# Fadi987/PL-BERT

Measured on AMD Instinct MI355X. Metric: phoneme-tokens/sec, higher is better.
Workload: dtype bf16; 1 GPU; PL-BERT masked-phoneme training step (fwd+loss+bwd+allreduce+AdamW), ALBERT hidden 768 / 12 shared layers / FFN 2048 / 12 heads, seq_len 512, batch 32 per GPU; global_batch=32, seq_len=512, parallelism=dp1

## Files before the change

include/plbert.h:

```cpp
#ifndef PLBERT_H
#define PLBERT_H

#include <stdint.h>

#ifdef __cplusplus
extern "C" {
#endif

typedef struct PlbEngine PlbEngine;

typedef struct {
  int32_t vocab_size;
  int32_t embedding_size;
  int32_t hidden_size;
  int32_t num_attention_heads;
  int32_t intermediate_size;
  int32_t num_hidden_layers;
  int32_t max_position_embeddings;
  int32_t type_vocab_size;
  float layer_norm_eps;
  int32_t num_phonemes;
  int32_t num_tokens;
  int32_t max_batch;
  int32_t max_seq;
  int32_t inference_only;
} PlbConfig;

enum PlbParam {
  PLB_WORD_EMB = 0,
  PLB_POS_EMB,
  PLB_TYPE_EMB,
  PLB_EMB_LN_W,
  PLB_EMB_LN_B,
  PLB_MAP_W,
  PLB_MAP_B,
  PLB_LN2_W,
  PLB_LN2_B,
  PLB_Q_W, PLB_K_W, PLB_V_W,
  PLB_Q_B, PLB_K_B, PLB_V_B,
  PLB_DENSE_W,
  PLB_DENSE_B,
  PLB_LN1_W,
  PLB_LN1_B,
  PLB_FFN_W,
  PLB_FFN_B,
  PLB_FFNO_W,
  PLB_FFNO_B,
  PLB_HEAD_W,
  PLB_HEAD_B,
  PLB_POOL_W,
  PLB_POOL_B,
  PLB_TOK_W,
  PLB_TOK_B,
  PLB_NPARAM
};

const char* plb_last_error(void);

int plb_create(const PlbConfig* cfg, PlbEngine** out);
void plb_destroy(PlbEngine* e);

int plb_param_layout(const PlbEngine* e, int64_t* offsets, int64_t* sizes, int64_t* total, int64_t* trainable);

int64_t plb_workspace_bytes(const PlbEngine* e);

int plb_bind(PlbEngine* e, float* params, float* grads, float* exp_avg, float* exp_avg_sq, void* workspace,
             int64_t workspace_bytes);

int plb_sync_weights(PlbEngine* e, void* stream);

int plb_forward(PlbEngine* e, const int64_t* ids, const int32_t* lengths, int32_t B, int32_t S, float* hidden,
                float* phoneme_logits, float* token_logits, void* stream);

int plb_pooler(PlbEngine* e, const float* hidden, int32_t B, int32_t S, float* pooled, void* stream);

int plb_loss_fwd_bwd(PlbEngine* e, const int64_t* masked_ids, const int64_t* labels, const int32_t* lengths,
                     const int32_t* idx_offsets, const int32_t* idx_flat, int32_t n_masked, int32_t B, int32_t S,
                     float* loss, void* stream);

int plb_loss_fwd(PlbEngine* e, const int64_t* masked_ids, const int64_t* labels, const int64_t* token_ids,
                 const int32_t* lengths, const int32_t* idx_offsets, const int32_t* idx_flat, int32_t n_masked, int32_t B,
                 int32_t S, float* loss, float* loss_parts, void* stream);

int plb_loss_fwd_bwd_dual(PlbEngine* e, const int64_t* masked_ids, const int64_t* labels, const int64_t* token_ids,
                          const int32_t* lengths, const int32_t* idx_offsets, const int32_t* idx_flat, int32_t n_masked,
                          int32_t B, int32_t S, float* loss, float* loss_parts, void* stream);

int plb_adamw_step(PlbEngine* e, double lr, double beta1, double beta2, double eps, double weight_decay, int32_t step,
                   double grad_scale, void* stream);

int64_t plb_grad_norm_floats(const PlbEngine* e);
int plb_grad_accum_bind(PlbEngine* e, float* accum);
int plb_grad_accum_add(PlbEngine* e, int32_t phase, float* norm_buf, void* stream);
int plb_grad_norm(PlbEngine* e, double grad_scale, double max_norm, float* norm_buf, int32_t have_partials, void* stream);
int plb_adamw_step_clipped(PlbEngine* e, double lr, double beta1, double beta2, double eps, double weight_decay,
                           int32_t step, double grad_scale, const float* norm_buf, void* stream);

int plb_set_fp8(PlbEngine* e, int32_t on, void* stream);
int plb_fp8_state(const PlbEngine* e, int32_t* enabled, int32_t* calibrated);
int plb_fp8_stats(PlbEngine* e, float clamped_calls[8], float worst_overshoot[8], void* stream);

int32_t plb_token_head_steps(const PlbEngine* e);
int plb_set_token_head_steps(PlbEngine* e, int32_t steps);

#define PLB_COMM_ID_BYTES 128
int plb_comm_unique_id(uint8_t id[PLB_COMM_ID_BYTES]);
int plb_comm_init(PlbEngine* e, const uint8_t id[PLB_COMM_ID_BYTES], int32_t rank, int32_t world);
int plb_comm_destroy(PlbEngine* e);
int plb_comm_info(const PlbEngine* e, int32_t* rank, int32_t* world, int32_t* rccl_version);
int plb_status(PlbEngine* e, int32_t* ln_exchange_timeouts);
int plb_status_ex(PlbEngine* e, int32_t* ln_exchange_timeouts, int32_t* skipped_updates);
int plb_poll_status(const PlbEngine* e, int32_t* ln_exchange_timeouts);
int plb_status_export(PlbEngine* e, float* out, void* stream);
int plb_status_import(PlbEngine* e, const float* summed, void* stream);
int plb_last_application_rows(const PlbEngine* e, int64_t* rows, int64_t* of);
typedef struct {
  const int32_t* row_start;
  int32_t rows;
  int32_t used;
} PlbPacking;
int plb_packing_plan(const int32_t* lengths, int32_t B, int32_t S, int32_t* row_start, int32_t* rows, int32_t* used);
int plb_forward_packed(PlbEngine* e, const int64_t* ids, const int32_t* lengths, int32_t B, int32_t S,
                       const PlbPacking* packing, float* hidden, float* phoneme_logits, float* token_logits, void* stream);
int plb_loss_fwd_bwd_packed(PlbEngine* e, const int64_t* masked_ids, const int64_t* labels, const int32_t* lengths,
                            const int32_t* idx_offsets, const int32_t* idx_flat, int32_t n_masked, int32_t B, int32_t S,
                            const PlbPacking* packing, float* loss, void* stream);
int plb_loss_fwd_packed(PlbEngine* e, const int64_t* masked_ids, const int64_t* labels, const int64_t* token_ids,
                        const int32_t* lengths, const int32_t* idx_offsets, const int32_t* idx_flat, int32_t n_masked,
                        int32_t B, int32_t S, const PlbPacking* packing, float* loss, float* loss_parts, void* stream);
int plb_last_call_rows(const PlbEngine* e, int64_t* rows, int64_t* of);
int plb_set_packed_dual(PlbEngine* e, int32_t on);
int plb_loss_fwd_bwd_dual_packed(PlbEngine* e, const int64_t* masked_ids, const int64_t* labels, const int64_t* token_ids,
                                 const int32_t* lengths, const int32_t* idx_offsets, const int32_t* idx_flat, int32_t n_masked,
                                 int32_t B, int32_t S, const PlbPacking* packing, float* loss, float* loss_parts, void* stream);
int plb_set_packed_fp8(PlbEngine* e, int32_t on);
int plb_encode(PlbEngine* e, const int64_t* ids, const int32_t* lengths, int32_t B, int32_t S, const PlbPacking* packing,
               float* hidden, void* stream);
int plb_encode_bwd(PlbEngine* e, const int64_t* ids, const int32_t* lengths, int32_t B, int32_t S, const PlbPacking* packing,
                   const float* d_hidden, void* stream);
int plb_comm_pieces(const PlbEngine* e, int32_t* collectives, int64_t* floats);
int plb_broadcast_params(PlbEngine* e, int32_t root, void* stream);
int plb_set_grad_overlap(PlbEngine* e, int32_t overlap);
int plb_allreduce_grads(PlbEngine* e, void* stream);

int plb_apply_mask(const int64_t* ids, const int32_t* sample_off, const int32_t* word_off, const int32_t* word_begin,
                   const int32_t* word_len, const int8_t* action, const int64_t* repl, const int64_t* word_token,
                   int64_t sep_token, const int32_t* crop_start, int32_t B, int32_t S, int32_t mask_id, int64_t* labels,
                   int64_t* masked, int64_t* tokens, int32_t* lengths_out, int32_t* idx_offsets, int32_t* idx_flat,
                   int32_t* scratch, void* stream);

int plb_mask_batch(const int64_t* labels, const int32_t* lengths, int32_t B, int32_t S, uint64_t seed, uint32_t step,
                   float word_pred_prob, float phoneme_mask_prob, float replace_prob, int32_t mask_id, int32_t sep_id,
                   int64_t* masked, int32_t* idx_offsets, int32_t* idx_flat, int32_t* scratch, void* stream);

void plb_profile_enable(int on);
int plb_profile_num_classes(void);
const char* plb_profile_class_name(int cls);
int plb_profile_read(double* ms, int64_t* launches, double* flops, double* bytes);

void plb_debug_skip_piece(int index);
void plb_debug_ln_fault(int mode, int launches);
int plb_debug_hb_audit(PlbEngine* e, int32_t on, int32_t break_wait);
int plb_debug_hb_report(const PlbEngine* e, int64_t* checks, int32_t* violations, char* first, int32_t first_bytes);
int plb_comm_trace(PlbEngine* e, int32_t on);
int plb_comm_trace_read(PlbEngine* e, int32_t max_pieces, int32_t* n, int64_t* begin, int64_t* end, float* released_ms,
                        float* done_ms, float* tail_ms);
void plb_set_gemm_nt_tile(int tile);
void plb_set_gemm_nt_prefetch(int on);
void plb_set_attn_bwd_fused(int on);
void plb_set_prune_last(int on);

#ifdef __cplusplus
}
#endif
#endif
```

plbert_amd/_lib.py:

```python
from __future__ import annotations

import ctypes as C
import os

import torch

HERE = os.path.dirname(os.path.abspath(__file__))
LIB_PATH = os.environ.get("PLBERT_HIP_LIB") or os.path.join(HERE, "libplbert_hip.so")

PLB_PARAM_NAMES = [
    "encoder.embeddings.word_embeddings.weight",
    "encoder.embeddings.position_embeddings.weight",
    "encoder.embeddings.token_type_embeddings.weight",
    "encoder.embeddings.LayerNorm.weight",
    "encoder.embeddings.LayerNorm.bias",
    "encoder.encoder.embedding_hidden_mapping_in.weight",
    "encoder.encoder.embedding_hidden_mapping_in.bias",
    "encoder.encoder.albert_layer_groups.0.albert_layers.0.full_layer_layer_norm.weight",
    "encoder.encoder.albert_layer_groups.0.albert_layers.0.full_layer_layer_norm.bias",
    "encoder.encoder.albert_layer_groups.0.albert_layers.0.attention.query.weight",
    "encoder.encoder.albert_layer_groups.0.albert_layers.0.attention.key.weight",
    "encoder.encoder.albert_layer_groups.0.albert_layers.0.attention.value.weight",
    "encoder.encoder.albert_layer_groups.0.albert_layers.0.attention.query.bias",
    "encoder.encoder.albert_layer_groups.0.albert_layers.0.attention.key.bias",
    "encoder.encoder.albert_layer_groups.0.albert_layers.0.attention.value.bias",
    "encoder.encoder.albert_layer_groups.0.albert_layers.0.attention.dense.weight",
    "encoder.encoder.albert_layer_groups.0.albert_layers.0.attention.dense.bias",
    "encoder.encoder.albert_layer_groups.0.albert_layers.0.attention.LayerNorm.weight",
    "encoder.encoder.albert_layer_groups.0.albert_layers.0.attention.LayerNorm.bias",
    "encoder.encoder.albert_layer_groups.0.albert_layers.0.ffn.weight",
    "encoder.encoder.albert_layer_groups.0.albert_layers.0.ffn.bias",
    "encoder.encoder.albert_layer_groups.0.albert_layers.0.ffn_output.weight",
    "encoder.encoder.albert_layer_groups.0.albert_layers.0.ffn_output.bias",
    "phoneme_predictor.weight",
    "phoneme_predictor.bias",
    "encoder.pooler.weight",
    "encoder.pooler.bias",
    "token_predictor.weight",
    "token_predictor.bias",
]
PLB_NPARAM = len(PLB_PARAM_NAMES)

PUBLIC_SYMBOLS = [
    "plb_last_error", "plb_create", "plb_destroy", "plb_param_layout", "plb_workspace_bytes", "plb_bind",
    "plb_sync_weights", "plb_forward", "plb_pooler", "plb_loss_fwd_bwd", "plb_loss_fwd", "plb_loss_fwd_bwd_dual", "plb_adamw_step",
    "plb_set_fp8", "plb_fp8_state", "plb_fp8_stats", "plb_token_head_steps", "plb_set_token_head_steps", "plb_comm_unique_id", "plb_comm_init", "plb_comm_destroy",
    "plb_comm_info", "plb_comm_pieces", "plb_last_application_rows", "plb_last_call_rows",
    "plb_packing_plan", "plb_forward_packed", "plb_loss_fwd_bwd_packed", "plb_loss_fwd_packed", "plb_set_packed_dual",
    "plb_set_packed_fp8",
    "plb_grad_norm_floats", "plb_grad_accum_bind", "plb_grad_accum_add", "plb_grad_norm", "plb_adamw_step_clipped",
    "plb_loss_fwd_bwd_dual_packed", "plb_encode", "plb_encode_bwd", "plb_status", "plb_status_ex", "plb_poll_status", "plb_status_export", "plb_status_import", "plb_broadcast_params", "plb_set_grad_overlap", "plb_allreduce_grads", "plb_apply_mask",
    "plb_mask_batch", "plb_profile_enable", "plb_profile_num_classes", "plb_profile_class_name", "plb_profile_read",
    "plb_debug_skip_piece", "plb_debug_ln_fault", "plb_debug_hb_audit", "plb_debug_hb_report", "plb_comm_trace", "plb_comm_trace_read",
    "plb_set_gemm_nt_tile", "plb_set_gemm_nt_prefetch", "plb_set_attn_bwd_fused", "plb_set_prune_last",
]


class PlbConfig(C.Structure):
    _fields_ = [
        ("vocab_size", C.c_int32), ("embedding_size", C.c_int32), ("hidden_size", C.c_int32),
        ("num_attention_heads", C.c_int32), ("intermediate_size", C.c_int32), ("num_hidden_layers", C.c_int32),
        ("max_position_embeddings", C.c_int32), ("type_vocab_size", C.c_int32), ("layer_norm_eps", C.c_float),
        ("num_phonemes", C.c_int32), ("num_tokens", C.c_int32), ("max_batch", C.c_int32), ("max_seq", C.c_int32),
        ("inference_only", C.c_int32),
    ]


class PlbGemmNT(C.Structure):
    _fields_ = [
        ("A", C.c_void_p), ("lda", C.c_int), ("B", C.c_void_p), ("ldb", C.c_int),
        ("M", C.c_int), ("N", C.c_int), ("K", C.c_int), ("Mstore", C.c_int),
        ("bias", C.c_void_p), ("res", C.c_void_p), ("ldr", C.c_int), ("aux", C.c_void_p), ("ldaux", C.c_int),
        ("C", C.c_void_p), ("ldc", C.c_int), ("C2", C.c_void_p), ("ldc2", C.c_int), ("Cf", C.c_void_p), ("ldcf", C.c_int),
        ("colpart", C.c_void_p),
        ("ce_cols", C.c_int), ("ce_tgt", C.c_void_p), ("ce_pmax", C.c_void_p), ("ce_psum", C.c_void_p),
        ("ce_tlogit", C.c_void_p), ("ce_lse", C.c_void_p), ("ce_w", C.c_void_p),
        ("deq_a", C.c_void_p), ("deq_b", C.c_void_p), ("C8", C.c_void_p), ("ldc8", C.c_int), ("q_scale", C.c_void_p),
        ("q_amax", C.c_void_p), ("c8_bf8", C.c_int),
        ("ln_gamma", C.c_void_p), ("ln_beta", C.c_void_p), ("ln_mean", C.c_void_p), ("ln_rstd", C.c_void_p),
        ("ln_eps", C.c_float), ("ln_xchg", C.c_void_p), ("ln_err", C.c_void_p), ("ln_fault", C.c_int),
    ]


class PlbGemmTN(C.Structure):
    _fields_ = [
        ("A", C.c_void_p), ("lda", C.c_int), ("Ncols", C.c_int), ("B", C.c_void_p), ("ldb", C.c_int),
        ("Mtot", C.c_int), ("N", C.c_int), ("K", C.c_int), ("rows_per_split", C.c_int), ("splits", C.c_int),
        ("slab", C.c_void_p), ("deq_a", C.c_void_p), ("deq_b", C.c_void_p),
    ]


class PlbAttn(C.Structure):
    _fields_ = [
        ("qkv", C.c_void_p), ("ldqkv", C.c_int), ("lengths", C.c_void_p),
        ("B", C.c_int), ("S", C.c_int), ("NH", C.c_int), ("H", C.c_int), ("scale", C.c_float),
        ("ctx", C.c_void_p), ("ldctx", C.c_int), ("lse", C.c_void_p),
        ("dctx", C.c_void_p), ("lddctx", C.c_int), ("delta", C.c_void_p), ("dqkv", C.c_void_p), ("lddqkv", C.c_int),
        ("colpart", C.c_void_p), ("colpart_accumulate", C.c_int),
        ("ctx8", C.c_void_p), ("ldctx8", C.c_int), ("ctx_scale", C.c_void_p), ("ctx_amax", C.c_void_p),
        ("dqkv8", C.c_void_p), ("lddqkv8", C.c_int), ("dqkv_scale", C.c_void_p), ("dqkv_amax", C.c_void_p),
        ("qoff", C.c_void_p), ("q", C.c_void_p), ("ldq", C.c_int), ("nq_total", C.c_int), ("dq", C.c_void_p), ("lddq", C.c_int),
        ("dq8", C.c_void_p), ("lddq8", C.c_int),
        ("row_start", C.c_void_p),
    ]


class PlbEmbed(C.Structure):
    _fields_ = [
        ("ids", C.c_void_p), ("T", C.c_int), ("S", C.c_int), ("E", C.c_int), ("V", C.c_int),
        ("word", C.c_void_p), ("pos", C.c_void_p), ("type0", C.c_void_p), ("gamma", C.c_void_p), ("beta", C.c_void_p),
        ("eps", C.c_float), ("out", C.c_void_p), ("ldo", C.c_int), ("dout", C.c_void_p), ("lddo", C.c_int),
        ("dx", C.c_void_p), ("dword", C.c_void_p), ("dpos", C.c_void_p), ("partials", C.c_void_p), ("nblocks", C.c_int),
        ("row_start", C.c_void_p), ("lengths", C.c_void_p), ("B", C.c_int), ("fill_slots", C.c_int),
    ]


class PlbPacking(C.Structure):
    _fields_ = [("row_start", C.c_void_p), ("rows", C.c_int32), ("used", C.c_int32)]


class PlbLayerNorm(C.Structure):
    _fields_ = [
        ("x", C.c_void_p), ("ldx", C.c_int), ("gamma", C.c_void_p), ("beta", C.c_void_p), ("eps", C.c_float),
        ("y", C.c_void_p), ("ldy", C.c_int), ("mean", C.c_void_p), ("rstd", C.c_void_p),
        ("T", C.c_int), ("H", C.c_int), ("Tzero", C.c_int),
        ("dy", C.c_void_p), ("lddy", C.c_int), ("dx", C.c_void_p), ("lddx", C.c_int),
        ("partials", C.c_void_p), ("nblocks", C.c_int), ("accumulate", C.c_int),
        ("out8", C.c_void_p), ("ld8", C.c_int), ("q_scale", C.c_void_p), ("q_amax", C.c_void_p),
    ]


PLB_NORM_PARTS = 1024


def norm_chunk(n):
    return (n + PLB_NORM_PARTS * 1024 - 1) // (PLB_NORM_PARTS * 1024) * 1024


def norm_chain(n):
    return 4 * (norm_chunk(n) // 1024) + 6 + 3


_lib = None


class HipLibraryMissing(RuntimeError):
    pass


def lib():
    global _lib
    if _lib is not None:
        return _lib
    if not os.path.exists(LIB_PATH):
        raise HipLibraryMissing(
            f"{LIB_PATH} is missing: build it with `python -m plbert_amd.build` (needs hipcc, gfx950). "
            "There is no CPU fallback for the PL-BERT hot path.")
    try:
        L = C.CDLL(LIB_PATH, mode=C.RTLD_GLOBAL)
    except OSError as ex:
        raise HipLibraryMissing(f"cannot load {LIB_PATH}: {ex}") from ex
    vp, i32, i64p, f32, f64 = C.c_void_p, C.c_int32, C.POINTER(C.c_int64), C.c_float, C.c_double
    L.plb_last_error.restype = C.c_char_p
    L.plb_last_error.argtypes = []
    L.plb_create.restype = C.c_int
    L.plb_create.argtypes = [C.POINTER(PlbConfig), C.POINTER(vp)]
    L.plb_destroy.restype = None
    L.plb_destroy.argtypes = [vp]
    L.plb_param_layout.restype = C.c_int
    L.plb_param_layout.argtypes = [vp, i64p, i64p, i64p, i64p]
    L.plb_workspace_bytes.restype = C.c_int64
    L.plb_workspace_bytes.argtypes = [vp]
    L.plb_bind.restype = C.c_int
    L.plb_bind.argtypes = [vp, vp, vp, vp, vp, vp, C.c_int64]
    L.plb_sync_weights.restype = C.c_int
    L.plb_sync_weights.argtypes = [vp, vp]
    L.plb_forward.restype = C.c_int
    L.plb_forward.argtypes = [vp, vp, vp, i32, i32, vp, vp, vp, vp]
    L.plb_loss_fwd_bwd.restype = C.c_int
    L.plb_loss_fwd_bwd.argtypes = [vp, vp, vp, vp, vp, vp, i32, i32, i32, vp, vp]
    L.plb_loss_fwd_bwd_dual.restype = C.c_int
    L.plb_loss_fwd_bwd_dual.argtypes = [vp, vp, vp, vp, vp, vp, vp, i32, i32, i32, vp, vp, vp]
    L.plb_pooler.restype = C.c_int
    L.plb_pooler.argtypes = [vp, vp, i32, i32, vp, vp]
    L.plb_loss_fwd.restype = C.c_int
    L.plb_loss_fwd.argtypes = [vp, vp, vp, vp, vp, vp, vp, i32, i32, i32, vp, vp, vp]
    L.plb_set_fp8.restype = C.c_int
    L.plb_set_fp8.argtypes = [vp, i32, vp]
    L.plb_fp8_state.restype = C.c_int
    L.plb_fp8_state.argtypes = [vp, C.POINTER(i32), C.POINTER(i32)]
    L.plb_token_head_steps.restype = i32
    L.plb_token_head_steps.argtypes = [vp]
    L.plb_set_token_head_steps.restype = C.c_int
    L.plb_set_token_head_steps.argtypes = [vp, i32]
    L.plb_comm_unique_id.restype = C.c_int
    L.plb_comm_unique_id.argtypes = [vp]
    L.plb_comm_init.restype = C.c_int
    L.plb_comm_init.argtypes = [vp, vp, i32, i32]
    L.plb_comm_destroy.restype = C.c_int
    L.plb_comm_destroy.argtypes = [vp]
    L.plb_comm_info.restype = C.c_int
    L.plb_comm_info.argtypes = [vp, C.POINTER(i32), C.POINTER(i32), C.POINTER(i32)]
    L.plb_status.restype = C.c_int
    L.plb_status.argtypes = [vp, C.POINTER(i32)]
    L.plb_status_ex.restype = C.c_int
    L.plb_status_ex.argtypes = [vp, C.POINTER(i32), C.POINTER(i32)]
    L.plb_poll_status.restype = C.c_int
    L.plb_poll_status.argtypes = [vp, C.POINTER(i32)]
    L.plb_fp8_stats.restype = C.c_int
    L.plb_fp8_stats.argtypes = [vp, C.POINTER(f32), C.POINTER(f32), vp]
    L.plb_last_application_rows.restype = C.c_int
    L.plb_last_application_rows.argtypes = [vp, i64p, i64p]
    if hasattr(L, "plb_packing_plan"):
        pk = C.POINTER(PlbPacking)
        L.plb_last_call_rows.restype = C.c_int
        L.plb_last_call_rows.argtypes = [vp, i64p, i64p]
        L.plb_packing_plan.restype = C.c_int
        L.plb_packing_plan.argtypes = [vp, i32, i32, vp, C.POINTER(i32), C.POINTER(i32)]
        L.plb_forward_packed.restype = C.c_int
        L.plb_forward_packed.argtypes = [vp, vp, vp, i32, i32, pk, vp, vp, vp, vp]
        L.plb_loss_fwd_bwd_packed.restype = C.c_int
        L.plb_loss_fwd_bwd_packed.argtypes = [vp, vp, vp, vp, vp, vp, i32, i32, i32, pk, vp, vp]
        L.plb_loss_fwd_packed.restype = C.c_int
        L.plb_loss_fwd_packed.argtypes = [vp, vp, vp, vp, vp, vp, vp, i32, i32, i32, pk, vp, vp, vp]
        L.plb_launch_ce_prepare_packed.restype = C.c_int
        L.plb_launch_ce_prepare_packed.argtypes = [vp, vp, vp, C.c_int, C.c_int, vp, vp, vp, vp, vp]
        L.plb_launch_unpack_rows.restype = C.c_int
        L.plb_launch_unpack_rows.argtypes = [vp, C.c_int, C.c_int, vp, vp, C.c_int, C.c_int, C.c_int, vp, vp]
    if hasattr(L, "plb_encode"):
        L.plb_encode.restype = C.c_int
        L.plb_encode.argtypes = [vp, vp, vp, i32, i32, C.POINTER(PlbPacking), vp, vp]
        L.plb_encode_bwd.restype = C.c_int
        L.plb_encode_bwd.argtypes = [vp, vp, vp, i32, i32, C.POINTER(PlbPacking), vp, vp]
        L.plb_launch_seed_dy.restype = C.c_int
        L.plb_launch_seed_dy.argtypes = [vp, vp, vp, C.c_int, C.c_int, C.c_int, C.c_int, vp, vp]
    if hasattr(L, "plb_set_packed_dual"):
        L.plb_set_packed_dual.restype = C.c_int
        L.plb_set_packed_dual.argtypes = [vp, i32]
        L.plb_loss_fwd_bwd_dual_packed.restype = C.c_int
        L.plb_loss_fwd_bwd_dual_packed.argtypes = [vp, vp, vp, vp, vp, vp, vp, i32, i32, i32, C.POINTER(PlbPacking), vp, vp, vp]
        L.plb_launch_pack_token_targets.restype = C.c_int
        L.plb_launch_pack_token_targets.argtypes = [vp, vp, vp, C.c_int, C.c_int, C.c_int, vp, vp]
        L.plb_launch_token_ce_combine_packed.restype = C.c_int
        L.plb_launch_token_ce_combine_packed.argtypes = [vp, vp, C.c_int, vp, vp, vp, C.c_int, C.c_int, C.c_int, vp, vp, vp, vp]
    if hasattr(L, "plb_set_packed_fp8"):
        L.plb_set_packed_fp8.restype = C.c_int
        L.plb_set_packed_fp8.argtypes = [vp, i32]
    if hasattr(L, "plb_grad_accum_add"):
        L.plb_grad_norm_floats.restype = C.c_int64
        L.plb_grad_norm_floats.argtypes = [vp]
        L.plb_grad_accum_bind.restype = C.c_int
        L.plb_grad_accum_bind.argtypes = [vp, vp]
        L.plb_grad_accum_add.restype = C.c_int
        L.plb_grad_accum_add.argtypes = [vp, i32, vp, vp]
        L.plb_grad_norm.restype = C.c_int
        L.plb_grad_norm.argtypes = [vp, f64, f64, vp, i32, vp]
        L.plb_adamw_step_clipped.restype = C.c_int
        L.plb_adamw_step_clipped.argtypes = [vp, f64, f64, f64, f64, f64, i32, f64, vp, vp]
        L.plb_launch_grad_accum.restype = C.c_int
        L.plb_launch_grad_accum.argtypes = [vp, vp, C.c_size_t, C.c_int, vp, vp]
        L.plb_launch_grad_sumsq.restype = C.c_int
        L.plb_launch_grad_sumsq.argtypes = [vp, C.c_size_t, vp, vp]
        L.plb_launch_grad_norm_finish.restype = C.c_int
        L.plb_launch_grad_norm_finish.argtypes = [vp, C.c_int, f64, f64, vp, vp]
        L.plb_launch_adamw_clipped.restype = C.c_int
        L.plb_launch_adamw_clipped.argtypes = [vp, vp, vp, vp, vp, C.c_size_t, f64, f64, f64, f64, f64, C.c_int, f64, vp, C.c_int,
                                               vp, C.c_int, vp]
    L.plb_status_export.restype = C.c_int
    L.plb_status_export.argtypes = [vp, vp, vp]
    L.plb_status_import.restype = C.c_int
    L.plb_status_import.argtypes = [vp, vp, vp]
    L.plb_debug_hb_audit.restype = C.c_int
    L.plb_debug_hb_audit.argtypes = [vp, i32, i32]
    L.plb_debug_hb_report.restype = C.c_int
    L.plb_debug_hb_report.argtypes = [vp, i64p, C.POINTER(i32), C.c_char_p, i32]
    L.plb_comm_trace.restype = C.c_int
    L.plb_comm_trace.argtypes = [vp, i32]
    L.plb_comm_trace_read.restype = C.c_int
    L.plb_comm_trace_read.argtypes = [vp, i32, C.POINTER(i32), i64p, i64p, C.POINTER(f32), C.POINTER(f32), C.POINTER(f32)]
    L.plb_debug_ln_fault.restype = None
    L.plb_debug_ln_fault.argtypes = [C.c_int, C.c_int]
    L.plb_debug_skip_piece.restype = None
    L.plb_debug_skip_piece.argtypes = [C.c_int]
    L.plb_comm_pieces.restype = C.c_int
    L.plb_comm_pieces.argtypes = [vp, C.POINTER(i32), C.POINTER(C.c_int64)]
    L.plb_broadcast_params.restype = C.c_int
    L.plb_broadcast_params.argtypes = [vp, i32, vp]
    L.plb_set_grad_overlap.restype = C.c_int
    L.plb_set_grad_overlap.argtypes = [vp, i32]
    L.plb_allreduce_grads.restype = C.c_int
    L.plb_allreduce_grads.argtypes = [vp, vp]
    L.plb_apply_mask.restype = C.c_int
    L.plb_apply_mask.argtypes = [vp, vp, vp, vp, vp, vp, vp, vp, C.c_int64, vp, i32, i32, i32, vp, vp, vp, vp, vp, vp, vp, vp]
    L.plb_adamw_step.restype = C.c_int
    L.plb_adamw_step.argtypes = [vp, f64, f64, f64, f64, f64, i32, f64, vp]
    L.plb_mask_batch.restype = C.c_int
    L.plb_mask_batch.argtypes = [vp, vp, i32, i32, C.c_uint64, C.c_uint32, f32, f32, f32, i32, i32, vp, vp, vp, vp, vp]
    L.plb_profile_enable.restype = None
    L.plb_profile_enable.argtypes = [C.c_int]
    L.plb_profile_num_classes.restype = C.c_int
    L.plb_profile_num_classes.argtypes = []
    L.plb_profile_class_name.restype = C.c_char_p
    L.plb_profile_class_name.argtypes = [C.c_int]
    L.plb_profile_read.restype = C.c_int
    L.plb_profile_read.argtypes = [C.POINTER(C.c_double), i64p, C.POINTER(C.c_double), C.POINTER(C.c_double)]
    L.plb_launch_gemm_nt.restype = C.c_int
    L.plb_launch_gemm_nt.argtypes = [C.POINTER(PlbGemmNT), C.c_int, C.c_int, vp]
    L.plb_set_gemm_nt_tile.restype = None
    L.plb_set_gemm_nt_tile.argtypes = [C.c_int]
    L.plb_set_gemm_nt_prefetch.restype = None
    L.plb_set_gemm_nt_prefetch.argtypes = [C.c_int]
    L.plb_launch_gemm_nt_fp8.restype = C.c_int
    L.plb_launch_gemm_nt_fp8.argtypes = [C.POINTER(PlbGemmNT), C.c_int, C.c_int, vp]
    L.plb_launch_gemm_nt_fp8_ln.restype = C.c_int
    L.plb_launch_gemm_nt_fp8_ln.argtypes = [C.POINTER(PlbGemmNT), C.c_int, C.c_int, vp]
    L.plb_launch_gemm_nt_fp8_gelud.restype = C.c_int
    L.plb_launch_gemm_nt_fp8_gelud.argtypes = [C.POINTER(PlbGemmNT), C.c_int, C.c_int, vp]
    L.plb_launch_gemm_tn.restype = C.c_int
    L.plb_launch_gemm_tn.argtypes = [C.POINTER(PlbGemmTN), vp]
    L.plb_launch_gemm_tn_big.restype = C.c_int
    L.plb_launch_gemm_tn_big.argtypes = [C.POINTER(PlbGemmTN), vp]
    L.plb_launch_gemm_tn_fp8.restype = C.c_int
    L.plb_launch_gemm_tn_fp8.argtypes = [C.POINTER(PlbGemmTN), vp]
    L.plb_launch_reduce_slabs.restype = C.c_int
    L.plb_launch_reduce_slabs.argtypes = [vp, C.c_int, C.c_size_t, vp, C.c_int, vp]
    L.plb_launch_attn_fwd.restype = C.c_int
    L.plb_launch_attn_fwd.argtypes = [C.POINTER(PlbAttn), vp]
    L.plb_launch_gemm_nt_ln.restype = C.c_int
    L.plb_launch_gemm_nt_ln.argtypes = [C.POINTER(PlbGemmNT), C.c_int, vp]
    L.plb_launch_gemm_nt_gelud.restype = C.c_int
    L.plb_launch_gemm_nt_gelud.argtypes = [C.POINTER(PlbGemmNT), C.c_int, vp]
    L.plb_launch_attn_bwd.restype = C.c_int
    L.plb_launch_attn_bwd.argtypes = [C.POINTER(PlbAttn), vp]
    L.plb_launch_attn_bwd_fused.restype = C.c_int
    L.plb_launch_attn_bwd_fused.argtypes = [C.POINTER(PlbAttn), vp]
    L.plb_set_prune_last.restype = None
    L.plb_set_prune_last.argtypes = [C.c_int]
    L.plb_set_attn_bwd_fused.restype = None
    L.plb_set_attn_bwd_fused.argtypes = [C.c_int]
    L.plb_launch_ln_fwd.restype = C.c_int
    L.plb_launch_ln_fwd.argtypes = [C.POINTER(PlbLayerNorm), vp]
    L.plb_launch_ln_bwd.restype = C.c_int
    L.plb_launch_ln_bwd.argtypes = [C.POINTER(PlbLayerNorm), vp]
    L.plb_launch_embed_scatter.restype = C.c_int
    L.plb_launch_embed_scatter.argtypes = [C.POINTER(PlbEmbed), C.c_int, vp]
    L.plb_launch_ce_prepare.restype = C.c_int
    L.plb_launch_ce_prepare.argtypes = [vp, vp, vp, C.c_int, C.c_int, vp, vp, vp, vp]
    L.plb_launch_colsum.restype = C.c_int
    L.plb_launch_colsum.argtypes = [vp, C.c_int, C.c_size_t, C.c_int, C.c_int, vp, C.c_int, C.c_int, vp, C.c_int, vp]
    _lib = L
    return L


def profile_enable(on):
    lib().plb_profile_enable(int(bool(on)))


def profile_read():
    L = lib()
    n = L.plb_profile_num_classes()
    ms, fl, by = (C.c_double * n)(), (C.c_double * n)(), (C.c_double * n)()
    cnt = (C.c_int64 * n)()
    check(L.plb_profile_read(ms, cnt, fl, by), "plb_profile_read")
    return {L.plb_profile_class_name(i).decode(): dict(ms=ms[i], launches=int(cnt[i]), flops=fl[i], bytes=by[i])
            for i in range(n) if cnt[i]}


def check(rc, what):
    if rc != 0:
        msg = lib().plb_last_error().decode("utf-8", "replace")
        raise RuntimeError(f"{what} failed: {msg or 'rc=%d' % rc}")
```

plbert_amd/csrc/engine.cpp:

```cpp
#include <stdarg.h>

#include <new>

#include "engine_internal.h"

static thread_local char g_err[512] = "";
int fail(const char* fmt, ...) {
  va_list ap;
  va_start(ap, fmt);
  vsnprintf(g_err, sizeof(g_err), fmt, ap);
  va_end(ap);
  return 1;
}
extern "C" const char* plb_last_error(void) { return g_err; }

static void layout_params(PlbEngine* e) {
  const int64_t V = e->V, E = e->E, H = e->H, I = e->I, P = e->P, NP = e->NP, NT = e->NT;
  int64_t sz[PLB_NPARAM];
  sz[PLB_WORD_EMB] = V * E; sz[PLB_POS_EMB] = P * E; sz[PLB_TYPE_EMB] = (int64_t)e->c.type_vocab_size * E;
  sz[PLB_EMB_LN_W] = E; sz[PLB_EMB_LN_B] = E;
  sz[PLB_MAP_W] = H * E; sz[PLB_MAP_B] = H;
  sz[PLB_LN2_W] = H; sz[PLB_LN2_B] = H;
  sz[PLB_Q_W] = sz[PLB_K_W] = sz[PLB_V_W] = H * H;
  sz[PLB_Q_B] = sz[PLB_K_B] = sz[PLB_V_B] = H;
  sz[PLB_DENSE_W] = H * H; sz[PLB_DENSE_B] = H;
  sz[PLB_LN1_W] = H; sz[PLB_LN1_B] = H;
  sz[PLB_FFN_W] = I * H; sz[PLB_FFN_B] = I;
  sz[PLB_FFNO_W] = H * I; sz[PLB_FFNO_B] = H;
  sz[PLB_HEAD_W] = NP * H; sz[PLB_HEAD_B] = NP;
  sz[PLB_POOL_W] = H * H; sz[PLB_POOL_B] = H;
  sz[PLB_TOK_W] = NT * H; sz[PLB_TOK_B] = NT;
  int64_t off = 0;
  for (int i = 0; i < PLB_NPARAM; ++i) {
    e->poff[i] = off;
    e->psize[i] = sz[i];
    off += sz[i];
    if (i == PLB_HEAD_B) e->ptrain = off;
  }
  e->ptotal = off;
}

namespace {
struct Carve {
  int64_t off = 0;
  int64_t take(int64_t bytes) {
    int64_t o = off;
    off = rup(off + bytes, 256);
    return o;
  }
};
}

extern "C" int plb_create(const PlbConfig* cfg, PlbEngine** out) {
  if (!cfg || !out) return fail("plb_create: null argument");
  const PlbConfig& c = *cfg;
  if (c.hidden_size != c.num_attention_heads * 64) return fail("plb_create: head_dim must be 64 (hidden %d, heads %d)", c.hidden_size, c.num_attention_heads);
  if (c.embedding_size % 64 || c.embedding_size > 256) return fail("plb_create: embedding_size must be a multiple of 64, <= 256");
  if (c.hidden_size % 128 || c.hidden_size > 1024) return fail("plb_create: hidden_size must be a multiple of 128, <= 1024");
  if (c.intermediate_size % 128) return fail("plb_create: intermediate_size must be a multiple of 128");
  if (c.num_phonemes < 4 || c.num_phonemes % 4 || c.num_phonemes > 256) return fail("plb_create: num_phonemes must be a multiple of 4 in [4,256]");
  if (c.num_tokens < 0 || c.num_tokens % 4) return fail("plb_create: num_tokens must be a non-negative multiple of 4");
  if (c.max_seq < 1 || c.max_seq > c.max_position_embeddings) return fail("plb_create: max_seq must be in [1, max_position_embeddings]");
  if (c.max_batch < 1 || c.num_hidden_layers < 1 || c.vocab_size < 1 || c.type_vocab_size < 1) return fail("plb_create: bad sizes");
  PlbEngine* e = new (std::nothrow) PlbEngine();
  if (!e) return fail("plb_create: out of host memory");
  e->c = c;
  e->E = c.embedding_size; e->H = c.hidden_size; e->I = c.intermediate_size; e->L = c.num_hidden_layers;
  e->NH = c.num_attention_heads; e->V = c.vocab_size; e->P = c.max_position_embeddings;
  e->NP = c.num_phonemes; e->NT = c.num_tokens;
  layout_params(e);
  const int64_t E = e->E, H = e->H, I = e->I, L = e->L;
  const int64_t T = (int64_t)c.max_batch * c.max_seq;
  const int64_t Tp = rup(T, 128);
  e->infer = c.inference_only != 0;
  const bool tr = !e->infer;
  const int64_t Ls = tr ? L : 1;
  e->Tcap = Tp;
  e->NMcap = Tp;
  e->ln_blocks = 512;
  if (const char* v = getenv("PLBERT_LN_BLOCKS")) { const int n = atoi(v); if (n >= 64 && n <= 4096) e->ln_blocks = n; }
  e->emb_blocks = 2048;
  if (const char* v = getenv("PLBERT_LN_FUSE"))
    e->ln_fuse = !strcmp(v, "off") ? 0 : !strcmp(v, "fwd") ? 1 : !strcmp(v, "bwd") ? 2 : 3;
  e->part_rows = e->ln_blocks > (int)(2 * Tp / 128) ? e->ln_blocks : (int)(2 * Tp / 128);
  if (const char* v = getenv("PLBERT_GELU_STASH")) e->gelu_dstash_on = strcmp(v, "u") != 0;
  if (const char* v = getenv("PLBERT_FP8_TN")) e->fp8_tn = strcmp(v, "0") != 0;
  if (const char* v = getenv("PLBERT_HB_AUDIT")) e->hb.on = strcmp(v, "0") != 0;
  Carve cv;
  e->o_wbf = cv.take((e->ptotal + 256 * (H > I ? H : I)) * 2);
  if (tr) {
    e->o_wqkvT = cv.take(rup(H, 128) * 3 * H * 2);
    e->o_wdT = cv.take(rup(H, 128) * H * 2);
    e->o_w1T = cv.take(rup(H, 128) * I * 2);
    e->o_w2T = cv.take(rup(I, 128) * H * 2);
    e->o_wpT = cv.take(rup(H, 128) * 256 * 2);
    e->o_winT = cv.take(rup(E, 128) * H * 2);
  }
  e->o_e = cv.take(Tp * E * 2);
  e->o_x = cv.take((tr ? L + 1 : 2) * Tp * H * 2);
  e->o_qkv = cv.take(Ls * Tp * 3 * H * 2);
  e->o_ctx = cv.take(Ls * Tp * H * 2);
  e->o_pre1 = cv.take(Ls * Tp * H * 2);
  e->o_a = cv.take(Ls * Tp * H * 2);
  e->o_u = cv.take(Ls * Tp * I * 2);
  e->o_g = cv.take(Ls * Tp * I * 2);
  e->o_pre2 = cv.take(Ls * Tp * H * 2);
  const int64_t stat = (int64_t)c.max_batch * e->NH * c.max_seq * 4;
  e->o_lse = cv.take(Ls * stat);
  e->o_mean1 = cv.take(Ls * Tp * 4); e->o_rstd1 = cv.take(Ls * Tp * 4);
  e->o_mean2 = cv.take(Ls * Tp * 4); e->o_rstd2 = cv.take(Ls * Tp * 4);
  e->lnx_bytes = (Tp / 128) * 16 * 128 * 2 * 8;
  e->o_lnx = cv.take(e->lnx_bytes);
  e->o_lnerr = cv.take(256);
  if (tr) {
    e->o_delta = cv.take(stat);
    e->o_dqkv = cv.take(L * Tp * 3 * H * 2);
    e->o_dpre1 = cv.take(L * Tp * H * 2);
    e->o_du = cv.take(L * Tp * I * 2);
    e->o_dpre2 = cv.take(L * Tp * H * 2);
    e->o_dy0 = cv.take(Tp * H * 2); e->o_dy1 = cv.take(Tp * H * 2);
    e->o_da = cv.take(Tp * H * 2); e->o_dctx = cv.take(Tp * H * 2);
    e->o_de = cv.take(Tp * E * 2);
  }
  const int64_t NM = e->NMcap;
  e->o_hm = cv.take(NM * H * 2);
  e->o_logm = cv.take(NM * 256 * 4);
  e->o_dlog = cv.take(NM * 256 * 2);
  e->o_rows = cv.take(NM * 4); e->o_tgt = cv.take(NM * 4); e->o_w = cv.take(NM * 4); e->o_lrows = cv.take(NM * 4);
  if (tr) {
    e->o_dhm = cv.take(NM * H * 2);
    int64_t slab = 0;
    {
      const int64_t Mtot = L * Tp;
      const int ntp = (int)rup(e->NT, 256);
      const int shapes[7][2] = {{(int)(3 * H), (int)H}, {(int)H, (int)H}, {(int)I, (int)H}, {(int)H, (int)I}, {(int)H, (int)E}, {e->NP, (int)H}, {ntp, (int)H}};
      for (int i = 0; i < (e->NT ? 7 : 6); ++i) {
        int rps;
        const int64_t mt = i < 4 ? Mtot : Tp;
        const int s = tn_splits(mt, shapes[i][0], shapes[i][1], &rps);
        const int64_t f = (int64_t)s * shapes[i][0] * shapes[i][1];
        if (f > slab) slab = f;
      }
    }
    e->slab_floats = slab;
    e->o_slab = cv.take(slab * 4);
    e->o_part1 = cv.take(L * e->part_rows * 3 * H * 4);
    e->o_part2 = cv.take(L * e->part_rows * 3 * H * 4);
    e->o_parte = cv.take((int64_t)e->emb_blocks * 2 * E * 4);
    e->o_dxe = cv.take(Tp * E * 4);
    e->o_ducol = cv.take(L * (2 * Tp / 128) * I * 4);
    e->qkvcol_rows = c.max_batch * ((c.max_seq + 127) / 128) * 4;
    e->o_qkvcol = cv.take((int64_t)L * e->qkvcol_rows * 3 * H * 4);
    e->o_scratch = cv.take(512 * (3 * H > I ? 3 * H : I) * 4);
    e->o_scratch2 = cv.take(512 * (3 * H > I ? 3 * H : I) * 4);
    {
      int rps;
      const int s2 = tn_splits(Tp, (int)H, (int)E, &rps);
      e->slab2_floats = (int64_t)s2 * H * E;
      e->o_slab2 = cv.take(e->slab2_floats * 4);
    }
  }
  if (e->NT) {
    const int64_t NTp = rup(e->NT, 256);
    e->NTp = (int)NTp;
    e->o_bt = cv.take(NTp * 4);
    e->o_tlrows = cv.take(Tp * 4);
    e->o_tpmax = cv.take(Tp * (NTp / 256) * 4);
    e->o_tpsum = cv.take(Tp * (NTp / 256) * 4);
    e->o_ttl = cv.take(Tp * 4); e->o_tlse = cv.take(Tp * 4); e->o_tw = cv.take(Tp * 4);
    e->o_ttgt = cv.take(Tp * 8);
    e->o_tloss = cv.take(256);
    if (tr) {
      e->o_wtT = cv.take(rup(H, 128) * NTp * 2);
      e->o_tdl = cv.take(Tp * NTp * 2);
      e->o_tscr = cv.take(32 * NTp * 4);
      e->o_tcolp = cv.take(2 * (Tp / 128) * NTp * 4);
      e->o_tgrad = cv.take(NTp * H * 4);
    }
  }
  e->o_x8 = cv.take(Ls * Tp * H); e->o_a8 = cv.take(Ls * Tp * H); e->o_g8 = cv.take(Ls * Tp * I); e->o_c8 = cv.take(Ls * Tp * H);
  e->o_wq8 = cv.take(rup(3 * H, 128) * H + 256 * H);
  e->o_wd8 = cv.take(rup(H, 128) * H + 256 * H);
  e->o_w18 = cv.take(rup(I, 128) * H + 256 * H);
  e->o_w28 = cv.take(rup(H, 128) * I + 256 * I);
  if (tr) {
    e->o_dp8 = cv.take(L * Tp * H); e->o_du8 = cv.take(L * Tp * I); e->o_dp18 = cv.take(L * Tp * H); e->o_dq8 = cv.take(L * Tp * 3 * H);
    e->o_w2T8 = cv.take(rup(I, 128) * H + 256 * H);
    e->o_w1T8 = cv.take(rup(H, 128) * I + 256 * I);
    e->o_wqT8 = cv.take(rup(H, 128) * 3 * H + 256 * 3 * H);
    e->o_wdT8 = cv.take(rup(H, 128) * H + 256 * H);
  }
  e->f8n = 8 * (int)L + 8;
  e->o_f8amax = cv.take((int64_t)e->f8n * 64 * 16 * 4); e->o_f8scale = cv.take(e->f8n * 4); e->o_f8deq = cv.take(e->f8n * 4);
  e->o_f8stats = cv.take(8 * 8 * 4);
  e->ws_bytes = cv.off;
  *out = e;
  return 0;
}

extern "C" void plb_destroy(PlbEngine* e) {
  if (!e) return;
  (void)plb_comm_destroy(e);
  if (e->ev_fork) (void)hipEventDestroy(e->ev_fork);
  if (e->ev_join) (void)hipEventDestroy(e->ev_join);
  if (e->side) (void)hipStreamDestroy(e->side);
  if (e->host_err) (void)hipHostFree(e->host_err);
  for (auto& t : e->trace) { (void)hipEventDestroy(t.released); (void)hipEventDestroy(t.done); }
  for (auto ev : e->trace_pool) (void)hipEventDestroy(ev);
  for (auto ev : {e->tr_call0, e->tr_tail0, e->tr_tail1}) if (ev) (void)hipEventDestroy(ev);
  delete e;
}

extern "C" int plb_param_layout(const PlbEngine* e, int64_t* offsets, int64_t* sizes, int64_t* total, int64_t* trainable) {
  if (!e) return fail("plb_param_layout: null engine");
  for (int i = 0; i < PLB_NPARAM; ++i) {
    if (offsets) offsets[i] = e->poff[i];
    if (sizes) sizes[i] = e->psize[i];
  }
  if (total) *total = e->ptotal;
  if (trainable) *trainable = e->ptrain;
  return 0;
}

extern "C" int64_t plb_workspace_bytes(const PlbEngine* e) { return e ? e->ws_bytes : -1; }

extern "C" int plb_bind(PlbEngine* e, float* params, float* grads, float* exp_avg, float* exp_avg_sq, void* workspace,
                        int64_t workspace_bytes) {
  if (!e || !params || !workspace) return fail("plb_bind: null argument");
  if (workspace_bytes < e->ws_bytes) return fail("plb_bind: workspace too small (%lld < %lld)", (long long)workspace_bytes, (long long)e->ws_bytes);
  if (((uintptr_t)params | (uintptr_t)grads | (uintptr_t)exp_avg | (uintptr_t)exp_avg_sq) & 15) return fail("plb_bind: buffers must be 16-byte aligned");
  if ((uintptr_t)workspace & 255) return fail("plb_bind: workspace must be 256-byte aligned");
  e->params = params; e->grads = grads; e->m = exp_avg; e->v = exp_avg_sq;
  e->ws = (char*)workspace;
  if (!e->host_err) {
    void* h = nullptr;
    if (hipHostMalloc(&h, 64, hipHostMallocMapped) == hipSuccess && h) {
      void* d = nullptr;
      if (hipHostGetDevicePointer(&d, h, 0) == hipSuccess && d) {
        e->host_err = (unsigned int*)h;
        e->host_err_dev = (unsigned int*)d;
        *e->host_err = 0;
      } else {
        (void)hipHostFree(h);
      }
    }
    if (!e->host_err) return fail("plb_bind: cannot allocate the pinned status word");
  }
  if (!e->side && grads && !getenv("PLBERT_NO_SIDE_STREAM")) {
    if (hipStreamCreateWithFlags(&e->side, hipStreamNonBlocking) != hipSuccess) e->side = nullptr;
    if (e->side && (hipEventCreateWithFlags(&e->ev_fork, kStreamOrderEvent) != hipSuccess ||
                    hipEventCreateWithFlags(&e->ev_join, kStreamOrderEvent) != hipSuccess)) {
      (void)hipStreamDestroy(e->side);
      e->side = nullptr;
    }
  }
  return 0;
}

int sync_transposes(PlbEngine* e, hipStream_t s, bool exact_fp8) {
  const int H = e->H, I = e->I, E = e->E;

  if (e->NT) {
    if (!e->tok_pad_zeroed) HIPTRY(hipMemsetAsync(e->at<float>(e->o_bt), 0, (size_t)e->NTp * 4, s));
    HIPTRY(hipMemcpyAsync(e->at<float>(e->o_bt), e->par(PLB_TOK_B), (size_t)e->NT * 4, hipMemcpyDeviceToDevice, s));
  }
  if (e->infer) {
    e->tok_pad_zeroed = true;
    if (e->fp8_on) return fp8_quantize_weights(e, s, exact_fp8 || e->fp8_wstale);
    return 0;
  }
  const float* tsrc[8] = {e->par(PLB_Q_W), e->par(PLB_DENSE_W), e->par(PLB_FFN_W), e->par(PLB_FFNO_W), e->par(PLB_HEAD_W),
                          e->par(PLB_MAP_W)};
  bf16_t* tdst[8] = {e->at<bf16_t>(e->o_wqkvT), e->at<bf16_t>(e->o_wdT), e->at<bf16_t>(e->o_w1T), e->at<bf16_t>(e->o_w2T),
                     e->at<bf16_t>(e->o_wpT), e->at<bf16_t>(e->o_winT)};
  int tR[8] = {3 * H, H, I, H, e->NP, H}, tC[8] = {H, H, H, I, H, E}, tld[8] = {3 * H, H, I, H, 256, H};
  int nt = 6;
  if (e->NT) {
    if (!e->tok_pad_zeroed) HIPTRY(hipMemsetAsync(e->at<bf16_t>(e->o_wtT), 0, (size_t)rup(H, 128) * e->NTp * 2, s));
    tsrc[nt] = e->par(PLB_TOK_W); tdst[nt] = e->at<bf16_t>(e->o_wtT); tR[nt] = e->NT; tC[nt] = H; tld[nt] = e->NTp;
    ++nt;
  }
  TRY(plb_launch_transpose_cast_multi(nt, tsrc, tR, tC, tdst, tld, s));
  e->tok_pad_zeroed = true;
  if (e->fp8_on) return fp8_quantize_weights(e, s, exact_fp8 || e->fp8_wstale);
  return 0;
}

extern "C" int plb_sync_weights(PlbEngine* e, void* stream) {
  if (!e || !e->ws) return fail("plb_sync_weights: engine not bound");
  drop_stash(e, "plb_sync_weights refreshed the compute copies since");
  end_accum_window(e, "plb_sync_weights refreshed the compute copies");
  hipStream_t s = (hipStream_t)stream;
  TRY(plb_launch_cast_bf16(e->params, e->at<bf16_t>(e->o_wbf), (size_t)e->ptotal, s));
  return sync_transposes(e, s);
}

extern "C" int plb_pooler(PlbEngine* e, const float* hidden, int32_t B, int32_t S, float* pooled, void* stream) {
  if (!e || !e->ws) return fail("plb_pooler: engine not bound");
  if (!hidden || !pooled || B < 1 || S < 1) return fail("plb_pooler: bad argument");
  TRY(plb_launch_pooler(hidden, B, S, e->H, e->par(PLB_POOL_W), e->par(PLB_POOL_B), pooled, (hipStream_t)stream));
  return 0;
}

#ifndef PLB_PACK_GRAN_MAX
#define PLB_PACK_GRAN_MAX 1024
#endif
extern "C" int plb_packing_plan(const int32_t* lengths, int32_t B, int32_t S, int32_t* row_start, int32_t* rows,
                                int32_t* used) {
  if (!lengths || !row_start || !rows || !used) return fail("plb_packing_plan: null argument");
  if (B < 1 || S < 1 || (int64_t)B * S > (int64_t)1 << 30) return fail("plb_packing_plan: bad shape %d x %d", B, S);
  const int64_t padded = rup((int64_t)B * S, 128);
  int64_t at = 0;
  bool full = true;
  for (int b = 0; b < B; ++b) {
    const int len = lengths[b] < 1 ? 1 : (lengths[b] > S ? S : lengths[b]);
    full = full && len == S;
    at += rup(len, 128);
  }
  const int64_t gran = (PLB_PACK_GRAN_MAX >= 1024 && rup(at, 1024) < padded) ? 1024
                       : (PLB_PACK_GRAN_MAX >= 256 && rup(at, 256) < padded) ? 256 : 128;
  if (full || rup(at, gran) >= padded) {
    for (int b = 0; b <= B; ++b) row_start[b] = b * S;
    *rows = (int32_t)padded; *used = B * S;
    return 0;
  }
  at = 0;
  for (int b = 0; b < B; ++b) {
    const int len = lengths[b] < 1 ? 1 : (lengths[b] > S ? S : lengths[b]);
    row_start[b] = (int32_t)at;
    at += rup(len, 128);
  }
  row_start[B] = (int32_t)at;
  *used = (int32_t)at;
  *rows = (int32_t)rup(at, gran);
  return 0;
}

extern "C" int plb_last_application_rows(const PlbEngine* e, int64_t* rows, int64_t* of) {
  if (!e) return fail("plb_last_application_rows: null engine");
  if (rows) *rows = e->last_app_rows[0];
  if (of) *of = e->last_app_rows[1];
  return 0;
}

extern "C" int plb_last_call_rows(const PlbEngine* e, int64_t* rows, int64_t* of) {
  if (!e) return fail("plb_last_call_rows: null engine");
  if (rows) *rows = e->last_exec_rows[0];
  if (of) *of = e->last_exec_rows[1];
  return 0;
}

extern "C" int plb_set_packed_dual(PlbEngine* e, int32_t on) {
  if (!e) return fail("plb_set_packed_dual: null engine");
  e->packed_dual = on != 0;
  return 0;
}
extern "C" int plb_set_packed_fp8(PlbEngine* e, int32_t on) {
  if (!e) return fail("plb_set_packed_fp8: null engine");
  e->packed_fp8 = on != 0;
  return 0;
}

extern "C" int32_t plb_token_head_steps(const PlbEngine* e) { return e ? e->tok_steps : -1; }
extern "C" int plb_set_token_head_steps(PlbEngine* e, int32_t steps) {
  if (!e || steps < 0) return fail("plb_set_token_head_steps: bad argument");
  e->tok_steps = steps;
  return 0;
}

extern "C" int plb_apply_mask(const int64_t* ids, const int32_t* sample_off, const int32_t* word_off,
                              const int32_t* word_begin, const int32_t* word_len, const int8_t* action, const int64_t* repl,
                              const int64_t* word_token, int64_t sep_token, const int32_t* crop_start, int32_t B, int32_t S,
                              int32_t mask_id, int64_t* labels, int64_t* masked, int64_t* tokens, int32_t* lengths_out,
                              int32_t* idx_offsets, int32_t* idx_flat, int32_t* scratch, void* stream) {
  if (!ids || !sample_off || !word_off || !word_begin || !word_len || !action || !repl || !crop_start || !labels || !masked ||
      !lengths_out || !idx_offsets || !idx_flat || !scratch)
    return fail("plb_apply_mask: null argument");
  if ((tokens != nullptr) != (word_token != nullptr)) return fail("plb_apply_mask: tokens and word_token go together");
  if (S < 1 || S > 1024 || B < 1 || B > 1024) return fail("plb_apply_mask: needs 1 <= S <= 1024, 1 <= B <= 1024");
  PlbApplyMask m;
  memset(&m, 0, sizeof(m));
  m.ids = ids; m.sample_off = sample_off; m.word_off = word_off; m.word_begin = word_begin; m.word_len = word_len;
  m.action = action; m.repl = repl; m.word_token = word_token; m.sep_token = sep_token; m.crop_start = crop_start;
  m.B = B; m.S = S; m.mask_id = mask_id;
  m.labels = labels; m.masked = masked; m.tokens = tokens; m.lengths_out = lengths_out;
  m.counts = scratch; m.idx_padded = scratch + B; m.offsets = idx_offsets; m.flat = idx_flat;
  TRY(plb_launch_apply_mask(&m, (hipStream_t)stream));
  return 0;
}

extern "C" int plb_mask_batch(const int64_t* labels, const int32_t* lengths, int32_t B, int32_t S, uint64_t seed,
                              uint32_t step, float word_pred_prob, float phoneme_mask_prob, float replace_prob,
                              int32_t mask_id, int32_t sep_id, int64_t* masked, int32_t* idx_offsets, int32_t* idx_flat,
                              int32_t* scratch, void* stream) {
  if (!labels || !masked || !idx_offsets || !idx_flat || !scratch) return fail("plb_mask_batch: null argument");
  if (S < 1 || S > 512 || B < 1 || B > 1024) return fail("plb_mask_batch: needs 1 <= S <= 512, 1 <= B <= 1024");
  PlbMask m;
  memset(&m, 0, sizeof(m));
  m.labels = labels; m.lengths = lengths; m.B = B; m.S = S; m.seed = seed; m.step = step;
  m.word_pred_prob = word_pred_prob; m.mask_prob = phoneme_mask_prob; m.replace_prob = replace_prob;
  m.mask_id = mask_id; m.sep_id = sep_id;
  m.masked = masked; m.counts = scratch; m.idx_padded = scratch + B; m.offsets = idx_offsets; m.flat = idx_flat;
  TRY(plb_launch_mask(&m, (hipStream_t)stream));
  return 0;
}

extern "C" int plb_adamw_step(PlbEngine* e, double lr, double beta1, double beta2, double eps, double weight_decay,
// ... 25 lines not shown
```

plbert_amd/csrc/engine_calls.cpp:

```cpp
#include "engine_internal.h"

void drop_stash(PlbEngine* e, const char* by) {
  if (e && e->stash_live) { e->stash_live = false; e->stash_dead_by = by; }
}

static int check_shape(const PlbEngine* e, int B, int S, const char* who) {
  if (!e || !e->ws) return fail("%s: engine not bound", who);
  if (B < 1 || S < 1 || B > e->c.max_batch || S > e->c.max_seq || (int64_t)B * S > (int64_t)e->c.max_batch * e->c.max_seq)
    return fail("%s: batch %d x seq %d exceeds the engine capacity %d x %d", who, B, S, e->c.max_batch, e->c.max_seq);
  return 0;
}

static Rows padded_rows(int B, int S) { return Rows{nullptr, B * S, rup(B * S, 128)}; }
static int pick_rows(PlbEngine* e, const PlbPacking* pk, const int32_t* lengths, bool padded, int B, int S, const char* who,
                     Rows* out) {
  *out = padded_rows(B, S);
  e->last_exec_rows[0] = e->last_exec_rows[1] = (int64_t)B * S;
  if (!pk || !pk->row_start) return 0;
  if (pk->rows < 128 || pk->rows % 128 || pk->used < 1 || pk->used > pk->rows)
    return fail("%s: packing plan of %d rows (%d used) is not one plb_packing_plan made", who, pk->rows, pk->used);
  if (pk->rows > out->Tp) return fail("%s: packing plan of %d rows exceeds the call's %lld", who, pk->rows, (long long)out->Tp);
  if (!lengths || padded || (e->fp8_on && !e->packed_fp8) || pk->rows == out->Tp) return 0;
  if (pk->used % 128) return fail("%s: packing plan with %d used rows: slots are multiples of 128", who, pk->used);
  *out = Rows{pk->row_start, pk->used, pk->rows};
// ... 101 lines not shown

static int phoneme_head(PlbEngine* e, bool backward, bool prune, const bf16_t* xL, int n_masked, int64_t Tp, bf16_t* dy,
                        float* loss, hipStream_t s) {
  const int H = e->H, NP = e->NP;
  const int NM = (int)rup(n_masked, 128);
  int32_t* rows = e->at<int32_t>(e->o_rows);
  bf16_t* hm = e->at<bf16_t>(e->o_hm);
  float* logm = e->at<float>(e->o_logm);
  float* lrows = e->at<float>(e->o_lrows);
  bf16_t* dlog = e->at<bf16_t>(e->o_dlog);
  bf16_t* dhm = e->at<bf16_t>(e->o_dhm);
  if (backward && !prune) HIPTRY(hipMemsetAsync(dy, 0, (size_t)Tp * H * 2, s));
  if (n_masked > 0) {
    if (!prune) TRY(plb_launch_gather_rows(xL, H, rows, n_masked, NM, H, hm, H, s));
    PlbGemmNT g = nt_desc(hm, e->wbf(PLB_HEAD_W), NM, NP, H);
    g.bias = e->par(PLB_HEAD_B); g.Cf = logm; g.ldcf = 256;
    TRY(plb_launch_gemm_nt(&g, 0, 1, s));
    TRY(plb_launch_ce_fwd_bwd(logm, 256, NP, e->at<int32_t>(e->o_tgt), e->at<float>(e->o_w), n_masked, NM, lrows, dlog, 256, s));
    TRY(plb_launch_sum_rows(lrows, n_masked, loss, s));
    if (backward) {
      if (weight_grad(e, dlog, 256, 256, hm, H, NM, NP, H, e->grd(PLB_HEAD_W), s)) return 1;
      TRY(plb_launch_colsum(dlog, 1, (size_t)NM, 256, 256, e->grd(PLB_HEAD_B), NP, 0, e->at<float>(e->o_scratch), 8, s));
      g = nt_desc(dlog, e->at<bf16_t>(e->o_wpT), NM, H, 256);
      g.C = dhm; g.ldc = H;
      TRY(plb_launch_gemm_nt(&g, 0, 0, s));
      if (!prune) TRY(plb_launch_scatter_rows(dhm, H, rows, n_masked, H, dy, H, s));
    }
  } else {
    HIPTRY(hipMemsetAsync(loss, 0, sizeof(float), s));
    if (backward)
      HIPTRY(hipMemsetAsync(e->grd(PLB_HEAD_W), 0, (size_t)(e->psize[PLB_HEAD_W] + e->psize[PLB_HEAD_B]) * 4, s));
  }
  if (!backward) return 0;
  HB_W(s, e->grd(PLB_HEAD_W), (e->ptrain - e->poff[PLB_HEAD_W]) * 4, "phoneme head gradients (weight-gradient GEMM, bias column sums)");
  if (overlapping(e) && reduce_pieces(e, kPieceHead, kPieceHead + 1, s)) return 1;
  return 0;
}

static int token_head(PlbEngine* e, bool backward, const bf16_t* xL, const int64_t* token_targets, const int32_t* lengths,
                      int B, int S, const Rows& rw, bf16_t* dy, float* loss, float* loss_parts, hipStream_t s) {
  const int H = e->H, NT = e->NT, NTp = e->NTp, T = B * S;
  const int64_t Tp = rw.Tp;
  const int tile = (Tp % 256 == 0) ? 256 : 1256;
  const int ntile = NTp / 256, cprows = tile == 256 ? 2 * (int)(Tp / 256) : 2 * (int)(Tp / 128);
  float* tlrows = e->at<float>(e->o_tlrows);
  float* tloss = e->at<float>(e->o_tloss);
  int64_t* ttgt = e->at<int64_t>(e->o_ttgt);
  if (rw.row_start) {
    TRY(plb_launch_pack_token_targets(token_targets, lengths, rw.row_start, B, S, (int)Tp, ttgt, s));
  } else {
  HIPTRY(hipMemcpyAsync(ttgt, token_targets, (size_t)T * 8, hipMemcpyDeviceToDevice, s));
  if (Tp > T) HIPTRY(hipMemsetAsync(ttgt + T, 0, (size_t)(Tp - T) * 8, s));
  }
  PlbGemmNT g = nt_desc(xL, e->wbf(PLB_TOK_W), Tp, NTp, H);
  g.bias = e->at<float>(e->o_bt);
  g.ce_cols = NT; g.ce_tgt = ttgt;
  g.ce_pmax = e->at<float>(e->o_tpmax); g.ce_psum = e->at<float>(e->o_tpsum); g.ce_tlogit = e->at<float>(e->o_ttl);
  const double ce_flops = 2.0 * (double)Tp * NTp * H;
  int tok = plb_prof_begin(PLB_K_GEMM_NT_CE, s, ce_flops, 0.0);
  TRY(plb_launch_gemm_nt_big(&g, tile, 3, 0, s));
  plb_prof_end(tok, s);
  if (rw.row_start) {
    TRY(plb_launch_token_ce_combine_packed(g.ce_pmax, g.ce_psum, ntile, g.ce_tlogit, lengths, rw.row_start, B, S, (int)Tp,
                                           e->at<float>(e->o_tlse), e->at<float>(e->o_tw), tlrows, s));
    TRY(plb_launch_sum_rows(tlrows, (int)Tp, tloss, s));
  } else {
  TRY(plb_launch_token_ce_combine(g.ce_pmax, g.ce_psum, ntile, g.ce_tlogit, lengths, B, S, (int)Tp,
                                  e->at<float>(e->o_tlse), e->at<float>(e->o_tw), tlrows, s));
  TRY(plb_launch_sum_rows(tlrows, T, tloss, s));
  }
  TRY(plb_launch_add_scalar(loss, loss, tloss, s));
  if (loss_parts) HIPTRY(hipMemcpyAsync(loss_parts + 1, tloss, sizeof(float), hipMemcpyDeviceToDevice, s));
  if (!backward) return 0;
  bf16_t* tdl = e->at<bf16_t>(e->o_tdl);
  g.ce_lse = e->at<float>(e->o_tlse); g.ce_w = e->at<float>(e->o_tw);
  g.C = tdl; g.ldc = NTp; g.colpart = e->at<float>(e->o_tcolp);
  tok = plb_prof_begin(PLB_K_GEMM_NT_CE, s, ce_flops, 0.0);
  TRY(plb_launch_gemm_nt_big(&g, tile, 4, 0, s));
  plb_prof_end(tok, s);
  TRY(plb_launch_colsum(g.colpart, 0, (size_t)cprows, NTp, NTp, e->grd(PLB_TOK_B), NT, 0, e->at<float>(e->o_tscr), 1, s));
  float* gw = NTp == NT ? e->grd(PLB_TOK_W) : e->at<float>(e->o_tgrad);
  if (weight_grad(e, tdl, NTp, NTp, xL, H, Tp, NTp, H, gw, s)) return 1;
  if (NTp != NT) HIPTRY(hipMemcpyAsync(e->grd(PLB_TOK_W), gw, (size_t)NT * H * 4, hipMemcpyDeviceToDevice, s));
  HB_W(s, e->grd(PLB_TOK_W), (e->ptotal - e->poff[PLB_TOK_W]) * 4, "token head gradients");
  if (overlapping(e) && reduce_piece(e, e->poff[PLB_TOK_W], e->ptotal, s)) return 1;
  g = nt_desc(tdl, e->at<bf16_t>(e->o_wtT), Tp, H, NTp);
  g.res = dy; g.ldr = H; g.C = dy; g.ldc = H;
  TRY(plb_launch_gemm_nt(&g, 0, 0, s));
  return 0;
}

static int backward_tail_streams(PlbEngine* e, const int64_t* masked_ids, const int32_t* lengths, bf16_t* dy, int B, int S,
                                 const Rows& rw, int du_rows, hipStream_t s, hipStream_t s2, float* scratch2) {
  const int E = e->E, H = e->H, I = e->I, L = e->L;
  const int T = rw.T;
  const int64_t Tp = rw.Tp;
  const int64_t Mtot = (int64_t)L * Tp;
  const int64_t Mtot_c = e->pruned_rows ? (int64_t)(L - 1) * Tp + e->pruned_rows : Mtot;
  const Slots st = slots(e, Tp, B, S, 0, true, e->part_rows_used, du_rows);
  const int64_t qkvcol_all = (int64_t)L * qkvcol_rows(B, S);
  bf16_t* evec = e->at<bf16_t>(e->o_e);
  bf16_t* de = e->at<bf16_t>(e->o_de);
  PlbGemmNT g = nt_desc(dy, e->at<bf16_t>(e->o_winT), Tp, E, H);
  g.C = de; g.ldc = E;
  HB_R(s2, dy, Tp * H * 2, "dX of application 0"); HB_W(s2, de, Tp * E * 2, "dE (map-in backward)");
  TRY(plb_launch_gemm_nt(&g, 0, 0, s2));
  HB_W(s2, e->at<float>(s2 != s ? e->o_slab2 : e->o_slab), (s2 != s ? e->slab2_floats : e->slab_floats) * 4, "map-in weight-gradient slab");
  HB_W(s2, e->grd(PLB_MAP_W), e->psize[PLB_MAP_W] * 4, "map-in weight gradient");
  if (weight_grad(e, dy, H, H, evec, E, Tp, H, E, e->grd(PLB_MAP_W), s2, s2 != s)) return 1;
  HB_W(s2, scratch2, 512 * (3 * H > I ? 3 * H : I) * 4, "column-sum scratch of the side stream");
  HB_W(s2, e->grd(PLB_MAP_B), H * 4, "map-in bias gradient");
  TRY(plb_launch_colsum(dy, 1, (size_t)Tp, H, H, e->grd(PLB_MAP_B), H, 0, scratch2, 128, s2));
  HB_W(s2, e->grd(PLB_TYPE_EMB), e->psize[PLB_TYPE_EMB] * 4, "token-type embedding gradient");
  HIPTRY(hipMemsetAsync(e->grd(PLB_TYPE_EMB), 0, (size_t)e->psize[PLB_TYPE_EMB] * 4, s2));
  PlbEmbed em;
  memset(&em, 0, sizeof(em));
  em.ids = masked_ids; em.T = T; em.S = S; em.E = E; em.V = e->V;
  em.word = e->par(PLB_WORD_EMB); em.pos = e->par(PLB_POS_EMB); em.type0 = e->par(PLB_TYPE_EMB);
  em.gamma = e->par(PLB_EMB_LN_W); em.beta = e->par(PLB_EMB_LN_B); em.eps = e->c.layer_norm_eps;
  em.dout = de; em.lddo = E; em.dword = e->grd(PLB_WORD_EMB); em.dpos = e->grd(PLB_POS_EMB);
  em.dx = e->at<float>(e->o_dxe);
  em.partials = e->at<float>(e->o_parte); em.nblocks = e->emb_blocks;
  if (rw.row_start) { em.row_start = rw.row_start; em.lengths = lengths; em.B = B; }
  HB_W(s2, em.dx, Tp * E * 4, "embedding LayerNorm backward rows"); HB_W(s2, em.partials, (int64_t)e->emb_blocks * 2 * E * 4, "embedding LayerNorm partials");
  HB_W(s2, e->grd(PLB_WORD_EMB), (e->poff[PLB_MAP_W] - e->poff[PLB_WORD_EMB]) * 4, "embedding tables' and embedding LayerNorm's gradients");
  TRY(plb_launch_embed_bwd(&em, s2));
  TRY(plb_launch_embed_scatter(&em, e->P, s2));
  TRY(plb_launch_colsum(em.partials, 0, (size_t)e->emb_blocks, 2 * E, 2 * E, e->grd(PLB_EMB_LN_W), 2 * E, 0, scratch2, 1, s2));
  TRY(plb_launch_colsum(e->grd(PLB_POS_EMB), 0, (size_t)e->P, E, E, e->grd(PLB_TYPE_EMB), E, 0, scratch2, 1, s2));
  HB_R(s2, st.qkvcol, qkvcol_all * 3 * H * 4, "Q/K/V bias partial rows");
  HB_W(s2, e->grd(PLB_Q_B), 3 * H * 4, "Q/K/V bias gradients");
  TRY(plb_launch_colsum(st.qkvcol, 0, (size_t)qkvcol_all, 3 * H, 3 * H, e->grd(PLB_Q_B), 3 * H, 0, scratch2, 64, s2));
  HB_W(s2, e->grd(PLB_FFN_B), I * 4, "ffn.bias gradient");
  if (du_rows > 0) {
    HB_R(s2, st.ducol, (int64_t)L * du_rows * I * 4, "dU column-sum partial rows");
    TRY(plb_launch_colsum(st.ducol, 0, (size_t)L * du_rows, I, I, e->grd(PLB_FFN_B), I, 0, scratch2, 16, s2));
  } else {
    HB_R(s2, st.du, Mtot_c * I * 2, "dU of every application");
    TRY(plb_launch_colsum(st.du, 1, (size_t)Mtot_c, I, I, e->grd(PLB_FFN_B), I, 0, scratch2, 64, s2));
  }
  const size_t prow = (size_t)L * e->part_rows_used;
  HB_R(s2, st.part1, (int64_t)L * e->part_rows * 3 * H * 4, "LayerNorm-1 backward partial rows");
  HB_W(s2, e->grd(PLB_DENSE_B), 3 * H * 4, "dense.bias + LayerNorm-1 affine gradients");
  TRY(plb_launch_colsum(st.part1, 0, prow, 3 * H, 3 * H, e->grd(PLB_LN1_W), 2 * H, 0, scratch2, 64, s2));
  TRY(plb_launch_copy_cols(scratch2, 64, 3 * H, 2 * H, H, e->grd(PLB_DENSE_B), s2));
  HB_R(s2, st.part2, (int64_t)L * e->part_rows * 3 * H * 4, "LayerNorm-2 backward partial rows");
  HB_W(s2, e->grd(PLB_LN2_W), 2 * H * 4, "LayerNorm-2 affine gradients"); HB_W(s2, e->grd(PLB_FFNO_B), H * 4, "ffn_output.bias gradient");
  TRY(plb_launch_colsum(st.part2, 0, prow, 3 * H, 3 * H, e->grd(PLB_LN2_W), 2 * H, 0, scratch2, 64, s2));
  TRY(plb_launch_copy_cols(scratch2, 64, 3 * H, 2 * H, H, e->grd(PLB_FFNO_B), s2));
  if (s2 != s) HIPTRY(ev_record(e, e->ev_join, s2));
  const bool ov = overlapping(e);
  const bool t8 = e->tn8_call;
  float* const slab = e->at<float>(e->o_slab);
  HB_W(s, slab, e->slab_floats * 4, "weight-gradient slab"); HB_W(s, e->grd(PLB_Q_W), 3 * H * H * 4, "Q/K/V weight gradients");
  if (t8 ? weight_grad8(e, st.dq8, st.x8, Mtot, 3 * H, H, F8_DQ, F8_X, e->grd(PLB_Q_W), s)
         : weight_grad(e, st.dqkv, 3 * H, 3 * H, st.x, H, Mtot, 3 * H, H, e->grd(PLB_Q_W), s)) return 1;
  if (ov && reduce_pieces(e, kPieceQkvW, kPieceFfnW, s)) return 1;
  HB_W(s, slab, e->slab_floats * 4, "weight-gradient slab"); HB_W(s, e->grd(PLB_FFN_W), (int64_t)I * H * 4, "ffn.weight gradient");
  if (t8 ? weight_grad8(e, st.du8, st.a8, Mtot_c, I, H, F8_DU, F8_A, e->grd(PLB_FFN_W), s)
         : weight_grad(e, st.du, I, I, st.a, H, Mtot_c, I, H, e->grd(PLB_FFN_W), s)) return 1;
  if (ov && reduce_pieces(e, kPieceFfnW, kPieceSmall, s)) return 1;
  if (ov) {
    if (reduce_pieces(e, kPieceSmall, kPieceFfnoW, s2)) return 1;
  }
  HB_W(s, slab, e->slab_floats * 4, "weight-gradient slab"); HB_W(s, e->grd(PLB_FFNO_W), (int64_t)I * H * 4, "ffn_output.weight gradient");
  if (t8 ? weight_grad8(e, st.dp8, st.g8, Mtot_c, H, I, F8_DP, F8_G, e->grd(PLB_FFNO_W), s)
         : weight_grad(e, st.dpre2, H, H, st.g, I, Mtot_c, H, I, e->grd(PLB_FFNO_W), s)) return 1;
  if (ov && reduce_pieces(e, kPieceFfnoW, kPieceDenseW, s)) return 1;
  HB_W(s, slab, e->slab_floats * 4, "weight-gradient slab"); HB_W(s, e->grd(PLB_DENSE_W), (int64_t)H * H * 4, "dense.weight gradient");
  if (t8 ? weight_grad8(e, st.dp18, st.c8, Mtot_c, H, H, F8_DP1, F8_C, e->grd(PLB_DENSE_W), s)
         : weight_grad(e, st.dpre1, H, H, st.ctx, H, Mtot_c, H, H, e->grd(PLB_DENSE_W), s)) return 1;
  if (ov && reduce_pieces(e, kPieceDenseW, kNPieces, s)) return 1;
  return 0;
}

static int backward_tail(PlbEngine* e, const int64_t* masked_ids, const int32_t* lengths, bf16_t* dy, int B, int S,
                         const Rows& rw, int du_rows, hipStream_t s) {
  hipStream_t s2 = s;
  float* scratch2 = e->at<float>(e->o_scratch);
  HB_W(s, e->ws, e->ws_bytes, "layer loop (whole workspace)");
  if (e->trace_on) (void)hipEventRecord(e->tr_tail0, s);
  if (e->side) {
    s2 = e->side;
    scratch2 = e->at<float>(e->o_scratch2);
    HIPTRY(ev_record(e, e->ev_fork, s));
    HIPTRY(ev_wait(e, s2, e->ev_fork));
  }
  const int rc = backward_tail_streams(e, masked_ids, lengths, dy, B, S, rw, du_rows, s, s2, scratch2);
  if (s2 != s) {
    if (rc) (void)ev_record(e, e->ev_join, s2);
    const hipError_t je = ev_wait(e, s, e->ev_join);
    if (!rc && je != hipSuccess) return fail("plb_loss_fwd_bwd: joining the side stream: %s", hipGetErrorString(je));
  }
  if (e->trace_on) { (void)hipEventRecord(e->tr_tail1, s); e->tr_tail_valid = true; }
  if (rc) return rc;
  HB_W(s, e->ws, e->ws_bytes, "after the side stream's join (whole workspace)");
  return pieces_done(e);
}

static int loss_impl(PlbEngine* e, bool backward, const int64_t* masked_ids, const int64_t* labels,
                     const int64_t* token_targets, const int32_t* lengths, const int32_t* idx_offsets,
                     const int32_t* idx_flat, int32_t n_masked, int32_t B, int32_t S, const PlbPacking* pk, float* loss,
                     float* loss_parts, void* stream) {
  const char* who = backward ? "plb_loss_fwd_bwd" : "plb_loss_fwd";
  if (check_shape(e, B, S, who)) return 1;
  drop_stash(e, "a plb_loss_* call rewrote the workspace since");
  if (backward && e->infer) return fail("%s: inference-only engine (PlbConfig.inference_only = 1)", who);
  if (backward && !e->grads) return fail("%s: no gradient buffer bound", who);
  if (!masked_ids || !labels || !idx_offsets || !loss) return fail("%s: null argument", who);
  if (n_masked < 0 || n_masked > e->NMcap) return fail("%s: n_masked %d out of range", who, n_masked);
  if (token_targets && !e->NT) return fail("%s: the engine has no token head (num_tokens = 0)", who);
  hipStream_t s = (hipStream_t)stream;
  Rows rw;
  if (pick_rows(e, pk, lengths, token_targets != nullptr && !e->packed_dual, B, S, who, &rw)) return 1;
  const int64_t Tp = rw.Tp;
  if (backward && begin_training_call(e, token_targets != nullptr, s)) return 1;
  if (n_masked == 0 && !token_targets) return zero_loss_call(e, backward, loss, s);

  const int NM = (int)rup(n_masked, 128);
  Prune pr = {e->at<int32_t>(e->o_rows), n_masked, NM};
  const bool prune = prune_enabled() && n_masked > 0 && !token_targets && e->L >= 2 && 2 * (int64_t)NM <= Tp;
  if (n_masked > 0) {
    if (rw.row_start)
      TRY(plb_launch_ce_prepare_packed(idx_offsets, idx_flat, labels, B, S, rw.row_start, e->at<int32_t>(e->o_rows),
                                       e->at<int32_t>(e->o_tgt), e->at<float>(e->o_w), s));
    else
      TRY(plb_launch_ce_prepare(idx_offsets, idx_flat, labels, B, S, e->at<int32_t>(e->o_rows), e->at<int32_t>(e->o_tgt),
                                e->at<float>(e->o_w), s));
  }
  if (backward) e->pruned_rows = prune ? NM : 0;
  e->last_app_rows[0] = prune ? NM : Tp; e->last_app_rows[1] = Tp;
  bf16_t* xL = nullptr;
  if (run_encoder(e, masked_ids, lengths, B, S, rw, backward, &xL, s, prune ? &pr : nullptr)) return 1;
  bf16_t* dy = backward ? e->at<bf16_t>(e->o_dy0) : nullptr;
  if (phoneme_head(e, backward, prune, xL, n_masked, Tp, dy, loss, s)) return 1;
  if (loss_parts) HIPTRY(hipMemcpyAsync(loss_parts, loss, sizeof(float), hipMemcpyDeviceToDevice, s));
  if (token_targets && token_head(e, backward, xL, token_targets, lengths, B, S, rw, dy, loss, loss_parts, s)) return 1;
  if (!backward) {
    if (e->fp8_on) {
      TRY(fp8_update_scales(e, s));
      e->fp8_ready = true;
    }
    e->last_loss = loss;
    TRY(plb_launch_step_status(e->at<unsigned int>(e->o_lnerr), loss, e->host_err_dev, nullptr, s));
    return 0;
  }

  int du_rows = 0;
  if (encoder_bwd(e, prune ? &pr : nullptr, lengths, B, S, rw, &dy, &du_rows, s)) return 1;
  if (status_exchange(e, s)) return 1;
  if (backward_tail(e, masked_ids, lengths, dy, B, S, rw, du_rows, s)) return 1;
  if (e->fp8_on) {
    TRY(fp8_update_scales(e, s));
    e->fp8_ready = true;
    e->fp8_bwd_ready = true;
  }
  return status_finish(e, loss, s);
}

extern "C" int plb_loss_fwd_bwd(PlbEngine* e, const int64_t* masked_ids, const int64_t* labels, const int32_t* lengths,
                                const int32_t* idx_offsets, const int32_t* idx_flat, int32_t n_masked, int32_t B,
                                int32_t S, float* loss, void* stream) {
  return loss_impl(e, true, masked_ids, labels, nullptr, lengths, idx_offsets, idx_flat, n_masked, B, S, nullptr, loss, nullptr,
                   stream);
}
extern "C" int plb_loss_fwd_bwd_packed(PlbEngine* e, const int64_t* masked_ids, const int64_t* labels, const int32_t* lengths,
                                       const int32_t* idx_offsets, const int32_t* idx_flat, int32_t n_masked, int32_t B,
                                       int32_t S, const PlbPacking* packing, float* loss, void* stream) {
  return loss_impl(e, true, masked_ids, labels, nullptr, lengths, idx_offsets, idx_flat, n_masked, B, S, packing, loss, nullptr,
                   stream);
}

extern "C" int plb_loss_fwd_bwd_dual(PlbEngine* e, const int64_t* masked_ids, const int64_t* labels,
                                     const int64_t* token_ids, const int32_t* lengths, const int32_t* idx_offsets,
                                     const int32_t* idx_flat, int32_t n_masked, int32_t B, int32_t S, float* loss,
                                     float* loss_parts, void* stream) {
  if (!token_ids) return fail("plb_loss_fwd_bwd_dual: token_ids is null");
  return loss_impl(e, true, masked_ids, labels, token_ids, lengths, idx_offsets, idx_flat, n_masked, B, S, nullptr, loss,
                   loss_parts, stream);
}

extern "C" int plb_loss_fwd_bwd_dual_packed(PlbEngine* e, const int64_t* masked_ids, const int64_t* labels,
                                            const int64_t* token_ids, const int32_t* lengths, const int32_t* idx_offsets,
                                            const int32_t* idx_flat, int32_t n_masked, int32_t B, int32_t S,
                                            const PlbPacking* packing, float* loss, float* loss_parts, void* stream) {
  if (!token_ids) return fail("plb_loss_fwd_bwd_dual_packed: token_ids is null");
  return loss_impl(e, true, masked_ids, labels, token_ids, lengths, idx_offsets, idx_flat, n_masked, B, S, packing, loss,
                   loss_parts, stream);
}

extern "C" int plb_loss_fwd(PlbEngine* e, const int64_t* masked_ids, const int64_t* labels, const int64_t* token_ids,
                            const int32_t* lengths, const int32_t* idx_offsets, const int32_t* idx_flat, int32_t n_masked,
                            int32_t B, int32_t S, float* loss, float* loss_parts, void* stream) {
  return loss_impl(e, false, masked_ids, labels, token_ids, lengths, idx_offsets, idx_flat, n_masked, B, S, nullptr, loss,
                   loss_parts, stream);
}
extern "C" int plb_loss_fwd_packed(PlbEngine* e, const int64_t* masked_ids, const int64_t* labels, const int64_t* token_ids,
                                   const int32_t* lengths, const int32_t* idx_offsets, const int32_t* idx_flat,
                                   int32_t n_masked, int32_t B, int32_t S, const PlbPacking* packing, float* loss,
                                   float* loss_parts, void* stream) {
  return loss_impl(e, false, masked_ids, labels, token_ids, lengths, idx_offsets, idx_flat, n_masked, B, S, packing, loss,
                   loss_parts, stream);
}

extern "C" int plb_encode(PlbEngine* e, const int64_t* ids, const int32_t* lengths, int32_t B, int32_t S,
                          const PlbPacking* pk, float* hidden, void* stream) {
  if (check_shape(e, B, S, "plb_encode")) return 1;
  if (e->infer) return fail("plb_encode: inference-only engine (PlbConfig.inference_only = 1): a differentiable forward keeps every application's activations");
  if (!e->grads) return fail("plb_encode: no gradient buffer bound");
  if (e->fp8_on) return fail("plb_encode: fp8 mode is on (the gradient sites' delayed scales belong to the pre-training loss); call plb_set_fp8(e, 0, stream) first");
  if (!ids || !hidden) return fail("plb_encode: %s is null", !ids ? "ids" : "hidden");
  hipStream_t s = (hipStream_t)stream;
  Rows rw;
  if (pick_rows(e, pk, lengths, false, B, S, "plb_encode", &rw)) return 1;
  drop_stash(e, "a plb_encode call that failed rewrote the workspace since");
  HB_W(s, e->ws, e->ws_bytes, "plb_encode (whole workspace)");
  e->last_app_rows[0] = e->last_app_rows[1] = rw.Tp;
  bf16_t* x = nullptr;
  if (run_encoder(e, ids, lengths, B, S, rw, true, &x, s)) return 1;
  if (lengths) TRY(plb_launch_unpack_rows(x, 1, e->H, rw.row_start, lengths, B, S, e->H, hidden, s));
  else TRY(plb_launch_bf16_to_f32(x, e->H, hidden, e->H, rw.T, e->H, s));
  TRY(plb_launch_step_status(e->at<unsigned int>(e->o_lnerr), nullptr, e->host_err_dev, nullptr, s));
  e->stash_live = true;
  e->stash_B = B; e->stash_S = S; e->stash_rows = rw.Tp; e->stash_used = rw.T; e->stash_row_start = rw.row_start;
  return 0;
}

extern "C" int plb_encode_bwd(PlbEngine* e, const int64_t* ids, const int32_t* lengths, int32_t B, int32_t S,
                              const PlbPacking* pk, const float* d_hidden, void* stream) {
  if (check_shape(e, B, S, "plb_encode_bwd")) return 1;
  if (e->infer) return fail("plb_encode_bwd: inference-only engine (PlbConfig.inference_only = 1)");
  if (!e->grads) return fail("plb_encode_bwd: no gradient buffer bound");
  if (!ids || !d_hidden) return fail("plb_encode_bwd: %s is null", !ids ? "ids" : "d_hidden");
  if (!e->stash_live) return fail("plb_encode_bwd: no live plb_encode stash: %s", e->stash_dead_by);
  if (B != e->stash_B || S != e->stash_S)
    return fail("plb_encode_bwd: batch %d x seq %d differs from the plb_encode call's %d x %d", B, S, e->stash_B, e->stash_S);
  hipStream_t s = (hipStream_t)stream;
  Rows rw;
  const int64_t exec_rows[2] = {e->last_exec_rows[0], e->last_exec_rows[1]};
  const bool plan_ok = pick_rows(e, pk, lengths, false, B, S, "plb_encode_bwd", &rw) == 0;
  const bool same = plan_ok && rw.Tp == e->stash_rows && rw.T == e->stash_used && rw.row_start == e->stash_row_start;
// ... 26 lines not shown
```

plbert_amd/csrc/engine_comm.cpp:

```cpp
#include <dlfcn.h>

#include "engine_internal.h"

namespace {
struct RcclId { char internal[128]; };
enum { kNcclSuccess = 0, kNcclFloat32 = 7, kNcclSum = 0 };
struct RcclApi {
  void* handle = nullptr;
  int (*GetUniqueId)(RcclId*) = nullptr;
  int (*CommInitRank)(RcclComm*, int, RcclId, int) = nullptr;
  int (*CommDestroy)(RcclComm) = nullptr;
  int (*AllReduce)(const void*, void*, size_t, int, int, RcclComm, hipStream_t) = nullptr;
  int (*Broadcast)(const void*, void*, size_t, int, int, RcclComm, hipStream_t) = nullptr;
  int (*GetVersion)(int*) = nullptr;
  const char* (*GetErrorString)(int) = nullptr;
  bool ok = false;
};
RcclApi g_rccl;
const char* rccl_load() {
  if (g_rccl.ok) return nullptr;
  const char* env = getenv("PLBERT_RCCL_LIB");
  void* h = nullptr;
  if (env && *env) h = dlopen(env, RTLD_NOW | RTLD_GLOBAL);
  if (!h) h = dlopen("librccl.so.1", RTLD_NOW | RTLD_NOLOAD);
  if (!h) h = dlopen("librccl.so.1", RTLD_NOW | RTLD_GLOBAL);
  if (!h) h = dlopen("librccl.so", RTLD_NOW | RTLD_GLOBAL);
  if (!h) return "cannot load librccl.so.1 (set PLBERT_RCCL_LIB)";
  g_rccl.handle = h;
#define RSYM(field, name) \
  *(void**)(&g_rccl.field) = dlsym(h, name); \
  if (!g_rccl.field) return "librccl lacks " name
  RSYM(GetUniqueId, "ncclGetUniqueId");
  RSYM(CommInitRank, "ncclCommInitRank");
  RSYM(CommDestroy, "ncclCommDestroy");
  RSYM(AllReduce, "ncclAllReduce");
  RSYM(Broadcast, "ncclBroadcast");
  RSYM(GetVersion, "ncclGetVersion");
  RSYM(GetErrorString, "ncclGetErrorString");
#undef RSYM
  g_rccl.ok = true;
  return nullptr;
}
}

void HbAudit::wait(int st, hipEvent_t e) {
  const int n = waits++;
  if (n == break_wait) { break_wait = -1; return; }
  auto it = ev.find(e);
  if (it == ev.end()) return;
  for (int i = 0; i < NS; ++i) if (it->second[i] > vc[st][i]) vc[st][i] = it->second[i];
}
void HbAudit::access(int st, const void* p, size_t bytes, bool wr, const char* what) {
  if (!p || !bytes) return;
  const uintptr_t a = (uintptr_t)p, b = a + bytes;
  vc[st][st] += 1;
  for (const Acc& x : log) {
    if (x.st == st || !(wr || x.wr) || x.b <= a || b <= x.a) continue;
    ++checks;
    if (x.tick > vc[st][x.st]) {
      if (!violations++) {
        char m[384];
        snprintf(m, sizeof(m), "%s of '%s' on the %s stream is not ordered after the %s of '%s' on the %s stream", wr ? "write" : "read",
                 what, name(st), x.wr ? "write" : "read", x.what, name(x.st));
        first = m;
      }
    }
  }
  log.push_back(Acc{what, a, b, st, vc[st][st], wr});
}

int hb_idx(const PlbEngine* e, hipStream_t s) {
  if (e->side && s == e->side) return HbAudit::SIDE;
  if (e->comm_stream && s == e->comm_stream) return HbAudit::COMM;
  return HbAudit::MAIN;
}
hipError_t ev_record(PlbEngine* e, hipEvent_t ev, hipStream_t s) {
  const hipError_t r = hipEventRecord(ev, s);
  if (e->hb.on) e->hb.record(ev, hb_idx(e, s));
  return r;
}
hipError_t ev_wait(PlbEngine* e, hipStream_t s, hipEvent_t ev) {
  const hipError_t r = hipStreamWaitEvent(s, ev, 0);
  if (e->hb.on) e->hb.wait(hb_idx(e, s), ev);
  return r;
}

static int g_debug_skip_piece = -1;
extern "C" void plb_debug_skip_piece(int index) { g_debug_skip_piece = index; }

static hipEvent_t trace_event(PlbEngine* e) {
  if (!e->trace_pool.empty()) { hipEvent_t v = e->trace_pool.back(); e->trace_pool.pop_back(); return v; }
  hipEvent_t v = nullptr;
  (void)hipEventCreate(&v);
  return v;
}
int reduce_piece(PlbEngine* e, int64_t a, int64_t b, hipStream_t after) {
  if (!e->comm || b <= a) return 0;
  if (g_debug_skip_piece >= 0 && e->piece_count == g_debug_skip_piece) {
    g_debug_skip_piece = -1;
    e->piece_count += 1;
    return 0;
  }
  PlbEngine::PieceTrace tr{a, b, nullptr, nullptr};
  if (e->trace_on) {
    tr.released = trace_event(e); tr.done = trace_event(e);
    (void)hipEventRecord(tr.released, after);
  }
  HIPTRY(ev_record(e, e->ev_piece, after));
  HIPTRY(ev_wait(e, e->comm_stream, e->ev_piece));
  HB_W(e->comm_stream, e->grads + a, (b - a) * 4, "all-reduce piece (in place)");
  const int rc = g_rccl.AllReduce(e->grads + a, e->grads + a, (size_t)(b - a), kNcclFloat32, kNcclSum, e->comm, e->comm_stream);
  if (rc != kNcclSuccess) return fail("ncclAllReduce: %s", g_rccl.GetErrorString(rc));
  if (e->trace_on) {
    (void)hipEventRecord(tr.done, e->comm_stream);
    e->trace.push_back(tr);
  }
  e->comm_pending = true;
  e->piece_floats += b - a;
  e->piece_count += 1;
  return 0;
}
bool overlapping(const PlbEngine* e) { return e->comm && e->overlap; }
int pieces_done(PlbEngine* e) {
  if (e->hb.on && e->hb.violations)
    return fail("happens-before audit: %d violation(s), first: %s", e->hb.violations, e->hb.first.c_str());
  if (!e->comm_pending) return 0;
  const int64_t want = e->ptrain + (e->tok_grads_live ? e->ptotal - e->poff[PLB_TOK_W] : 0);
  if (e->piece_floats != want)
    return fail("gradient exchange covered %lld of %lld floats", (long long)e->piece_floats, (long long)want);
  HIPTRY(ev_record(e, e->ev_comm_done, e->comm_stream));
  e->grads_reduced = true;
  return 0;
}
struct PieceRange { int begin, end; };
static const PieceRange kPieces[] = {
    {PLB_HEAD_W, PLB_HEAD_B + 1},
    {PLB_Q_W, PLB_Q_B},
    {PLB_FFN_W, PLB_FFN_B},
    {PLB_WORD_EMB, PLB_Q_W}, {PLB_Q_B, PLB_DENSE_W}, {PLB_DENSE_B, PLB_FFN_W}, {PLB_FFN_B, PLB_FFNO_W}, {PLB_FFNO_B, PLB_HEAD_W},
    {PLB_FFNO_W, PLB_FFNO_B},
    {PLB_DENSE_W, PLB_DENSE_B}};
static_assert(sizeof(kPieces) / sizeof(kPieces[0]) == kNPieces, "piece table");
int64_t piece_begin(const PlbEngine* e, int i) { return e->poff[kPieces[i].begin]; }
int64_t piece_end(const PlbEngine* e, int i) { return e->poff[kPieces[i].end]; }
int reduce_pieces(PlbEngine* e, int from, int to, hipStream_t after) {
  for (int i = from; i < to; ++i)
    if (reduce_piece(e, piece_begin(e, i), piece_end(e, i), after)) return 1;
  return 0;
}

static float* status_float(const PlbEngine* e) { return e->at<float>(e->o_lnerr) + 16; }
int status_exchange(PlbEngine* e, hipStream_t s) {
  if (!e->comm) return 0;
  float* f = status_float(e);
  TRY(plb_launch_status_export(e->at<unsigned int>(e->o_lnerr), f, s));
  hipStream_t cs = overlapping(e) ? e->comm_stream : s;
  if (cs != s) {
    HIPTRY(ev_record(e, e->ev_piece, s));
    HIPTRY(ev_wait(e, cs, e->ev_piece));
  }
  const int rc = g_rccl.AllReduce(f, f, 1, kNcclFloat32, kNcclSum, e->comm, cs);
  if (rc != kNcclSuccess) return fail("ncclAllReduce (status word): %s", g_rccl.GetErrorString(rc));
  if (cs != s) {
    HIPTRY(ev_record(e, e->ev_status, cs));
    e->status_pending = true;
  }
  e->status_collectives += 1;
  return 0;
}
int status_finish(PlbEngine* e, float* loss, hipStream_t s) {
  if (e->status_pending) {
    HIPTRY(ev_wait(e, s, e->ev_status));
    e->status_pending = false;
  }
  e->last_loss = loss;
  TRY(plb_launch_step_status(e->at<unsigned int>(e->o_lnerr), loss, e->host_err_dev, e->comm ? status_float(e) : nullptr, s));
  return 0;
}

extern "C" int plb_comm_unique_id(uint8_t id[PLB_COMM_ID_BYTES]) {
  if (!id) return fail("plb_comm_unique_id: null argument");
  if (const char* err = rccl_load()) return fail("plb_comm_unique_id: %s", err);
  RcclId u;
  memset(&u, 0, sizeof(u));
  const int rc = g_rccl.GetUniqueId(&u);
  if (rc != kNcclSuccess) return fail("ncclGetUniqueId: %s", g_rccl.GetErrorString(rc));
  static_assert(sizeof(u) == PLB_COMM_ID_BYTES, "unique id size");
  memcpy(id, &u, sizeof(u));
  return 0;
}

extern "C" int plb_comm_destroy(PlbEngine* e) {
  if (!e) return fail("plb_comm_destroy: null engine");
  if (e->comm_stream) (void)hipStreamSynchronize(e->comm_stream);
  if (e->comm && g_rccl.ok) (void)g_rccl.CommDestroy(e->comm);
  e->comm = nullptr; e->comm_rank = 0; e->comm_world = 1; e->comm_pending = false;
  if (e->ev_piece) { (void)hipEventDestroy(e->ev_piece); e->ev_piece = nullptr; }
  if (e->ev_comm_done) { (void)hipEventDestroy(e->ev_comm_done); e->ev_comm_done = nullptr; }
  if (e->ev_status) { (void)hipEventDestroy(e->ev_status); e->ev_status = nullptr; }
  e->status_pending = false;
  if (e->comm_stream) { (void)hipStreamDestroy(e->comm_stream); e->comm_stream = nullptr; }
  return 0;
}

extern "C" int plb_comm_init(PlbEngine* e, const uint8_t id[PLB_COMM_ID_BYTES], int32_t rank, int32_t world) {
  if (!e || !id) return fail("plb_comm_init: null argument");
  if (!e->grads) return fail("plb_comm_init: bind the gradient buffer first (plb_bind)");
  if (world < 1 || rank < 0 || rank >= world) return fail("plb_comm_init: rank %d of %d", rank, world);
  if (e->comm) return fail("plb_comm_init: the engine already has a communicator");
  if (const char* err = rccl_load()) return fail("plb_comm_init: %s", err);
  int lo = 0, hi = 0;
  (void)hipDeviceGetStreamPriorityRange(&lo, &hi);
  HIPTRY(hipStreamCreateWithPriority(&e->comm_stream, hipStreamNonBlocking, hi));
  HIPTRY(hipEventCreateWithFlags(&e->ev_piece, kStreamOrderEvent));
  HIPTRY(hipEventCreateWithFlags(&e->ev_comm_done, kStreamOrderEvent));
  HIPTRY(hipEventCreateWithFlags(&e->ev_status, kStreamOrderEvent));
  RcclId u;
  memcpy(&u, id, sizeof(u));
  const int rc = g_rccl.CommInitRank(&e->comm, world, u, rank);
  if (rc != kNcclSuccess) {
    e->comm = nullptr;
    (void)plb_comm_destroy(e);
    return fail("ncclCommInitRank(rank %d of %d): %s", rank, world, g_rccl.GetErrorString(rc));
  }
  e->comm_rank = rank; e->comm_world = world;
  return 0;
// ... 141 lines not shown
```

plbert_amd/csrc/engine_internal.h:

```cpp
#pragma once
#include <hip/hip_runtime.h>
#include <stdint.h>
#include <stdio.h>
#include <stdlib.h>
#include <string.h>

#include <array>
#include <map>
#include <string>
#include <vector>

#include "../../include/plbert.h"
#include "plbert_kernels.h"

#pragma GCC visibility push(hidden)

int fail(const char* fmt, ...);

static const unsigned kStreamOrderEvent = hipEventDisableTiming | hipEventReleaseToDevice;

inline int64_t rup(int64_t x, int64_t m) { return (x + m - 1) / m * m; }

#define TRY(x)                                                                    \
  do {                                                                            \
    int rc_ = (x);                                                                \
    if (rc_) return fail("%s failed (rc %d) at %s:%d", #x, rc_, __FILE__, __LINE__); \
  } while (0)
#define HIPTRY(x)                                                                                   \
  do {                                                                                              \
    hipError_t e_ = (x);                                                                            \
    if (e_ != hipSuccess) return fail("%s: %s at %s:%d", #x, hipGetErrorString(e_), __FILE__, __LINE__); \
  } while (0)
#define HB_R(stream, ptr, bytes, what) do { if (e->hb.on) e->hb.access(hb_idx(e, stream), (ptr), (size_t)(bytes), false, what); } while (0)
#define HB_W(stream, ptr, bytes, what) do { if (e->hb.on) e->hb.access(hb_idx(e, stream), (ptr), (size_t)(bytes), true, what); } while (0)

typedef void* RcclComm;

struct HbAudit {
  enum { MAIN = 0, SIDE = 1, COMM = 2, NS = 3 };
  typedef std::array<uint64_t, NS> VC;
  struct Acc { const char* what; uintptr_t a, b; int st; uint64_t tick; bool wr; };
  bool on = false;
  int break_wait = -1;
  int waits = 0;
  VC vc[NS] = {{0, 0, 0}, {0, 0, 0}, {0, 0, 0}};
  std::map<hipEvent_t, VC> ev;
  std::vector<Acc> log;
  int64_t checks = 0;
  int violations = 0;
  std::string first;
  static const char* name(int st) { return st == MAIN ? "main" : st == SIDE ? "side" : "comm"; }
  void record(hipEvent_t e, int st) { vc[st][st] += 1; ev[e] = vc[st]; }
  void wait(int st, hipEvent_t e);
  void access(int st, const void* p, size_t bytes, bool wr, const char* what);
  void new_call() { log.clear(); waits = 0; }
};

struct PlbEngine {
  PlbConfig c;
  int64_t poff[PLB_NPARAM], psize[PLB_NPARAM], ptotal, ptrain;
  int E, H, I, L, NH, V, P, NP, NT;
  int64_t Tcap;
  int64_t NMcap;
  int NTp = 0;
  bool infer = false;
  int qkvcol_rows = 0;
  int64_t slab2_floats;
  int64_t slab_floats;
  int64_t ws_bytes;
  int ln_blocks, emb_blocks;
  int part_rows = 0;
  int ln_fuse = 3;
  int64_t lnx_bytes = 0;
  bool gelu_dstash_on = true;
  bool fp8_tn = true;
  int f8n = 0;
  bool packed_dual = false;
  bool packed_fp8 = false;
  int64_t o_wbf, o_wqkvT, o_wdT, o_w1T, o_w2T, o_wpT, o_winT;
  int64_t o_e, o_x, o_qkv, o_ctx, o_pre1, o_a, o_u, o_g, o_pre2;
  int64_t o_lse, o_delta, o_mean1, o_rstd1, o_mean2, o_rstd2;
  int64_t o_dqkv, o_dpre1, o_du, o_dpre2;
  int64_t o_dy0, o_dy1, o_da, o_dctx, o_de;
  int64_t o_hm, o_logm, o_dlog, o_dhm, o_rows, o_tgt, o_w, o_lrows;
  int64_t o_slab, o_part1, o_part2, o_parte, o_scratch, o_dxe, o_ducol, o_slab2, o_scratch2, o_qkvcol = 0;
  int64_t o_lnx = 0, o_lnerr = 0;
  int64_t o_bt = 0, o_wtT = 0, o_tdl = 0, o_tlrows = 0, o_tscr = 0, o_tgrad = 0, o_tloss = 0;
  int64_t o_tpmax = 0, o_tpsum = 0, o_ttl = 0, o_tlse = 0, o_tw = 0, o_ttgt = 0, o_tcolp = 0;
  int64_t o_x8 = 0, o_a8 = 0, o_g8 = 0, o_c8 = 0, o_dp8 = 0, o_du8 = 0, o_dp18 = 0, o_dq8 = 0;
  int64_t o_wq8 = 0, o_wd8 = 0, o_w18 = 0, o_w28 = 0, o_w2T8 = 0, o_w1T8 = 0, o_wqT8 = 0, o_wdT8 = 0;
  int64_t o_f8amax = 0, o_f8scale = 0, o_f8deq = 0, o_f8stats = 0;
  bool fp8_on = false, fp8_ready = false, fp8_bwd_ready = false, fp8_wstale = true;
  bool u_is_derivative = false;
  bool tn8_call = false;
  int part_rows_used = 0;
  int pruned_rows = 0;
  int64_t last_app_rows[2] = {0, 0};
  int64_t last_exec_rows[2] = {0, 0};
  bool tok_grads_live = false;
  bool head_grads_live = true;
  bool tok_pad_zeroed = false;
  int tok_steps = 0;
  float* accum = nullptr;
  bool grads_fresh = false;
  bool win_open = false;
  const char* win_closed_by = "no FIRST add has opened one";
  bool win_head = false, win_tok = false;
  bool win_reduced = false;
  const float* norm_src = nullptr;
  int norm_nparts = 0;
  bool norm_reduced = false;
  bool stash_live = false;
  const char* stash_dead_by = "no plb_encode has run on this engine";
  int stash_B = 0, stash_S = 0;
  int64_t stash_rows = 0, stash_used = 0;
  const int32_t* stash_row_start = nullptr;
  RcclComm comm = nullptr;
  int comm_rank = 0, comm_world = 1;
  hipStream_t comm_stream = nullptr;
  hipEvent_t ev_piece = nullptr, ev_comm_done = nullptr;
  bool overlap = true;
  bool comm_pending = false;
  bool grads_reduced = false;
  int64_t piece_floats = 0;
  int32_t piece_count = 0;
  hipEvent_t ev_status = nullptr;
  bool status_pending = false;
  int32_t status_collectives = 0;
  float* last_loss = nullptr;
  HbAudit hb;
  struct PieceTrace { int64_t a, b; hipEvent_t released, done; };
  bool trace_on = false;
  std::vector<PieceTrace> trace;
  std::vector<hipEvent_t> trace_pool;
  hipEvent_t tr_call0 = nullptr, tr_tail0 = nullptr, tr_tail1 = nullptr;
  bool tr_tail_valid = false;
  hipStream_t side = nullptr;
  hipEvent_t ev_fork = nullptr, ev_join = nullptr;
  unsigned int* host_err = nullptr;
  unsigned int* host_err_dev = nullptr;
  float *params = nullptr, *grads = nullptr, *m = nullptr, *v = nullptr;
  char* ws = nullptr;

  template <typename T>
  T* at(int64_t off) const { return reinterpret_cast<T*>(ws + off); }
  bf16_t* wbf(int which) const { return at<bf16_t>(o_wbf) + poff[which]; }
  float* par(int which) const { return params + poff[which]; }
  float* grd(int which) const { return grads + poff[which]; }
};

enum { F8_X = 0, F8_A, F8_G, F8_C, F8_DP, F8_DU, F8_DP1, F8_DQ, F8_NSITE };
enum { F8_AMAX_WORDS = 64 * 16 };
enum { F8W_QKV = 0, F8W_D, F8W_1, F8W_2, F8W_2T, F8W_1T, F8W_QKVT, F8W_DT, F8W_N };

struct Rows {
  const int32_t* row_start;
  int T; int64_t Tp;
};

struct F8Site {
  float* scale = nullptr;
  float* amax = nullptr;
  float* deq = nullptr;
  F8Site() = default;
  F8Site(const PlbEngine* e, int kind, int l);
};
struct F8Weight {
  const uint8_t* img;
  const float* deq;
  F8Weight(const PlbEngine* e, int w);
};

struct F8Op { const uint8_t* A8; const uint8_t* B8; const float* deq_a; const float* deq_b; int a_bf8; };

struct Slots {
  bf16_t *x, *y;
  bf16_t *qkv, *ctx, *pre1, *a, *u, *g, *pre2;
  float *mean1, *rstd1, *mean2, *rstd2, *lse;
  uint8_t *x8, *x8n, *c8, *a8, *g8;
  bf16_t *dqkv, *dpre1, *du, *dpre2;
  uint8_t *dp8, *du8, *dp18, *dq8;
  float *part1, *part2, *qkvcol, *ducol;
};

struct LnSlot { const float* gamma; const float* beta; const bf16_t* pre; float* mean; float* rstd; float* partials; };

struct Prune { const int32_t* rows; int n; int Mc; };

struct Bwd {
  const int32_t* lengths;
  const int32_t* row_start;
  int B, S, T;
  int64_t Tp;
  bool f8, calib;
  bool fuse_b;
  int prows;
  int du_rows;
  hipStream_t s;
};

enum { kPieceHead = 0, kPieceQkvW, kPieceFfnW, kPieceSmall, kPieceFfnoW = kPieceSmall + 5, kPieceDenseW, kNPieces };

int hb_idx(const PlbEngine* e, hipStream_t s);
hipError_t ev_record(PlbEngine* e, hipEvent_t ev, hipStream_t s);
hipError_t ev_wait(PlbEngine* e, hipStream_t s, hipEvent_t ev);
int reduce_piece(PlbEngine* e, int64_t a, int64_t b, hipStream_t after);
bool overlapping(const PlbEngine* e);
int pieces_done(PlbEngine* e);
int64_t piece_begin(const PlbEngine* e, int i);
int64_t piece_end(const PlbEngine* e, int i);
int reduce_pieces(PlbEngine* e, int from, int to, hipStream_t after);
int status_exchange(PlbEngine* e, hipStream_t s);
int status_finish(PlbEngine* e, float* loss, hipStream_t s);
int f8_site(const PlbEngine* e, int site, int l);
float* f8_deq(const PlbEngine* e, int i);
int fp8_quantize_weights(PlbEngine* e, hipStream_t s, bool exact = true);
int fp8_update_scales(PlbEngine* e, hipStream_t s);
bool f8_call(const PlbEngine* e, int64_t Tp, bool train);
bool tn8_ok(const PlbEngine* e, int64_t Mtot);
PlbGemmNT nt_desc(const bf16_t* A, const bf16_t* B, int64_t M, int N, int K);
int qkvcol_rows(int B, int S);
Slots slots(const PlbEngine* e, int64_t Tp, int B, int S, int l, bool stash, int prows = 0, int du_rows = 0);
bool prune_enabled();
int run_encoder(PlbEngine* e, const int64_t* ids, const int32_t* lengths, int B, int S, const Rows& rw, bool stash,
                bf16_t** xout, hipStream_t s, const Prune* pr = nullptr);
int tn_splits(int64_t Mtot, int N, int K, int* rows_per_split);
int weight_grad(PlbEngine* e, const bf16_t* A, int lda, int Ncols, const bf16_t* Bm, int ldb, int64_t Mtot, int N,
                int K, float* out, hipStream_t s, bool side_slab = false);
int weight_grad8(PlbEngine* e, const uint8_t* A8, const uint8_t* B8, int64_t Mtot, int N, int K, int site_a, int site_b,
                 float* out, hipStream_t s);
int encoder_bwd(PlbEngine* e, const Prune* pr, const int32_t* lengths, int B, int S, const Rows& rw, bf16_t** dy,
                int* du_rows, hipStream_t s);
void drop_stash(PlbEngine* e, const char* by);
int sync_transposes(PlbEngine* e, hipStream_t s, bool exact_fp8 = true);
void end_accum_window(PlbEngine* e, const char* by);

#pragma GCC visibility pop
```

plbert_amd/csrc/engine_layers.cpp:

```cpp
#include "engine_internal.h"

static bool tn_big(int64_t Mtot, int Ncols, int K) { return Ncols % 256 == 0 && K % 256 == 0 && Mtot >= 8192; }
static bool tn_fill_chip() {
  static const bool v = [] { const char* e = getenv("PLBERT_TN_SPLITS"); return !(e && !strcmp(e, "xcd")); }();
  return v;
}
static int tn_cus() {
  static const int v = [] {
    const char* e = getenv("PLBERT_TN_CUS");
    const int n = e ? atoi(e) : 256;
    return (n >= 64 && n <= 256) ? n : 256;
  }();
  return v;
}
int tn_splits(int64_t Mtot, int N, int K, int* rows_per_split) {
  const bool big = tn_big(Mtot, N, K);
  const int tiles = big ? (N / 256) * (K / 256) : ((N + 127) / 128) * ((K + 127) / 128);
  int splits = 768 / tiles;
  if (big) {
    int s = 32 / tiles;
    if (s < 1) s = 1;
    splits = tiles >= 256 ? 1 : (tn_fill_chip() ? (tn_cus() / tiles > 0 ? tn_cus() / tiles : 1) : 8 * s);
  }
  const int64_t maxs = Mtot / 64;
  if (splits > maxs) splits = (int)maxs;
  if (splits < 1) splits = 1;
  int64_t rps = rup((Mtot + splits - 1) / splits, 64);
  splits = (int)((Mtot + rps - 1) / rps);
  *rows_per_split = (int)rps;
  return splits;
}

PlbGemmNT nt_desc(const bf16_t* A, const bf16_t* B, int64_t M, int N, int K) {
  PlbGemmNT g;
  memset(&g, 0, sizeof(g));
  g.A = A; g.lda = K; g.B = B; g.ldb = K; g.M = (int)M; g.N = N; g.K = K; g.Mstore = (int)M;
  return g;
}

static F8Op f8_op(const uint8_t* a8, const F8Site& a, const F8Weight& w, int a_bf8) { return F8Op{a8, w.img, a.deq, w.deq, a_bf8}; }
static PlbGemmNT f8_operands(const PlbGemmNT* g, const F8Op* f8) {
  PlbGemmNT q = *g;
  q.A = reinterpret_cast<const bf16_t*>(f8->A8); q.B = reinterpret_cast<const bf16_t*>(f8->B8);
  q.deq_a = f8->deq_a; q.deq_b = f8->deq_b;
  return q;
}
static int gemm_nt_any(PlbGemmNT* g, int act, const F8Op* f8, hipStream_t s) {
  if (!f8) return plb_launch_gemm_nt(g, act, 0, s);
  PlbGemmNT q = f8_operands(g, f8);
  return plb_launch_gemm_nt_fp8(&q, act, f8->a_bf8, s);
}
static int gemm_nt_ln_any(PlbGemmNT* g, int mode, const F8Op* f8, hipStream_t s) {
  if (!f8) return plb_launch_gemm_nt_ln(g, mode, s);
  PlbGemmNT q = f8_operands(g, f8);
  return plb_launch_gemm_nt_fp8_ln(&q, mode, f8->a_bf8, s);
}
static int gemm_nt_gelud_any(PlbGemmNT* g, int backward, const F8Op* f8, hipStream_t s) {
  if (!f8) return plb_launch_gemm_nt_gelud(g, backward, s);
  PlbGemmNT q = f8_operands(g, f8);
  return plb_launch_gemm_nt_fp8_gelud(&q, backward, f8->a_bf8, s);
}
static void f8_out(PlbGemmNT* g, uint8_t* img, int ld, const F8Site& q, int bf8) {
  g->C8 = img; g->ldc8 = ld; g->q_scale = q.scale; g->q_amax = q.amax; g->c8_bf8 = bf8;
}

int qkvcol_rows(int B, int S) { return B * ((S + 127) / 128) * 4; }
Slots slots(const PlbEngine* e, int64_t Tp, int B, int S, int l, bool stash, int prows, int du_rows) {
  const int64_t H = e->H, I = e->I, sl = stash ? l : 0;
  auto bf = [&](int64_t off, int64_t width) { return e->at<bf16_t>(off) + sl * Tp * width; };
  auto u8 = [&](int64_t off, int64_t width) { return e->at<uint8_t>(off) + sl * Tp * width; };
  auto f32 = [&](int64_t off, int64_t per_layer) { return e->at<float>(off) + sl * per_layer; };
  Slots v;
  memset(&v, 0, sizeof(v));
  v.x = e->at<bf16_t>(e->o_x) + (int64_t)(stash ? l : l & 1) * Tp * H;
  v.y = e->at<bf16_t>(e->o_x) + (int64_t)(stash ? l + 1 : (l + 1) & 1) * Tp * H;
  v.qkv = bf(e->o_qkv, 3 * H); v.ctx = bf(e->o_ctx, H); v.pre1 = bf(e->o_pre1, H); v.a = bf(e->o_a, H);
  v.u = bf(e->o_u, I); v.g = bf(e->o_g, I); v.pre2 = bf(e->o_pre2, H);
  v.mean1 = f32(e->o_mean1, Tp); v.rstd1 = f32(e->o_rstd1, Tp); v.mean2 = f32(e->o_mean2, Tp); v.rstd2 = f32(e->o_rstd2, Tp);
  v.lse = f32(e->o_lse, (int64_t)B * e->NH * S);
  v.x8 = u8(e->o_x8, H); v.c8 = u8(e->o_c8, H); v.a8 = u8(e->o_a8, H); v.g8 = u8(e->o_g8, I);
  v.x8n = e->at<uint8_t>(e->o_x8) + (stash ? l + 1 : 0) * Tp * H;
  if (stash) {
    v.dqkv = bf(e->o_dqkv, 3 * H); v.dpre1 = bf(e->o_dpre1, H); v.du = bf(e->o_du, I); v.dpre2 = bf(e->o_dpre2, H);
    v.dp8 = u8(e->o_dp8, H); v.du8 = u8(e->o_du8, I); v.dp18 = u8(e->o_dp18, H); v.dq8 = u8(e->o_dq8, 3 * H);
    v.part1 = f32(e->o_part1, (int64_t)prows * 3 * H); v.part2 = f32(e->o_part2, (int64_t)prows * 3 * H);
    v.qkvcol = f32(e->o_qkvcol, (int64_t)qkvcol_rows(B, S) * 3 * H); v.ducol = f32(e->o_ducol, (int64_t)du_rows * I);
  }
  return v;
}

static bool ln_fusable(const PlbEngine* e, int64_t Tp, int bit) {
  const int H = e->H;
  return (e->ln_fuse & bit) && Tp % 1024 == 0 && (H % 384 == 0 ? H / 384 : H % 256 == 0 ? H / 256 : 99) <= 4;
}
static bool gelu_dstash(PlbEngine* e, int64_t Tp, bool f8_call) {
  e->u_is_derivative = e->gelu_dstash_on && (f8_call ? Tp % 128 == 0 : Tp % 256 == 0) && e->I % 256 == 0;
  return e->u_is_derivative;
}
static void ln_fields(const PlbEngine* e, PlbGemmNT* g, const float* gamma, const float* beta, float* mean, float* rstd) {
  g->ln_gamma = gamma; g->ln_beta = beta; g->ln_mean = mean; g->ln_rstd = rstd; g->ln_eps = e->c.layer_norm_eps;
  g->ln_xchg = e->at<unsigned long long>(e->o_lnx); g->ln_err = e->at<unsigned int>(e->o_lnerr);
}
static LnSlot ln1_slot(const PlbEngine* e, const Slots& v) {
  return LnSlot{e->par(PLB_LN1_W), e->par(PLB_LN1_B), v.pre1, v.mean1, v.rstd1, v.part1};
}
static LnSlot ln2_slot(const PlbEngine* e, const Slots& v) {
  return LnSlot{e->par(PLB_LN2_W), e->par(PLB_LN2_B), v.pre2, v.mean2, v.rstd2, v.part2};
}
static int gemm_ln_fwd(PlbEngine* e, PlbGemmNT* g, const F8Op* f8, bool fused, const LnSlot& ln, bf16_t* y, int T,
                       uint8_t* y8, const F8Site& q, hipStream_t s) {
  const int H = e->H;
  if (fused) {
    g->C2 = y; g->ldc2 = H;
    ln_fields(e, g, ln.gamma, ln.beta, ln.mean, ln.rstd);
    if (y8) f8_out(g, y8, H, q, 0);
    TRY(gemm_nt_ln_any(g, 5, f8, s));
    return 0;
  }
  TRY(gemm_nt_any(g, 0, f8, s));
  PlbLayerNorm p;
  memset(&p, 0, sizeof(p));
  p.x = g->C; p.ldx = H; p.gamma = ln.gamma; p.beta = ln.beta; p.eps = e->c.layer_norm_eps;
  p.y = y; p.ldy = H; p.T = T; p.H = H; p.mean = ln.mean; p.rstd = ln.rstd;
  if (y8) { p.out8 = y8; p.ld8 = H; p.q_scale = q.scale; p.q_amax = q.amax; }
  TRY(plb_launch_ln_fwd(&p, s));
  return 0;
}
static int ln_bwd(PlbEngine* e, const LnSlot& ln, int nblocks, const bf16_t* dy, bf16_t* dx, int T, int Tzero, uint8_t* dx8,
                  const F8Site& q, hipStream_t s) {
  const int H = e->H;
  PlbLayerNorm p;
  memset(&p, 0, sizeof(p));
  p.x = ln.pre; p.ldx = H; p.gamma = ln.gamma; p.T = T; p.H = H; p.Tzero = Tzero; p.mean = ln.mean; p.rstd = ln.rstd;
  p.dy = dy; p.lddy = H; p.dx = dx; p.lddx = H; p.partials = ln.partials; p.nblocks = nblocks;
  if (dx8) { p.out8 = dx8; p.ld8 = H; p.q_scale = q.scale; p.q_amax = q.amax; }
  TRY(plb_launch_ln_bwd(&p, s));
  return 0;
}
static int gemm_ln_bwd(PlbEngine* e, PlbGemmNT* g, const F8Op* f8, bool fused, const LnSlot& ln, int nblocks, bf16_t* dx, int T,
                       int Tzero, uint8_t* dx8, const F8Site& q, hipStream_t s) {
  if (fused) {
    g->C = dx; g->aux = ln.pre; g->ldaux = e->H; g->colpart = ln.partials;
    ln_fields(e, g, ln.gamma, nullptr, ln.mean, ln.rstd);
    if (dx8) f8_out(g, dx8, e->H, q, 1);
    TRY(gemm_nt_ln_any(g, 6, f8, s));
    return 0;
  }
  TRY(gemm_nt_any(g, 0, f8, s));
  return ln_bwd(e, ln, nblocks, g->C, dx, T, Tzero, dx8, q, s);
}

static int g_prune_last = -1;
extern "C" void plb_set_prune_last(int on) { g_prune_last = on < 0 ? -1 : (on ? 1 : 0); }
bool prune_enabled() {
  static const bool v = [] { const char* e = getenv("PLBERT_PRUNE_LAST"); return !(e && !strcmp(e, "0")); }();
  return g_prune_last < 0 ? v : g_prune_last != 0;
}
static int last_application_fwd_pruned(PlbEngine* e, const Prune* pr, bool stash, bool calib, bool tn8, const Slots& sl,
                                       const bf16_t* ctx_att, hipStream_t s) {
  const int H = e->H, I = e->I, L = e->L, Mc = pr->Mc, n = pr->n;
  const F8Site sA(e, F8_A, L - 1), sG(e, F8_G, L - 1), sC(e, F8_C, L - 1);
  bf16_t* ctxc = stash ? sl.ctx : sl.pre1;
  bf16_t* xc = stash ? e->at<bf16_t>(e->o_da) : sl.a;
  bf16_t* pre1c = stash ? sl.pre1 : sl.ctx;
  bf16_t* ac = stash ? sl.a : sl.pre1;
  TRY(plb_launch_gather_rows(ctx_att, H, pr->rows, n, Mc, H, ctxc, H, s));
  TRY(plb_launch_gather_rows(sl.x, H, pr->rows, n, Mc, H, xc, H, s));
  PlbGemmNT g = nt_desc(ctxc, e->wbf(PLB_DENSE_W), Mc, H, H);
  g.bias = e->par(PLB_DENSE_B); g.res = xc; g.ldr = H; g.C = pre1c; g.ldc = H;
  const LnSlot ln1 = {e->par(PLB_LN1_W), e->par(PLB_LN1_B), pre1c, sl.mean1, sl.rstd1, nullptr};
  if (gemm_ln_fwd(e, &g, nullptr, false, ln1, ac, Mc, nullptr, F8Site(), s)) return 1;
  if (calib) TRY(plb_launch_amax(ac, 1, (size_t)n, H, H, sA.amax, s));
  g = nt_desc(ac, e->wbf(PLB_FFN_W), Mc, I, H);
  g.bias = e->par(PLB_FFN_B); g.C = sl.u; g.ldc = I; g.C2 = sl.g; g.ldc2 = I;
  TRY(plb_launch_gemm_nt(&g, 1, 0, s));
  if (calib) TRY(plb_launch_amax(sl.g, 1, (size_t)n, I, I, sG.amax, s));
  g = nt_desc(sl.g, e->wbf(PLB_FFNO_W), Mc, H, I);
  g.bias = e->par(PLB_FFNO_B); g.res = ac; g.ldr = H; g.C = sl.pre2; g.ldc = H;
  if (gemm_ln_fwd(e, &g, nullptr, false, ln2_slot(e, sl), e->at<bf16_t>(e->o_hm), Mc, nullptr, F8Site(), s)) return 1;
  if (tn8) {
    const void* src[3] = {ctxc, ac, sl.g}; const int fl[3] = {1, 1, 1};
    const size_t nel[3] = {(size_t)Mc * H, (size_t)Mc * H, (size_t)Mc * I};
    const float* sc[3] = {sC.scale, sA.scale, sG.scale};
    uint8_t* dst[3] = {sl.c8, sl.a8, sl.g8};
    float* am[3] = {sC.amax, sA.amax, sG.amax};
    TRY(plb_launch_quantize_multi(3, src, fl, nel, sc, dst, am, s));
  }
  return 0;
}

int run_encoder(PlbEngine* e, const int64_t* ids, const int32_t* lengths, int B, int S, const Rows& rw, bool stash,
                       bf16_t** xout, hipStream_t s, const Prune* pr) {
  const int E = e->E, H = e->H, I = e->I, L = e->L;
  const int T = rw.T;
  const int64_t Tp = rw.Tp;
  const bool f8 = f8_call(e, Tp, stash);
  const bool calib = e->fp8_on && !f8;
  const int T8 = (f8 && rw.row_start) ? (int)Tp : T;
  if (e->fp8_on && e->fp8_wstale) TRY(fp8_quantize_weights(e, s));
  PlbEmbed em;
  memset(&em, 0, sizeof(em));
  em.ids = ids; em.T = T; em.S = S; em.E = E; em.V = e->V;
  em.word = e->par(PLB_WORD_EMB); em.pos = e->par(PLB_POS_EMB); em.type0 = e->par(PLB_TYPE_EMB);
  em.gamma = e->par(PLB_EMB_LN_W); em.beta = e->par(PLB_EMB_LN_B); em.eps = e->c.layer_norm_eps;
  em.out = e->at<bf16_t>(e->o_e); em.ldo = E;
  if (rw.row_start) {
    em.row_start = rw.row_start; em.lengths = lengths; em.B = B; em.T = (int)Tp;
    em.fill_slots = e->fp8_on;
  }
  TRY(plb_launch_embed_fwd(&em, s));

  const Slots first = slots(e, Tp, B, S, 0, stash);
  PlbGemmNT g = nt_desc(em.out, e->wbf(PLB_MAP_W), Tp, H, E);
  g.bias = e->par(PLB_MAP_B); g.C = first.x; g.ldc = H;
  TRY(plb_launch_gemm_nt(&g, 0, 0, s));
  if (f8) {
    const F8Site sX(e, F8_X, 0);
    const void* src1[1] = {first.x}; const int bf1[1] = {1}; const size_t n1[1] = {(size_t)T8 * H};
    const float* sc1[1] = {sX.scale}; uint8_t* dst1[1] = {first.x8}; float* am1[1] = {sX.amax};
    TRY(plb_launch_quantize_multi(1, src1, bf1, n1, sc1, dst1, am1, s));
  }
  const bool fuse_f = ln_fusable(e, Tp, 1);
  const bool dstash = gelu_dstash(e, Tp, f8);
  if (stash) e->tn8_call = f8 && e->fp8_tn && dstash && tn8_ok(e, (int64_t)L * Tp);
  const bool tn8 = stash && e->tn8_call;

  for (int l = 0; l < L; ++l) {
    const Slots sl = slots(e, Tp, B, S, l, stash);
    const F8Site sX(e, F8_X, l), sA(e, F8_A, l), sG(e, F8_G, l), sC(e, F8_C, l);
    if (calib) TRY(plb_launch_amax(sl.x, 1, (size_t)T, H, H, sX.amax, s));
    g = nt_desc(sl.x, e->wbf(PLB_Q_W), Tp, 3 * H, H);
    g.bias = e->par(PLB_Q_B); g.C = sl.qkv; g.ldc = 3 * H;
    const F8Op oq = f8_op(sl.x8, sX, F8Weight(e, F8W_QKV), 0);
    TRY(gemm_nt_any(&g, 0, f8 ? &oq : nullptr, s));
    PlbAttn at;
    memset(&at, 0, sizeof(at));
    at.qkv = sl.qkv; at.ldqkv = 3 * H; at.lengths = lengths; at.B = B; at.S = S; at.NH = e->NH; at.H = H;
    at.row_start = rw.row_start;
    const bool pruned_layer = pr != nullptr && l == L - 1;
    bf16_t* const ctx_att = (pruned_layer && stash) ? e->at<bf16_t>(e->o_dy1) : sl.ctx;
    at.scale = 0.125f; at.ctx = ctx_att; at.ldctx = H; at.lse = sl.lse;
    if (f8 && !pruned_layer) { at.ctx8 = sl.c8; at.ldctx8 = H; at.ctx_scale = sC.scale; at.ctx_amax = sC.amax; }
    if (rw.row_start && e->fp8_on && S % 128) {
      HIPTRY(hipMemsetAsync(ctx_att, 0, (size_t)T * H * 2, s));
      if (at.ctx8) HIPTRY(hipMemsetAsync(sl.c8, 0, (size_t)T * H, s));
    }
    TRY(plb_launch_attn_fwd(&at, s));
    if (rw.row_start && Tp > T) {
      HIPTRY(hipMemsetAsync(ctx_att + (int64_t)T * H, 0, (size_t)(Tp - T) * H * 2, s));
      if (at.ctx8) HIPTRY(hipMemsetAsync(sl.c8 + (int64_t)T * H, 0, (size_t)(Tp - T) * H, s));
    }
    if (calib) TRY(plb_launch_amax(ctx_att, 1, (size_t)T, H, H, sC.amax, s));
    if (pruned_layer) {
      if (last_application_fwd_pruned(e, pr, stash, calib, tn8, sl, ctx_att, s)) return 1;
      *xout = e->at<bf16_t>(e->o_hm);
      break;
    }
    g = nt_desc(sl.ctx, e->wbf(PLB_DENSE_W), Tp, H, H);
    g.bias = e->par(PLB_DENSE_B); g.res = sl.x; g.ldr = H; g.C = sl.pre1; g.ldc = H;
    const F8Op od = f8_op(sl.c8, sC, F8Weight(e, F8W_D), 0);
    if (gemm_ln_fwd(e, &g, f8 ? &od : nullptr, fuse_f, ln1_slot(e, sl), sl.a, T8, f8 ? sl.a8 : nullptr, sA, s)) return 1;
    if (calib) TRY(plb_launch_amax(sl.a, 1, (size_t)T, H, H, sA.amax, s));
    g = nt_desc(sl.a, e->wbf(PLB_FFN_W), Tp, I, H);
    g.bias = e->par(PLB_FFN_B); g.C = sl.u; g.ldc = I; g.C2 = sl.g; g.ldc2 = I;
    if (f8) f8_out(&g, sl.g8, I, sG, 0);
    const F8Op o1 = f8_op(sl.a8, sA, F8Weight(e, F8W_1), 0);
    if (dstash) {
      if (tn8) { g.C2 = nullptr; g.ldc2 = 0; }
      TRY(gemm_nt_gelud_any(&g, 0, f8 ? &o1 : nullptr, s));
    } else {
      TRY(gemm_nt_any(&g, 1, f8 ? &o1 : nullptr, s));
    }
    if (calib) TRY(plb_launch_amax(sl.g, 1, (size_t)T, I, I, sG.amax, s));
    g = nt_desc(sl.g, e->wbf(PLB_FFNO_W), Tp, H, I);
    g.bias = e->par(PLB_FFNO_B); g.res = sl.a; g.ldr = H; g.C = sl.pre2; g.ldc = H;
    const F8Op o2 = f8_op(sl.g8, sG, F8Weight(e, F8W_2), 0);
    const bool next8 = f8 && l + 1 < L;
    if (gemm_ln_fwd(e, &g, f8 ? &o2 : nullptr, fuse_f, ln2_slot(e, sl), sl.y, T8, next8 ? sl.x8n : nullptr,
                    next8 ? F8Site(e, F8_X, l + 1) : F8Site(), s))
      return 1;
    *xout = sl.y;
  }
  return 0;
}

int weight_grad(PlbEngine* e, const bf16_t* A, int lda, int Ncols, const bf16_t* Bm, int ldb, int64_t Mtot, int N,
                       int K, float* out, hipStream_t s, bool side_slab) {
  PlbGemmTN t;
  memset(&t, 0, sizeof(t));
  t.A = A; t.lda = lda; t.Ncols = Ncols; t.B = Bm; t.ldb = ldb; t.Mtot = (int)Mtot; t.N = N; t.K = K;
  t.splits = tn_splits(Mtot, N, K, &t.rows_per_split);
  const bool direct = t.splits == 1 && N == Ncols;
  if (!direct && (int64_t)t.splits * N * K > (side_slab ? e->slab2_floats : e->slab_floats)) return fail("weight_grad: slab too small");
  t.slab = direct ? out : e->at<float>(side_slab ? e->o_slab2 : e->o_slab);
  if (N == Ncols && tn_big(Mtot, Ncols, K)) {
    const int tok = plb_prof_begin(PLB_K_GEMM_TN, s, 2.0 * (double)Mtot * N * K, 0.0);
    TRY(plb_launch_gemm_tn_big(&t, s));
    plb_prof_end(tok, s);
  } else {
    TRY(plb_launch_gemm_tn(&t, s));
  }
  if (!direct) TRY(plb_launch_reduce_slabs(t.slab, t.splits, (size_t)N * K, out, 0, s));
  return 0;
}

int weight_grad8(PlbEngine* e, const uint8_t* A8, const uint8_t* B8, int64_t Mtot, int N, int K, int site_a, int site_b,
                        float* out, hipStream_t s) {
  PlbGemmTN t;
  memset(&t, 0, sizeof(t));
  t.A = reinterpret_cast<const bf16_t*>(A8); t.lda = N; t.Ncols = N; t.B = reinterpret_cast<const bf16_t*>(B8); t.ldb = K;
  t.Mtot = (int)Mtot; t.N = N; t.K = K;
  t.splits = tn_splits(Mtot, N, K, &t.rows_per_split);
  t.rows_per_split = (int)rup(t.rows_per_split, 128);
  t.splits = (int)((Mtot + t.rows_per_split - 1) / t.rows_per_split);
  if ((int64_t)t.splits * N * K > e->slab_floats) return fail("weight_grad8: slab too small");
  t.slab = e->at<float>(e->o_slab);
  t.deq_a = f8_deq(e, f8_site(e, site_a, 0)); t.deq_b = f8_deq(e, f8_site(e, site_b, 0));
  const int tok = plb_prof_begin(PLB_K_GEMM_TN_FP8, s, 2.0 * (double)Mtot * N * K, 0.0);
  TRY(plb_launch_gemm_tn_fp8(&t, s));
  plb_prof_end(tok, s);
  TRY(plb_launch_reduce_slabs(t.slab, t.splits, (size_t)N * K, out, 0, s));
  return 0;
}

static int post_attention_bwd(PlbEngine* e, const Bwd& c, int l, const Slots& sl, const bf16_t* dy) {
  const int H = e->H, I = e->I, T = c.T, Tp = (int)c.Tp;
  hipStream_t s = c.s;
  const F8Site sDP(e, F8_DP, l), sDU(e, F8_DU, l), sDP1(e, F8_DP1, l);
  if (l == e->L - 1 && ln_bwd(e, ln2_slot(e, sl), c.prows, dy, sl.dpre2, T, Tp, c.f8 ? sl.dp8 : nullptr, sDP, s)) return 1;
  if (c.calib) TRY(plb_launch_amax(sl.dpre2, 1, (size_t)T, H, H, sDP.amax, s));
  PlbGemmNT g = nt_desc(sl.dpre2, e->at<bf16_t>(e->o_w2T), Tp, I, H);
  g.aux = sl.u; g.ldaux = I; g.C = sl.du; g.ldc = I;
  if (c.du_rows > 0) g.colpart = sl.ducol;
  if (c.f8) f8_out(&g, sl.du8, I, sDU, 1);
  const F8Op ou = f8_op(sl.dp8, sDP, F8Weight(e, F8W_2T), 1);
  if (e->u_is_derivative) {
    if (e->tn8_call) g.C = nullptr;
    TRY(gemm_nt_gelud_any(&g, 1, c.f8 ? &ou : nullptr, s));
  } else {
    TRY(gemm_nt_any(&g, 2, c.f8 ? &ou : nullptr, s));
  }
  if (c.calib) TRY(plb_launch_amax(sl.du, 1, (size_t)T, I, I, sDU.amax, s));
  g = nt_desc(sl.du, e->at<bf16_t>(e->o_w1T), Tp, H, I);
  g.res = sl.dpre2; g.ldr = H; g.C = e->at<bf16_t>(e->o_da); g.ldc = H;
  const F8Op oa = f8_op(sl.du8, sDU, F8Weight(e, F8W_1T), 1);
  if (gemm_ln_bwd(e, &g, c.f8 ? &oa : nullptr, c.fuse_b, ln1_slot(e, sl), c.prows, sl.dpre1, T, Tp, c.f8 ? sl.dp18 : nullptr,
                  sDP1, s))
    return 1;
  if (c.calib) TRY(plb_launch_amax(sl.dpre1, 1, (size_t)T, H, H, sDP1.amax, s));
  g = nt_desc(sl.dpre1, e->at<bf16_t>(e->o_wdT), Tp, H, H);
  g.C = e->at<bf16_t>(e->o_dctx); g.ldc = H;
  const F8Op oc = f8_op(sl.dp18, sDP1, F8Weight(e, F8W_DT), 1);
  TRY(gemm_nt_any(&g, 0, c.f8 ? &oc : nullptr, s));
  return 0;
}

static int last_application_bwd_pruned(PlbEngine* e, const Bwd& c, const Slots& sl, const Prune* pr) {
  const int H = e->H, I = e->I, L = e->L, Mc = pr->Mc, n = pr->n;
  hipStream_t s = c.s;
  const F8Site sDP(e, F8_DP, L - 1), sDU(e, F8_DU, L - 1), sDP1(e, F8_DP1, L - 1);
  bf16_t* const dac = e->at<bf16_t>(e->o_da);
  bf16_t* const dctxc = e->at<bf16_t>(e->o_dy0);
  bf16_t* const dctx = e->at<bf16_t>(e->o_dctx);
  if (ln_bwd(e, ln2_slot(e, sl), c.prows, e->at<bf16_t>(e->o_dhm), sl.dpre2, Mc, Mc, nullptr, F8Site(), s)) return 1;
  if (c.calib) TRY(plb_launch_amax(sl.dpre2, 1, (size_t)n, H, H, sDP.amax, s));
  PlbGemmNT g = nt_desc(sl.dpre2, e->at<bf16_t>(e->o_w2T), Mc, I, H);
  g.aux = sl.u; g.ldaux = I; g.C = sl.du; g.ldc = I;
  TRY(plb_launch_gemm_nt(&g, 2, 0, s));
  if (c.calib) TRY(plb_launch_amax(sl.du, 1, (size_t)n, I, I, sDU.amax, s));
  if (c.du_rows > 0) {
    TRY(plb_launch_colsum(sl.du, 1, (size_t)Mc, I, I, sl.ducol, I, 0, e->at<float>(e->o_scratch), 16, s));
    if (c.du_rows > 1) HIPTRY(hipMemsetAsync(sl.ducol + I, 0, (size_t)(c.du_rows - 1) * I * 4, s));
  }
  g = nt_desc(sl.du, e->at<bf16_t>(e->o_w1T), Mc, H, I);
  g.res = sl.dpre2; g.ldr = H; g.C = dac; g.ldc = H;
  if (gemm_ln_bwd(e, &g, nullptr, false, ln1_slot(e, sl), c.prows, sl.dpre1, Mc, Mc, nullptr, F8Site(), s)) return 1;
  if (c.calib) TRY(plb_launch_amax(sl.dpre1, 1, (size_t)n, H, H, sDP1.amax, s));
  if (e->tn8_call) {
    const void* src[3] = {sl.dpre2, sl.du, sl.dpre1}; const int fl[3] = {3, 3, 3};
    const size_t nel[3] = {(size_t)Mc * H, (size_t)Mc * I, (size_t)Mc * H};
    const float* sc[3] = {sDP.scale, sDU.scale, sDP1.scale};
    uint8_t* dst[3] = {sl.dp8, sl.du8, sl.dp18};
    float* am[3] = {sDP.amax, sDU.amax, sDP1.amax};
    TRY(plb_launch_quantize_multi(3, src, fl, nel, sc, dst, am, s));
  }
  g = nt_desc(sl.dpre1, e->at<bf16_t>(e->o_wdT), Mc, H, H);
  g.C = dctxc; g.ldc = H;
  TRY(plb_launch_gemm_nt(&g, 0, 0, s));
  HIPTRY(hipMemsetAsync(dctx, 0, (size_t)c.Tp * H * 2, s));
  TRY(plb_launch_scatter_rows(dctxc, H, pr->rows, n, H, dctx, H, s));
  HIPTRY(hipMemsetAsync(dac, 0, (size_t)c.Tp * H * 2, s));
  TRY(plb_launch_scatter_rows(sl.dpre1, H, pr->rows, n, H, dac, H, s));
  return 0;
}

static int attention_bwd_dx(PlbEngine* e, const Bwd& c, int l, const Slots& sl, bf16_t* ctx, const bf16_t* res,
                            bf16_t* dx) {
  const int H = e->H, T = c.T;
  hipStream_t s = c.s;
  const F8Site sDQ(e, F8_DQ, l);
  PlbAttn at;
  memset(&at, 0, sizeof(at));
  at.qkv = sl.qkv; at.ldqkv = 3 * H; at.lengths = c.lengths; at.B = c.B; at.S = c.S; at.NH = e->NH; at.H = H; at.scale = 0.125f;
  at.row_start = c.row_start;
  at.ctx = ctx; at.ldctx = H; at.lse = sl.lse;
  at.dctx = e->at<bf16_t>(e->o_dctx); at.lddctx = H; at.delta = e->at<float>(e->o_delta); at.dqkv = sl.dqkv; at.lddqkv = 3 * H;
  at.colpart = sl.qkvcol; at.colpart_accumulate = 0;
  if (c.f8) {
    at.dqkv8 = sl.dq8; at.lddqkv8 = 3 * H; at.dqkv_scale = sDQ.scale; at.dqkv_amax = sDQ.amax;
    if (e->tn8_call) at.dqkv = nullptr;
  }
  if (c.row_start && c.S % 128 && at.dqkv) HIPTRY(hipMemsetAsync(sl.dqkv, 0, (size_t)T * 3 * H * 2, s));
  if (c.row_start && c.S % 128 && at.dqkv8) HIPTRY(hipMemsetAsync(sl.dq8, 0, (size_t)T * 3 * H, s));
  TRY(plb_launch_attn_bwd(&at, s));
  if (c.Tp > T) {
    if (at.dqkv) HIPTRY(hipMemsetAsync(sl.dqkv + (int64_t)T * 3 * H, 0, (size_t)(c.Tp - T) * 3 * H * 2, s));
    if (c.f8) HIPTRY(hipMemsetAsync(sl.dq8 + (int64_t)T * 3 * H, 0, (size_t)(c.Tp - T) * 3 * H, s));
  }
  if (c.calib) TRY(plb_launch_amax(sl.dqkv, 1, (size_t)T, 3 * H, 3 * H, sDQ.amax, s));
  PlbGemmNT g = nt_desc(sl.dqkv, e->at<bf16_t>(e->o_wqkvT), c.Tp, H, 3 * H);
  g.res = res; g.ldr = H; g.C = dx; g.ldc = H;
  const F8Op ox = f8_op(sl.dq8, sDQ, F8Weight(e, F8W_QKVT), 1);
  if (l == 0) {
    TRY(gemm_nt_any(&g, 0, c.f8 ? &ox : nullptr, s));
    return 0;
  }
  const Slots below = slots(e, c.Tp, c.B, c.S, l - 1, true, c.prows, c.du_rows);
  return gemm_ln_bwd(e, &g, c.f8 ? &ox : nullptr, c.fuse_b, ln2_slot(e, below), c.prows, below.dpre2, T, (int)c.Tp,
                     c.f8 ? below.dp8 : nullptr, F8Site(e, F8_DP, l - 1), s);
}

int encoder_bwd(PlbEngine* e, const Prune* pr, const int32_t* lengths, int B, int S, const Rows& rw, bf16_t** dy,
                       int* du_rows, hipStream_t s) {
  const int I = e->I, L = e->L;
  Bwd c;
  c.lengths = lengths; c.row_start = rw.row_start; c.B = B; c.S = S; c.T = rw.T; c.Tp = rw.Tp; c.s = s;
  const int Tp = (int)c.Tp;
  c.f8 = f8_call(e, Tp, true);
  c.calib = e->fp8_on && !c.f8;
  c.du_rows = e->u_is_derivative ? (c.f8 ? 2 * (Tp / plb_gemm_nt_fp8_gelud_tile_rows(Tp)) : 2 * (Tp / 256))
                                 : (c.f8 ? 2 * (Tp / 128) : plb_gemm_nt_colpart_rows(Tp, I, e->H));
  c.fuse_b = ln_fusable(e, Tp, 2);
  c.prows = c.fuse_b ? 2 * Tp / 128 : e->ln_blocks;
  e->part_rows_used = c.prows;
  bf16_t* dx = e->at<bf16_t>(e->o_dy1);
  for (int l = L - 1; l >= 0; --l) {
    const Slots sl = slots(e, c.Tp, B, S, l, true, c.prows, c.du_rows);
    if (pr && l == L - 1) {
      if (last_application_bwd_pruned(e, c, sl, pr)) return 1;
      if (attention_bwd_dx(e, c, l, sl, e->at<bf16_t>(e->o_dy1), e->at<bf16_t>(e->o_da), dx)) return 1;
    } else {
      if (post_attention_bwd(e, c, l, sl, *dy)) return 1;
      if (attention_bwd_dx(e, c, l, sl, sl.ctx, sl.dpre1, dx)) return 1;
    }
    bf16_t* tmp = *dy; *dy = dx; dx = tmp;
// ... 5 lines not shown
```

plbert_amd/csrc/gemm_big.hip:

```cpp
#include "gemm_nt_pipeline.h"

namespace {

template <int V, bool PF>
int launch_big(const PlbGemmNT* p, int act, int out_f32, hipStream_t stream) {
  constexpr int TM = (V == 2 ? 2 : 1) * 128, TN = (V == 3 ? 3 : 2) * 128;
  if (p->M % TM || p->N % TN || p->K % 64 || p->M <= 0 || p->N <= 0 || p->K <= 0) return 1;
  dim3 grid((p->M / TM) * (p->N / TN)), block(512);
  if (out_f32) {
    if (act != 0) return 1;
    hipLaunchKernelGGL((gemm_nt_big_kernel<V, 0, true, PF>), grid, block, 0, stream, *p);
  } else if (act == 0) {
    if (p->colpart) hipLaunchKernelGGL((gemm_nt_big_kernel<V, 0, false, PF>), grid, block, 0, stream, *p);
    else hipLaunchKernelGGL((gemm_nt_big_kernel<V, 0, false, PF, false, false, true>), grid, block, 0, stream, *p);
  } else if (act == 1) {
    hipLaunchKernelGGL((gemm_nt_big_kernel<V, 1, false, PF>), grid, block, 0, stream, *p);
  } else if (act == 2) {
    hipLaunchKernelGGL((gemm_nt_big_kernel<V, 2, false, PF>), grid, block, 0, stream, *p);
  } else if ((act == 3 || act == 4) && TN == 256) {
    if (!p->ce_tgt || p->ce_cols < 1 || p->ce_cols > p->N) return 1;
    if (act == 3) {
      if (!p->ce_pmax || !p->ce_psum || !p->ce_tlogit) return 1;
      hipLaunchKernelGGL((gemm_nt_big_kernel<V, 3, false, PF>), grid, block, 0, stream, *p);
    } else {
      if (!p->ce_lse || !p->ce_w || !p->C) return 1;
      hipLaunchKernelGGL((gemm_nt_big_kernel<V, 4, false, PF>), grid, block, 0, stream, *p);
    }
  } else {
    return 1;
  }
  return hipGetLastError() == hipSuccess ? 0 : 2;
}

DEVI int tn_g(int row) { return ((row >> 1) & 1) | (((row >> 3) & 1) << 1); }

__global__ __launch_bounds__(512) __attribute__((amdgpu_num_vgpr(224))) void gemm_tn_big_kernel(PlbGemmTN p) {
  __shared__ __attribute__((aligned(16))) bf16_t smem[2 * 4 * HT];
  const int tid = threadIdx.x, lane = tid & 63;
  const int uw = __builtin_amdgcn_readfirstlane(tid >> 6);
  const int wm = uw >> 2, wn = uw & 3;
  const int nbk = p.K >> 8;
  const int tiles = (p.Ncols >> 8) * nbk;
  const int logical = xcd_remap(blockIdx.x, gridDim.x);
  const int split = logical / tiles, tile = logical % tiles;
  const int bn = tile / nbk, bk = tile % nbk;
  const int t_begin = split * p.rows_per_split;
  int t_end = t_begin + p.rows_per_split;
  if (t_end > p.Mtot) t_end = p.Mtot;
  const int nk = (t_end - t_begin) >> 6;

  const int i0 = 2 * uw, i1 = 2 * uw + 1;
  const int r0 = (i0 & 7) * 8 + (lane >> 3), r1 = (i1 & 7) * 8 + (lane >> 3);
  const int sc0 = (((lane & 7) ^ (2 * tn_g(r0))) * 8) + (i0 >> 3) * 64;
  const int sc1 = (((lane & 7) ^ (2 * tn_g(r1))) * 8) + (i1 >> 3) * 64;
  const int dst0 = (i0 >> 3) * 4096 + (i0 & 7) * 8 * 64, dst1 = (i1 >> 3) * 4096 + (i1 & 7) * 8 * 64;
  const int fg = lane >> 4, li = lane & 15, q4 = li >> 2, p4 = li & 3;
  const int gsw = 2 * (((q4 >> 1) & 1) | ((fg & 1) << 1));
  const int rowbase = (8 * fg + q4) * 64 + (p4 & 1) * 4;
  int aoff[4], boff[2];
#pragma unroll
  for (int mi = 0; mi < 4; ++mi) aoff[mi] = wm * 4096 + rowbase + (((2 * mi + (p4 >> 1)) ^ gsw) << 3);
#pragma unroll
  for (int ni = 0; ni < 2; ++ni)
    boff[ni] = (wn >> 1) * 4096 + rowbase + (((4 * (wn & 1) + 2 * ni + (p4 >> 1)) ^ gsw) << 3);
  const unsigned lds0 = (unsigned)(size_t)&smem[0];
#define FRAG(r, kk) (bf16x8{r[2 * (kk)][0], r[2 * (kk)][1], r[2 * (kk)][2], r[2 * (kk)][3],              \
                            r[2 * (kk) + 1][0], r[2 * (kk) + 1][1], r[2 * (kk) + 1][2], r[2 * (kk) + 1][3]})

  f32x4 acc[2][4][2][2];
#pragma unroll
  for (int a = 0; a < 2; ++a)
#pragma unroll
    for (int b = 0; b < 4; ++b)
#pragma unroll
      for (int c = 0; c < 2; ++c)
#pragma unroll
        for (int d = 0; d < 2; ++d) acc[a][b][c][d] = f32x4{0.f, 0.f, 0.f, 0.f};
#ifndef TN_DBG
#define TN_DBG 0
#endif
#if TN_DBG
  unsigned long long tnw_ = 0, tnq_ = 0;
#define TN_W0() tnq_ = __builtin_readcyclecounter()
#define TN_W1() tnw_ += __builtin_readcyclecounter() - tnq_
#else
#define TN_W0()
#define TN_W1()
#endif
#define LANDED(more)                                                      \
  do {                                                                    \
    TN_W0();                                                              \
    if (more) asm volatile("s_waitcnt vmcnt(6)" ::: "memory");            \
    else asm volatile("s_waitcnt vmcnt(0)" ::: "memory");                 \
    TN_W1();                                                              \
  } while (0)

  s16x4 ra1[4][4], rb2[2][2][4];
#define TR1(dst, addr, OFF) dst = lds_read_tr16_addr((addr) + (OFF))
#define RD4(dst, ad_, o_)   \
  do { TR1(dst[0], ad_, (o_)); TR1(dst[1], ad_, (o_) + 512); TR1(dst[2], ad_, (o_) + 4096); TR1(dst[3], ad_, (o_) + 4608); PIN(); } while (0)
#define RA4(buf, h, mi) RD4(ra1[mi], abase[buf][mi], (h) * 16384)
#define RB4(bb, buf, h, ni) RD4(rb2[bb][ni], bbase[buf][ni], (2 + (h)) * 16384)
#define SA_(h, kt) ((const char*)p.A + ((size_t)(t_begin + (kt) * 64) * p.lda + bn * 256 + (h) * 128) * 2)
#define SB_(h, kt) ((const char*)p.B + ((size_t)(t_begin + (kt) * 64) * p.ldb + bk * 256 + (h) * 128) * 2)
#define STG_A(buf, h, kt)                                                                     \
  do {                                                                                        \
    const char* sb_ = SA_(h, kt);                                                             \
    DMA16(sb_, vA0, ldsb + (((buf) * 4 + (h)) * HT + dst0) * 2);                              \
    DMA16(sb_, vA1, ldsb + (((buf) * 4 + (h)) * HT + dst1) * 2);                              \
    PIN();                                                                                    \
  } while (0)
#define STG_B(buf, h, kt)                                                                     \
  do {                                                                                        \
    const char* sb_ = SB_(h, kt);                                                             \
    DMA16(sb_, vB0, ldsb + (((buf) * 4 + 2 + (h)) * HT + dst0) * 2);                          \
    DMA16(sb_, vB1, ldsb + (((buf) * 4 + 2 + (h)) * HT + dst1) * 2);                          \
    PIN();                                                                                    \
  } while (0)
  const uint32_t vA0 = (uint32_t)(r0 * p.lda + sc0) * 2, vA1 = (uint32_t)(r1 * p.lda + sc1) * 2;
  const uint32_t vB0 = (uint32_t)(r0 * p.ldb + sc0) * 2, vB1 = (uint32_t)(r1 * p.ldb + sc1) * 2;
  const uint32_t ldsb = LDS_ADDR(&smem[0]);
  unsigned abase[2][4], bbase[2][2];
#pragma unroll
  for (int bf = 0; bf < 2; ++bf) {
#pragma unroll
    for (int mi = 0; mi < 4; ++mi) abase[bf][mi] = lds0 + 65536u * bf + 2u * aoff[mi];
#pragma unroll
    for (int ni = 0; ni < 2; ++ni) bbase[bf][ni] = lds0 + 65536u * bf + 2u * boff[ni];
  }
#define PO_(pc) ((pc) == 0 ? 0 : (pc) == 1 ? 512 : (pc) == 2 ? 4096 : 4608)
#define RA1(buf, h, mi, pc) do { TR1(ra1[mi][pc], abase[buf][mi], (h) * 16384 + PO_(pc)); PIN(); } while (0)
#define RB1(bb, buf, h, ni, pc) do { TR1(rb2[bb][ni][pc], bbase[buf][ni], (2 + (h)) * 16384 + PO_(pc)); PIN(); } while (0)
#define MF1(mh, nh, bb, j)                                                                                      \
  do {                                                                                                          \
    acc[mh][(j) >> 2][nh][(j) & 1] = __builtin_amdgcn_mfma_f32_16x16x32_bf16(                                   \
        FRAG(rb2[bb][(j) & 1], ((j) >> 1) & 1), FRAG(ra1[(j) >> 2], ((j) >> 1) & 1), acc[mh][(j) >> 2][nh][(j) & 1], 0, 0, 0); \
    PIN();                                                                                                      \
  } while (0)
#define PH1(mh, nh, bb, s0, s1, s2, s3, s4, s5, s6, s7, s8, s9, s10, s11, s12, s13, s14, s15)                    \
  do {                                                                                                          \
    BARRIER(); PIN();                                                                                           \
    MF1(mh, nh, bb, 0); s0; MF1(mh, nh, bb, 1); s1; MF1(mh, nh, bb, 2); s2; MF1(mh, nh, bb, 3); s3;             \
    MF1(mh, nh, bb, 4); s4; MF1(mh, nh, bb, 5); s5; MF1(mh, nh, bb, 6); s6; MF1(mh, nh, bb, 7); s7;             \
    MF1(mh, nh, bb, 8); s8; MF1(mh, nh, bb, 9); s9; MF1(mh, nh, bb, 10); s10; MF1(mh, nh, bb, 11); s11;         \
    MF1(mh, nh, bb, 12); s12; MF1(mh, nh, bb, 13); s13; MF1(mh, nh, bb, 14); s14; MF1(mh, nh, bb, 15); s15;     \
  } while (0)
#define NOP_ (void)0
#define TWO(x, y) do { x; y; } while (0)
#define TN_STEP(bb)                                                                                             \
  do {                                                                                                          \
    constexpr int b = (bb);  \
    const bool n1 = t + 1 < nk, n2 = t + 2 < nk;                                                                \
                                  \
    PH1(0, 0, bb, RA1(b, 0, 3, 0), RA1(b, 0, 3, 1), RA1(b, 0, 3, 2), RA1(b, 0, 3, 3),                           \
        RB1(1 - bb, b, 1, 0, 0), RB1(1 - bb, b, 1, 0, 1), RB1(1 - bb, b, 1, 0, 2), RB1(1 - bb, b, 1, 0, 3),     \
        RB1(1 - bb, b, 1, 1, 0), RB1(1 - bb, b, 1, 1, 1), RB1(1 - bb, b, 1, 1, 2), RB1(1 - bb, b, 1, 1, 3),     \
        TWO(if (n1) STG_A(b ^ 1, 1, t + 1), NOP_), NOP_, NOP_, NOP_);                                           \
                              \
    PH1(0, 1, 1 - bb, NOP_, NOP_, NOP_, NOP_, RA1(b, 1, 0, 0), RA1(b, 1, 0, 1), RA1(b, 1, 0, 2), RA1(b, 1, 0, 3), \
        RA1(b, 1, 1, 0), RA1(b, 1, 1, 1), RA1(b, 1, 1, 2), RA1(b, 1, 1, 3),                                     \
        RA1(b, 1, 2, 0), RA1(b, 1, 2, 1), RA1(b, 1, 2, 2), TWO(RA1(b, 1, 2, 3), TWO(if (n2) STG_A(b, 0, t + 2), NOP_))); \
                                                                             \
    PH1(1, 1, 1 - bb, RA1(b, 1, 3, 0), RA1(b, 1, 3, 1), RA1(b, 1, 3, 2), RA1(b, 1, 3, 3),                       \
        TWO(if (n2) STG_B(b, 0, t + 2), NOP_), NOP_, NOP_, NOP_, TWO(if (n2) STG_B(b, 1, t + 2), NOP_), NOP_, NOP_, NOP_, \
        NOP_, NOP_, NOP_, NOP_);                                                                                \
    LANDED(n2);                                                                                                 \
                    \
    PH1(1, 0, bb, RB1(1 - bb, b ^ 1, 0, 0, 0), RB1(1 - bb, b ^ 1, 0, 0, 1), RB1(1 - bb, b ^ 1, 0, 0, 2),        \
        RB1(1 - bb, b ^ 1, 0, 0, 3),                                                                            \
        TWO(RA1(b ^ 1, 0, 0, 0), RB1(1 - bb, b ^ 1, 0, 1, 0)), TWO(RA1(b ^ 1, 0, 0, 1), RB1(1 - bb, b ^ 1, 0, 1, 1)), \
        TWO(RA1(b ^ 1, 0, 0, 2), RB1(1 - bb, b ^ 1, 0, 1, 2)), TWO(RA1(b ^ 1, 0, 0, 3), RB1(1 - bb, b ^ 1, 0, 1, 3)), \
        RA1(b ^ 1, 0, 1, 0), RA1(b ^ 1, 0, 1, 1), RA1(b ^ 1, 0, 1, 2), RA1(b ^ 1, 0, 1, 3),                     \
        RA1(b ^ 1, 0, 2, 0), RA1(b ^ 1, 0, 2, 1), RA1(b ^ 1, 0, 2, 2), RA1(b ^ 1, 0, 2, 3));                    \
  } while (0)
  if (nk > 0) {
    STG_A(0, 0, 0); STG_B(0, 0, 0); STG_B(0, 1, 0); STG_A(0, 1, 0);
    if (nk > 1) { STG_A(1, 0, 1); STG_B(1, 0, 1); STG_B(1, 1, 1); }
    LANDED(nk > 1);
  }
  BARRIER();
#if TN_DBG
  tnw_ = 0;
  const unsigned long long tn_c0 = __builtin_readcyclecounter(), tn_r0 = __builtin_amdgcn_s_memrealtime();
#endif
  if (nk > 0) {
    RA4(0, 0, 0); RA4(0, 0, 1); RA4(0, 0, 2); RB4(0, 0, 0, 0); RB4(0, 0, 0, 1);
    int t = 0;
    while (true) {
      TN_STEP(0);
      if (++t >= nk) break;
      TN_STEP(1);
      if (++t >= nk) break;
    }
    BARRIER();
  }
#if TN_DBG
  if ((blockIdx.x == 17 || blockIdx.x == 130) && lane == 0 && (uw == 0 || uw == 5)) {
    const unsigned long long dc = __builtin_readcyclecounter() - tn_c0, dr = __builtin_amdgcn_s_memrealtime() - tn_r0;
    printf("TN blk %d wave %d: %d K-tiles, %.3f us per K-tile, %.0f MHz, vmcnt wait %.1f %% of the loop\n", (int)blockIdx.x, uw, nk,
           (double)dr / 100.0 / nk, (double)dc / ((double)dr / 100.0), 100.0 * (double)tnw_ / (double)dc);
  }
#endif
#undef TN_STEP
#undef TWO
#undef NOP_
#undef PH1
#undef MF1
#undef RA1
#undef RB1
#undef PO_
#undef RA4
#undef RB4
#undef RD4
#undef TR1
#undef STG_A
#undef STG_B
#undef SA_
#undef SB_
#undef FRAG
#undef LANDED

  float* out = p.slab + (size_t)split * p.N * p.K;
  int lane_e = (int)__builtin_amdgcn_mbcnt_hi(~0u, __builtin_amdgcn_mbcnt_lo(~0u, 0u));
  asm volatile("" : "+v"(lane_e));
  const int li_e = lane_e & 15, fg_e = lane_e >> 4;
#pragma unroll
  for (int mh = 0; mh < 2; ++mh)
#pragma unroll
    for (int mi = 0; mi < 4; ++mi) {
      const int n = bn * 256 + mh * 128 + wm * 64 + mi * 16 + li_e;
      if (n >= p.N) continue;
#pragma unroll
      for (int nh = 0; nh < 2; ++nh)
#pragma unroll
        for (int ni = 0; ni < 2; ++ni) {
          const int k0 = bk * 256 + nh * 128 + wn * 32 + ni * 16 + 4 * fg_e;
          const f32x4 v = acc[mh][mi][nh][ni];
          *(float4*)(out + (size_t)n * p.K + k0) = make_float4(v[0], v[1], v[2], v[3]);
        }
    }
}

}

extern "C" int plb_launch_gemm_tn_big(const PlbGemmTN* p, hipStream_t stream) {
  if (p->Ncols % 256 || p->K % 256 || p->rows_per_split % 64 || p->Mtot % 64 || p->splits <= 0) return 1;
  if ((long)p->splits * p->rows_per_split < p->Mtot) return 1;
  dim3 grid((p->Ncols / 256) * (p->K / 256) * p->splits), block(512);
  hipLaunchKernelGGL(gemm_tn_big_kernel, grid, block, 0, stream, *p);
  return hipGetLastError() == hipSuccess ? 0 : 2;
}

static int g_nt_prefetch = -1;
extern "C" void plb_set_gemm_nt_prefetch(int on) { g_nt_prefetch = on; }

extern "C" int plb_launch_gemm_nt_big(const PlbGemmNT* p, int tile, int act, int out_f32, hipStream_t stream) {
  const bool pf = g_nt_prefetch < 0 ? (tile != 256 || act != 0) : (g_nt_prefetch != 0);
  if (pf)
    return tile == 384 ? launch_big<3, true>(p, act, out_f32, stream)
           : tile == 1256 ? launch_big<1, true>(p, act, out_f32, stream) : launch_big<2, true>(p, act, out_f32, stream);
  return tile == 384 ? launch_big<3, false>(p, act, out_f32, stream)
         : tile == 1256 ? launch_big<1, false>(p, act, out_f32, stream) : launch_big<2, false>(p, act, out_f32, stream);
}
```

plbert_amd/csrc/plbert_kernels.h:

```cpp
#pragma once
#include <hip/hip_runtime.h>
#include <stdint.h>

typedef uint16_t bf16_t;

extern "C" {

enum PlbKernelClass {
  PLB_K_GEMM_NT = 0, PLB_K_GEMM_NT_GELU, PLB_K_GEMM_NT_GELUBWD, PLB_K_GEMM_NT_F32, PLB_K_GEMM_TN,
  PLB_K_ATTN_FWD, PLB_K_ATTN_BWD_DQ, PLB_K_ATTN_BWD_DKV, PLB_K_LN_FWD, PLB_K_LN_BWD, PLB_K_EMBED_FWD,
  PLB_K_EMBED_BWD, PLB_K_COLSUM, PLB_K_REDUCE, PLB_K_ROWS, PLB_K_CE, PLB_K_ADAMW, PLB_K_CAST, PLB_K_TOKEN_CE, PLB_K_GEMM_NT_CE, PLB_K_GEMM_NT_SMALL, PLB_K_FP8, PLB_K_ATTN_BWD,
  PLB_K_GEMM_NT_FP8, PLB_K_GEMM_NT_GELU_FP8, PLB_K_GEMM_NT_GELUBWD_FP8,
  PLB_K_GEMM_NT_LNFWD, PLB_K_GEMM_NT_LNBWD,
  PLB_K_GEMM_NT_LNFWD_FP8, PLB_K_GEMM_NT_LNBWD_FP8, PLB_K_GEMM_TN_FP8,
  PLB_K_NCLASS
};
int plb_prof_begin(int cls, hipStream_t s, double flops, double bytes);
void plb_prof_end(int tok, hipStream_t s);

typedef struct {
  const bf16_t* A; int lda;
  const bf16_t* B; int ldb;
  int M, N, K;
  int Mstore;
  const float* bias;
  const bf16_t* res; int ldr;
  const bf16_t* aux; int ldaux;
  bf16_t* C; int ldc;
  bf16_t* C2; int ldc2;
  float* Cf; int ldcf;
  float* colpart;
  int ce_cols;
  const int64_t* ce_tgt;
  float* ce_pmax; float* ce_psum;
  float* ce_tlogit;
  const float* ce_lse;
  const float* ce_w;
  const float* deq_a; const float* deq_b;
  uint8_t* C8; int ldc8;
  const float* q_scale;
  float* q_amax;
  int c8_bf8;
  const float* ln_gamma; const float* ln_beta;
  float* ln_mean; float* ln_rstd;
  float ln_eps;
  unsigned long long* ln_xchg;
  unsigned int* ln_err;
  int ln_fault;
} PlbGemmNT;
int plb_launch_gemm_nt_ln(const PlbGemmNT* p, int mode, hipStream_t stream);
int plb_launch_gemm_nt_gelud(const PlbGemmNT* p, int backward, hipStream_t stream);
int plb_launch_gemm_nt_fp8(const PlbGemmNT* p, int act, int a_bf8, hipStream_t stream);
int plb_launch_gemm_nt_fp8_ln(const PlbGemmNT* p, int mode, int a_bf8, hipStream_t stream);
int plb_launch_gemm_nt_fp8_gelud(const PlbGemmNT* p, int backward, int a_bf8, hipStream_t stream);
int plb_gemm_nt_fp8_gelud_tile_rows(int M);
int plb_ln_fault_take(void);
int plb_launch_gemm_nt(const PlbGemmNT* p, int act, int out_f32, hipStream_t stream);
int plb_launch_gemm_nt_big(const PlbGemmNT* p, int tile, int act, int out_f32, hipStream_t stream);
int plb_gemm_nt_colpart_rows(int M, int N, int K);
void plb_set_gemm_nt_tile(int tile);
void plb_set_gemm_nt_prefetch(int on);

typedef struct {
  const bf16_t* A; int lda; int Ncols;
  const bf16_t* B; int ldb;
  int Mtot, N, K;
  int rows_per_split, splits;
  float* slab;
  const float* deq_a; const float* deq_b;
} PlbGemmTN;
int plb_launch_gemm_tn(const PlbGemmTN* p, hipStream_t stream);
int plb_launch_gemm_tn_fp8(const PlbGemmTN* p, hipStream_t stream);
int plb_launch_gemm_tn_big(const PlbGemmTN* p, hipStream_t stream);

int plb_launch_reduce_slabs(const float* slab, int splits, size_t n, float* out, int accumulate, hipStream_t stream);

typedef struct {
  const int64_t* ids; int T, S, E, V;
  const float *word, *pos, *type0, *gamma, *beta;
  float eps;
  bf16_t* out; int ldo;
  const bf16_t* dout; int lddo;
  float* dx;
  float *dword, *dpos;
  float* partials;
  int nblocks;
  const int32_t* row_start; const int32_t* lengths; int B; int fill_slots;
} PlbEmbed;
int plb_launch_embed_fwd(const PlbEmbed* p, hipStream_t stream);
int plb_launch_embed_bwd(const PlbEmbed* p, hipStream_t stream);
int plb_launch_embed_scatter(const PlbEmbed* p, int P, hipStream_t stream);

typedef struct {
  const bf16_t* x; int ldx;
  const float *gamma, *beta; float eps;
  bf16_t* y; int ldy;
  float *mean, *rstd;
  int T, H;
  int Tzero;
  const bf16_t* dy; int lddy;
  bf16_t* dx; int lddx;
  float* partials; int nblocks;
  int accumulate;
  uint8_t* out8; int ld8; const float* q_scale; float* q_amax;
} PlbLayerNorm;
int plb_launch_amax(const void* x, int is_bf16, size_t rows, int cols, int ld, float* amax, hipStream_t stream);
int plb_launch_fp8_scales(float* amax, float* scale, float* deq, int n, float fmax, int group, hipStream_t stream);
int plb_launch_fp8_scales2(float* amax, float* scale, float* deq, int n, float fmax, int group, int n2, float fmax2,
                           float* stats, int hist_from, hipStream_t stream);
int plb_launch_quantize(const void* x, int is_bf16, size_t rows, int cols, int ld, const float* scale, uint8_t* out, int ldo,
                        int bf8, hipStream_t stream);
int plb_launch_quantize_multi(int n, const void* const* src, const int* is_bf16, const size_t* elements,
                              const float* const* scale, uint8_t* const* dst, float* const* amax, hipStream_t stream);
int plb_launch_ln_fwd(const PlbLayerNorm* p, hipStream_t stream);
int plb_launch_ln_bwd(const PlbLayerNorm* p, hipStream_t stream);

int plb_launch_colsum(const void* X, int is_bf16, size_t R, int N, int ld, float* out, int Nout, int accumulate,
                      float* scratch, int nsplit, hipStream_t stream);

int plb_launch_copy_cols(const float* scratch, int nsplit, int N, int col0, int Nout, float* out, hipStream_t stream);

int plb_launch_pooler(const float* hidden, int B, int S, int H, const float* W, const float* bias, float* pooled,
                      hipStream_t stream);

typedef struct {
  const bf16_t* qkv; int ldqkv;
  const int32_t* lengths;
  int B, S, NH, H;
  float scale;
  bf16_t* ctx; int ldctx;
  float* lse;
  const bf16_t* dctx; int lddctx;
  float* delta;
  bf16_t* dqkv; int lddqkv;
  float* colpart;
  int colpart_accumulate;
  uint8_t* ctx8; int ldctx8; const float* ctx_scale; float* ctx_amax;
  uint8_t* dqkv8; int lddqkv8; const float* dqkv_scale; float* dqkv_amax;
  const int32_t* qoff; const bf16_t* q; int ldq; int nq_total; bf16_t* dq; int lddq; uint8_t* dq8; int lddq8;
  const int32_t* row_start;
} PlbAttn;
int plb_launch_attn_fwd(const PlbAttn* p, hipStream_t stream);
int plb_launch_attn_bwd(const PlbAttn* p, hipStream_t stream);
int plb_launch_attn_bwd_fused(const PlbAttn* p, hipStream_t stream);
void plb_debug_skip_piece(int index);
void plb_debug_ln_fault(int mode, int launches);
void plb_set_attn_bwd_fused(int on);

int plb_launch_gather_rows(const bf16_t* src, int lds_, const int32_t* rows, int n, int npad, int H, bf16_t* dst,
                           int ldd, hipStream_t stream);
int plb_launch_scatter_rows(const bf16_t* src, int lds_, const int32_t* rows, int n, int H, bf16_t* dst, int ldd,
                            hipStream_t stream);
int plb_launch_ce_prepare(const int32_t* offsets, const int32_t* flat, const int64_t* labels, int B, int S,
                          int32_t* rows, int32_t* tgt, float* w, hipStream_t stream);
int plb_launch_ce_prepare_packed(const int32_t* offsets, const int32_t* flat, const int64_t* labels, int B, int S,
                                 const int32_t* row_start, int32_t* rows, int32_t* tgt, float* w, hipStream_t stream);
int plb_launch_unpack_rows(const void* src, int src_is_bf16, int lds_, const int32_t* row_start, const int32_t* lengths,
                           int B, int S, int C, float* dst, hipStream_t stream);
int plb_launch_seed_dy(const float* d_hidden, const int32_t* lengths, const int32_t* row_start, int B, int S, int H, int Tp,
                       bf16_t* dy, hipStream_t stream);
int plb_launch_ce_fwd_bwd(const float* logits, int ldl, int V, const int32_t* tgt, const float* w, int n, int npad,
                          float* loss_rows, bf16_t* dlogits, int ldd, hipStream_t stream);
int plb_launch_sum_rows(const float* x, int n, float* out, hipStream_t stream);
int plb_launch_token_ce_combine(const float* pmax, const float* psum, int ntiles, const float* tlogit,
                                const int32_t* lengths, int B, int S, int rows, float* lse, float* w, float* loss_rows,
                                hipStream_t stream);
int plb_launch_token_ce_combine_packed(const float* pmax, const float* psum, int ntiles, const float* tlogit,
                                       const int32_t* lengths, const int32_t* row_start, int B, int S, int rows, float* lse,
                                       float* w, float* loss_rows, hipStream_t stream);
int plb_launch_pack_token_targets(const int64_t* token_ids, const int32_t* lengths, const int32_t* row_start, int B, int S,
                                  int rows, int64_t* out, hipStream_t stream);
int plb_launch_add_scalar(float* out, const float* a, const float* b, hipStream_t stream);

typedef struct {
  const int64_t* labels; const int32_t* lengths;
  int B, S;
  uint64_t seed; uint32_t step;
  float word_pred_prob, mask_prob, replace_prob;
  int mask_id, sep_id;
  int64_t* masked; int32_t *counts, *idx_padded, *offsets, *flat;
} PlbMask;
int plb_launch_mask(const PlbMask* p, hipStream_t stream);

typedef struct {
  const int64_t* ids; const int32_t *sample_off, *word_off, *word_begin, *word_len; const int8_t* action;
  const int64_t* repl; const int64_t* word_token; int64_t sep_token; const int32_t* crop_start;
  int B, S, mask_id;
  int64_t *labels, *masked, *tokens; int32_t *lengths_out, *counts, *idx_padded, *offsets, *flat;
} PlbApplyMask;
int plb_launch_apply_mask(const PlbApplyMask* p, hipStream_t stream);

int plb_launch_adamw(float* p, const float* g, float* m, float* v, bf16_t* p_bf16, size_t n, double lr, double beta1,
                     double beta2, double eps, double wd, int step, double grad_scale, unsigned int* skip_if_nonzero,
                     int count_skip, hipStream_t stream);
#define PLB_NORM_PARTS 1024
static inline size_t plb_norm_chunk(size_t n) {
  return (n + (size_t)PLB_NORM_PARTS * 1024 - 1) / ((size_t)PLB_NORM_PARTS * 1024) * 1024;
}
#define PLB_NORM_CHAIN(n) (4 * (plb_norm_chunk(n) / 1024) + 6 + 3)
int plb_launch_grad_accum(float* accum, float* grads, size_t n, int phase, float* partials, hipStream_t stream);
int plb_launch_grad_sumsq(const float* grads, size_t n, float* partials, hipStream_t stream);
int plb_launch_grad_norm_finish(const float* partials, int nparts, double grad_scale, double max_norm, float* out,
                                hipStream_t stream);
int plb_launch_adamw_clipped(float* p, const float* g, float* m, float* v, bf16_t* p_bf16, size_t n, double lr, double beta1,
                             double beta2, double eps, double wd, int step, double grad_scale,
                             unsigned int* skip_if_nonzero, int count_skip, float* norm, int count_nonfinite,
                             hipStream_t stream);
int plb_launch_step_status(unsigned int* ln_err, float* loss, unsigned int* host_mirror, const float* summed, hipStream_t stream);
int plb_launch_status_export(const unsigned int* ln_err, float* out, hipStream_t stream);
int plb_launch_cast_bf16(const float* src, bf16_t* dst, size_t n, hipStream_t stream);
int plb_launch_transpose_cast(const float* src, int R, int C, bf16_t* dst, int ldd, hipStream_t stream);
int plb_launch_transpose_cast_multi(int n, const float* const* src, const int* R, const int* C, bf16_t* const* dst,
                                    const int* ldd, hipStream_t stream);
int plb_launch_bf16_to_f32(const bf16_t* src, int lds_, float* dst, int ldd, int R, int C, hipStream_t stream);

}
```

Before: 1.771 million tokens/s.

## Fill weight-grad GEMM tails with dense.weight rider tiles and move slab sums aside

The split-K weight-gradient GEMM kernel can now take extra 'rider' work units: pieces of the dense.weight gradient GEMM are placed in the idle slots of the QKV/FFN/FFN-out weight-grad launches, and the remaining rows run in a smaller follow-up launch. Separately, the per-weight slab reductions are issued on a new dedicated stream with events, using a second slab buffer, so they overlap with the next weight-grad GEMM. This targets tail underutilisation of the GPU and serialized reduction kernels in the backward pass. The cost is extra workspace, more event synchronisation, and a larger kernel argument plus per-block rider branching.

```diff
diff --git a/include/plbert.h b/include/plbert.h
--- a/include/plbert.h
+++ b/include/plbert.h
@@ -169,6 +169,8 @@
 void plb_set_gemm_nt_prefetch(int on);
 void plb_set_attn_bwd_fused(int on);
 void plb_set_prune_last(int on);
+void plb_set_tn_riders(int on);
+void plb_set_tn_sums_aside(int on);
 
 #ifdef __cplusplus
 }
diff --git a/plbert_amd/_lib.py b/plbert_amd/_lib.py
--- a/plbert_amd/_lib.py
+++ b/plbert_amd/_lib.py
@@ -53,6 +53,7 @@
     "plb_mask_batch", "plb_profile_enable", "plb_profile_num_classes", "plb_profile_class_name", "plb_profile_read",
     "plb_debug_skip_piece", "plb_debug_ln_fault", "plb_debug_hb_audit", "plb_debug_hb_report", "plb_comm_trace", "plb_comm_trace_read",
     "plb_set_gemm_nt_tile", "plb_set_gemm_nt_prefetch", "plb_set_attn_bwd_fused", "plb_set_prune_last",
+    "plb_set_tn_riders", "plb_set_tn_sums_aside",
 ]
 
 
@@ -87,6 +88,21 @@
         ("A", C.c_void_p), ("lda", C.c_int), ("Ncols", C.c_int), ("B", C.c_void_p), ("ldb", C.c_int),
         ("Mtot", C.c_int), ("N", C.c_int), ("K", C.c_int), ("rows_per_split", C.c_int), ("splits", C.c_int),
         ("slab", C.c_void_p), ("deq_a", C.c_void_p), ("deq_b", C.c_void_p),
+    ]
+
+
+class PlbTNUnit(C.Structure):
+    _fields_ = [("tile", C.c_int), ("t_begin", C.c_int), ("rows", C.c_int), ("slot", C.c_int)]
+
+
+PLB_TN_MAX_RIDERS = 32
+
+
+class PlbGemmTNRiders(C.Structure):
+    _fields_ = [
+        ("A", C.c_void_p), ("lda", C.c_int), ("Ncols", C.c_int), ("B", C.c_void_p), ("ldb", C.c_int),
+        ("Mtot", C.c_int), ("N", C.c_int), ("K", C.c_int), ("slab", C.c_void_p), ("slots", C.c_int),
+        ("n_units", C.c_int), ("unit", PlbTNUnit * PLB_TN_MAX_RIDERS),
     ]
 
 
@@ -336,6 +352,13 @@
     L.plb_launch_attn_bwd_fused.argtypes = [C.POINTER(PlbAttn), vp]
     L.plb_set_prune_last.restype = None
     L.plb_set_prune_last.argtypes = [C.c_int]
+    if hasattr(L, "plb_set_tn_riders"):
+        L.plb_set_tn_riders.restype = None
+        L.plb_set_tn_riders.argtypes = [C.c_int]
+        L.plb_set_tn_sums_aside.restype = None
+        L.plb_set_tn_sums_aside.argtypes = [C.c_int]
+        L.plb_launch_gemm_tn_big_pair.restype = C.c_int
+        L.plb_launch_gemm_tn_big_pair.argtypes = [C.POINTER(PlbGemmTN), C.POINTER(PlbGemmTNRiders), vp]
     L.plb_set_attn_bwd_fused.restype = None
     L.plb_set_attn_bwd_fused.argtypes = [C.c_int]
     L.plb_launch_ln_fwd.restype = C.c_int
diff --git a/plbert_amd/csrc/engine.cpp b/plbert_amd/csrc/engine.cpp
--- a/plbert_amd/csrc/engine.cpp
+++ b/plbert_amd/csrc/engine.cpp
@@ -135,15 +135,23 @@
       const int ntp = (int)rup(e->NT, 256);
       const int shapes[7][2] = {{(int)(3 * H), (int)H}, {(int)H, (int)H}, {(int)I, (int)H}, {(int)H, (int)I}, {(int)H, (int)E}, {e->NP, (int)H}, {ntp, (int)H}};
       for (int i = 0; i < (e->NT ? 7 : 6); ++i) {
-        int rps;
         const int64_t mt = i < 4 ? Mtot : Tp;
-        const int s = tn_splits(mt, shapes[i][0], shapes[i][1], &rps);
-        const int64_t f = (int64_t)s * shapes[i][0] * shapes[i][1];
+        int64_t s = tn_splits_ceiling(shapes[i][0], shapes[i][1]);
+        if (s > mt / 64) s = mt / 64 > 0 ? mt / 64 : 1;
+        const int64_t f = s * shapes[i][0] * shapes[i][1];
         if (f > slab) slab = f;
       }
     }
     e->slab_floats = slab;
     e->o_slab = cv.take(slab * 4);
+    if (H % 256 == 0 && I % 256 == 0) {
+      const int64_t dtiles = (H / 256) * (H / 256);
+      e->slabd_floats = (kTnRiderSlotsMax + (dtiles >= 256 ? 1 : 256 / dtiles)) * H * H;
+      e->o_slabd = cv.take(e->slabd_floats * 4);
+      const int64_t f1 = (int64_t)tn_splits_ceiling((int)I, (int)H) * I * H, f3 = (int64_t)tn_splits_ceiling((int)H, (int)H) * H * H;
+      e->slabB_floats = f1 > f3 ? f1 : f3;
+      e->o_slabB = cv.take(e->slabB_floats * 4);
+    }
     e->o_part1 = cv.take(L * e->part_rows * 3 * H * 4);
     e->o_part2 = cv.take(L * e->part_rows * 3 * H * 4);
     e->o_parte = cv.take((int64_t)e->emb_blocks * 2 * E * 4);
@@ -204,6 +212,8 @@
   if (e->ev_fork) (void)hipEventDestroy(e->ev_fork);
   if (e->ev_join) (void)hipEventDestroy(e->ev_join);
   if (e->side) (void)hipStreamDestroy(e->side);
+  for (auto ev : {e->ev_tn, e->ev_red[0], e->ev_red[1], e->ev_red[2], e->ev_join_red}) if (ev) (void)hipEventDestroy(ev);
+  if (e->red) (void)hipStreamDestroy(e->red);
   if (e->host_err) (void)hipHostFree(e->host_err);
   for (auto& t : e->trace) { (void)hipEventDestroy(t.released); (void)hipEventDestroy(t.done); }
   for (auto ev : e->trace_pool) (void)hipEventDestroy(ev);
@@ -253,6 +263,17 @@
       (void)hipStreamDestroy(e->side);
       e->side = nullptr;
     }
+    if (e->side && e->o_slabB && hipStreamCreateWithFlags(&e->red, hipStreamNonBlocking) == hipSuccess) {
+      bool ok = hipEventCreateWithFlags(&e->ev_tn, kStreamOrderEvent) == hipSuccess &&
+                hipEventCreateWithFlags(&e->ev_join_red, kStreamOrderEvent) == hipSuccess;
+      for (int i = 0; i < 3; ++i) ok = ok && hipEventCreateWithFlags(&e->ev_red[i], kStreamOrderEvent) == hipSuccess;
+      if (!ok) {
+        (void)hipStreamDestroy(e->red);
+        e->red = nullptr;
+      }
+    } else {
+      e->red = nullptr;
+    }
   }
   return 0;
 }
diff --git a/plbert_amd/csrc/engine_calls.cpp b/plbert_amd/csrc/engine_calls.cpp
--- a/plbert_amd/csrc/engine_calls.cpp
+++ b/plbert_amd/csrc/engine_calls.cpp
@@ -277,25 +277,44 @@
   const bool ov = overlapping(e);
   const bool t8 = e->tn8_call;
   float* const slab = e->at<float>(e->o_slab);
-  HB_W(s, slab, e->slab_floats * 4, "weight-gradient slab"); HB_W(s, e->grd(PLB_Q_W), 3 * H * H * 4, "Q/K/V weight gradients");
+  TnRiderPlan rp;
+  if (!t8) {
+    const int64_t hrows[kTnRiderHosts] = {Mtot, Mtot_c, Mtot_c};
+    const int hn[kTnRiderHosts] = {3 * H, I, H}, hk[kTnRiderHosts] = {H, H, I};
+    if (tn_rider_plan(e, hrows, hn, hk, st.dpre1, st.ctx, Mtot_c, H, H, &rp)) return 1;
+  }
+  const bool aside = !t8 && s2 != s && tn_sums_aside(e, Mtot, Mtot_c);
+  hipStream_t const sr = aside ? e->red : s;
+  float* const slabB = aside ? e->at<float>(e->o_slabB) : slab;
+  const int64_t slabB_bytes = (aside ? e->slabB_floats : e->slab_floats) * 4;
+  const auto sum_in = [&](int buf) { SlabSum v; if (aside) { v.stream = sr; v.buf = buf; } return v; };
+  if (rp.on) HB_W(s, e->at<float>(e->o_slabd), e->slabd_floats * 4, "dense.weight gradient slab (rider units)");
+  HB_W(s, slab, e->slab_floats * 4, "weight-gradient slab");
+  if (!aside) HB_W(s, e->grd(PLB_Q_W), 3 * H * H * 4, "Q/K/V weight gradients");
   if (t8 ? weight_grad8(e, st.dq8, st.x8, Mtot, 3 * H, H, F8_DQ, F8_X, e->grd(PLB_Q_W), s)
-         : weight_grad(e, st.dqkv, 3 * H, 3 * H, st.x, H, Mtot, 3 * H, H, e->grd(PLB_Q_W), s)) return 1;
-  if (ov && reduce_pieces(e, kPieceQkvW, kPieceFfnW, s)) return 1;
-  HB_W(s, slab, e->slab_floats * 4, "weight-gradient slab"); HB_W(s, e->grd(PLB_FFN_W), (int64_t)I * H * 4, "ffn.weight gradient");
+         : weight_grad(e, st.dqkv, 3 * H, 3 * H, st.x, H, Mtot, 3 * H, H, e->grd(PLB_Q_W), s, false, rp.on ? &rp.host[0] : nullptr, sum_in(0))) return 1;
+  if (ov && reduce_pieces(e, kPieceQkvW, kPieceFfnW, sr)) return 1;
+  HB_W(s, slabB, slabB_bytes, "weight-gradient slab");
+  if (!aside) HB_W(s, e->grd(PLB_FFN_W), (int64_t)I * H * 4, "ffn.weight gradient");
   if (t8 ? weight_grad8(e, st.du8, st.a8, Mtot_c, I, H, F8_DU, F8_A, e->grd(PLB_FFN_W), s)
-         : weight_grad(e, st.du, I, I, st.a, H, Mtot_c, I, H, e->grd(PLB_FFN_W), s)) return 1;
-  if (ov && reduce_pieces(e, kPieceFfnW, kPieceSmall, s)) return 1;
+         : weight_grad(e, st.du, I, I, st.a, H, Mtot_c, I, H, e->grd(PLB_FFN_W), s, false, rp.on ? &rp.host[1] : nullptr, sum_in(1))) return 1;
+  if (ov && reduce_pieces(e, kPieceFfnW, kPieceSmall, sr)) return 1;
   if (ov) {
     if (reduce_pieces(e, kPieceSmall, kPieceFfnoW, s2)) return 1;
   }
-  HB_W(s, slab, e->slab_floats * 4, "weight-gradient slab"); HB_W(s, e->grd(PLB_FFNO_W), (int64_t)I * H * 4, "ffn_output.weight gradient");
+  if (aside) HIPTRY(ev_wait(e, s, e->ev_red[0]));
+  HB_W(s, slab, e->slab_floats * 4, "weight-gradient slab");
+  if (!aside) HB_W(s, e->grd(PLB_FFNO_W), (int64_t)I * H * 4, "ffn_output.weight gradient");
   if (t8 ? weight_grad8(e, st.dp8, st.g8, Mtot_c, H, I, F8_DP, F8_G, e->grd(PLB_FFNO_W), s)
-         : weight_grad(e, st.dpre2, H, H, st.g, I, Mtot_c, H, I, e->grd(PLB_FFNO_W), s)) return 1;
-  if (ov && reduce_pieces(e, kPieceFfnoW, kPieceDenseW, s)) return 1;
-  HB_W(s, slab, e->slab_floats * 4, "weight-gradient slab"); HB_W(s, e->grd(PLB_DENSE_W), (int64_t)H * H * 4, "dense.weight gradient");
+         : weight_grad(e, st.dpre2, H, H, st.g, I, Mtot_c, H, I, e->grd(PLB_FFNO_W), s, false, rp.on ? &rp.host[2] : nullptr, sum_in(0))) return 1;
+  if (ov && reduce_pieces(e, kPieceFfnoW, kPieceDenseW, sr)) return 1;
+  if (aside && !rp.on) HIPTRY(ev_wait(e, s, e->ev_red[1]));
+  if (!rp.on) HB_W(s, slabB, slabB_bytes, "weight-gradient slab");
+  if (!aside) HB_W(s, e->grd(PLB_DENSE_W), (int64_t)H * H * 4, "dense.weight gradient");
   if (t8 ? weight_grad8(e, st.dp18, st.c8, Mtot_c, H, H, F8_DP1, F8_C, e->grd(PLB_DENSE_W), s)
-         : weight_grad(e, st.dpre1, H, H, st.ctx, H, Mtot_c, H, H, e->grd(PLB_DENSE_W), s)) return 1;
-  if (ov && reduce_pieces(e, kPieceDenseW, kNPieces, s)) return 1;
+         : rp.on ? weight_grad_rest(e, rp, st.dpre1, st.ctx, Mtot_c, H, H, e->grd(PLB_DENSE_W), s, sum_in(2))
+                 : weight_grad(e, st.dpre1, H, H, st.ctx, H, Mtot_c, H, H, e->grd(PLB_DENSE_W), s, false, nullptr, sum_in(1))) return 1;
+  if (ov && reduce_pieces(e, kPieceDenseW, kNPieces, sr)) return 1;
   return 0;
 }
 
@@ -311,7 +330,13 @@
     HIPTRY(ev_record(e, e->ev_fork, s));
     HIPTRY(ev_wait(e, s2, e->ev_fork));
   }
+  e->red_used = false;
   const int rc = backward_tail_streams(e, masked_ids, lengths, dy, B, S, rw, du_rows, s, s2, scratch2);
+  if (e->red_used) {
+    (void)ev_record(e, e->ev_join_red, e->red);
+    const hipError_t je = ev_wait(e, s, e->ev_join_red);
+    if (!rc && je != hipSuccess) return fail("plb_loss_fwd_bwd: joining the slab sums' stream: %s", hipGetErrorString(je));
+  }
   if (s2 != s) {
     if (rc) (void)ev_record(e, e->ev_join, s2);
     const hipError_t je = ev_wait(e, s, e->ev_join);
diff --git a/plbert_amd/csrc/engine_comm.cpp b/plbert_amd/csrc/engine_comm.cpp
--- a/plbert_amd/csrc/engine_comm.cpp
+++ b/plbert_amd/csrc/engine_comm.cpp
@@ -72,6 +72,7 @@
 int hb_idx(const PlbEngine* e, hipStream_t s) {
   if (e->side && s == e->side) return HbAudit::SIDE;
   if (e->comm_stream && s == e->comm_stream) return HbAudit::COMM;
+  if (e->red && s == e->red) return HbAudit::RED;
   return HbAudit::MAIN;
 }
 hipError_t ev_record(PlbEngine* e, hipEvent_t ev, hipStream_t s) {
diff --git a/plbert_amd/csrc/engine_internal.h b/plbert_amd/csrc/engine_internal.h
--- a/plbert_amd/csrc/engine_internal.h
+++ b/plbert_amd/csrc/engine_internal.h
@@ -37,19 +37,19 @@
 typedef void* RcclComm;
 
 struct HbAudit {
-  enum { MAIN = 0, SIDE = 1, COMM = 2, NS = 3 };
+  enum { MAIN = 0, SIDE = 1, COMM = 2, RED = 3, NS = 4 };
   typedef std::array<uint64_t, NS> VC;
   struct Acc { const char* what; uintptr_t a, b; int st; uint64_t tick; bool wr; };
   bool on = false;
   int break_wait = -1;
   int waits = 0;
-  VC vc[NS] = {{0, 0, 0}, {0, 0, 0}, {0, 0, 0}};
+  VC vc[NS] = {};
   std::map<hipEvent_t, VC> ev;
   std::vector<Acc> log;
   int64_t checks = 0;
   int violations = 0;
   std::string first;
-  static const char* name(int st) { return st == MAIN ? "main" : st == SIDE ? "side" : "comm"; }
+  static const char* name(int st) { return st == MAIN ? "main" : st == SIDE ? "side" : st == COMM ? "comm" : "slab-sum"; }
   void record(hipEvent_t e, int st) { vc[st][st] += 1; ev[e] = vc[st]; }
   void wait(int st, hipEvent_t e);
   void access(int st, const void* p, size_t bytes, bool wr, const char* what);
@@ -67,6 +67,7 @@
   int qkvcol_rows = 0;
   int64_t slab2_floats;
   int64_t slab_floats;
+  int64_t slabd_floats = 0;
   int64_t ws_bytes;
   int ln_blocks, emb_blocks;
   int part_rows = 0;
@@ -84,6 +85,8 @@
   int64_t o_dy0, o_dy1, o_da, o_dctx, o_de;
   int64_t o_hm, o_logm, o_dlog, o_dhm, o_rows, o_tgt, o_w, o_lrows;
   int64_t o_slab, o_part1, o_part2, o_parte, o_scratch, o_dxe, o_ducol, o_slab2, o_scratch2, o_qkvcol = 0;
+  int64_t o_slabd = 0, o_slabB = 0;
+  int64_t slabB_floats = 0;
   int64_t o_lnx = 0, o_lnerr = 0;
   int64_t o_bt = 0, o_wtT = 0, o_tdl = 0, o_tlrows = 0, o_tscr = 0, o_tgrad = 0, o_tloss = 0;
   int64_t o_tpmax = 0, o_tpsum = 0, o_ttl = 0, o_tlse = 0, o_tw = 0, o_ttgt = 0, o_tcolp = 0;
@@ -137,6 +140,9 @@
   bool tr_tail_valid = false;
   hipStream_t side = nullptr;
   hipEvent_t ev_fork = nullptr, ev_join = nullptr;
+  hipStream_t red = nullptr;
+  hipEvent_t ev_tn = nullptr, ev_red[3] = {nullptr, nullptr, nullptr}, ev_join_red = nullptr;
+  bool red_used = false;
   unsigned int* host_err = nullptr;
   unsigned int* host_err_dev = nullptr;
   float *params = nullptr, *grads = nullptr, *m = nullptr, *v = nullptr;
@@ -225,8 +231,25 @@
 int run_encoder(PlbEngine* e, const int64_t* ids, const int32_t* lengths, int B, int S, const Rows& rw, bool stash,
                 bf16_t** xout, hipStream_t s, const Prune* pr = nullptr);
 int tn_splits(int64_t Mtot, int N, int K, int* rows_per_split);
+int tn_splits_ceiling(int N, int K);
+constexpr int kTnRiderHosts = 3, kTnRiderSlotsMax = 8;
+struct TnRiderPlan {
+  bool on = false;
+  int slots = 0;
+  int64_t rows = 0;
+  int rows_per_split = 0, splits = 0;
+  PlbGemmTNRiders host[kTnRiderHosts];
+};
+int tn_rider_plan(PlbEngine* e, const int64_t host_rows[kTnRiderHosts], const int host_n[kTnRiderHosts],
+                  const int host_k[kTnRiderHosts], const bf16_t* A, const bf16_t* Bm, int64_t Mtot, int N, int K,
+                  TnRiderPlan* plan);
+struct SlabSum { hipStream_t stream = nullptr; int buf = 0; };
+bool tn_sums_aside(const PlbEngine* e, int64_t Mtot, int64_t Mtot_c);
 int weight_grad(PlbEngine* e, const bf16_t* A, int lda, int Ncols, const bf16_t* Bm, int ldb, int64_t Mtot, int N,
-                int K, float* out, hipStream_t s, bool side_slab = false);
+                int K, float* out, hipStream_t s, bool side_slab = false, const PlbGemmTNRiders* riders = nullptr,
+                SlabSum sum = SlabSum());
+int weight_grad_rest(PlbEngine* e, const TnRiderPlan& plan, const bf16_t* A, const bf16_t* Bm, int64_t Mtot, int N, int K,
+                     float* out, hipStream_t s, SlabSum sum = SlabSum());
 int weight_grad8(PlbEngine* e, const uint8_t* A8, const uint8_t* B8, int64_t Mtot, int N, int K, int site_a, int site_b,
                  float* out, hipStream_t s);
 int encoder_bwd(PlbEngine* e, const Prune* pr, const int32_t* lengths, int B, int S, const Rows& rw, bf16_t** dy,
diff --git a/plbert_amd/csrc/engine_layers.cpp b/plbert_amd/csrc/engine_layers.cpp
--- a/plbert_amd/csrc/engine_layers.cpp
+++ b/plbert_amd/csrc/engine_layers.cpp
@@ -29,6 +29,17 @@
   splits = (int)((Mtot + rps - 1) / rps);
   *rows_per_split = (int)rps;
   return splits;
+}
+
+int tn_splits_ceiling(int N, int K) {
+  int most = 768 / (((N + 127) / 128) * ((K + 127) / 128));
+  if (N % 256 == 0 && K % 256 == 0) {
+    const int tiles = (N / 256) * (K / 256);
+    const int s = 32 / tiles > 0 ? 32 / tiles : 1;
+    const int big = tiles >= 256 ? 1 : (tn_fill_chip() ? (tn_cus() / tiles > 0 ? tn_cus() / tiles : 1) : 8 * s);
+    if (big > most) most = big;
+  }
+  return most > 0 ? most : 1;
 }
 
 PlbGemmNT nt_desc(const bf16_t* A, const bf16_t* B, int64_t M, int N, int K) {
@@ -284,23 +295,134 @@
   return 0;
 }
 
+static int slab_sum(PlbEngine* e, const float* slab, int splits, size_t n, float* out, hipStream_t s, SlabSum sum) {
+  if (!sum.stream) return plb_launch_reduce_slabs(slab, splits, n, out, 0, s);
+  HIPTRY(ev_record(e, e->ev_tn, s));
+  HIPTRY(ev_wait(e, sum.stream, e->ev_tn));
+  e->red_used = true;
+  HB_R(sum.stream, slab, (int64_t)splits * n * 4, "weight-gradient slab (its sum)");
+  HB_W(sum.stream, out, n * 4, "weight gradient (sum of its slabs)");
+  TRY(plb_launch_reduce_slabs(slab, splits, n, out, 0, sum.stream));
+  HIPTRY(ev_record(e, e->ev_red[sum.buf], sum.stream));
+  return 0;
+}
+
+static int g_tn_sums_aside = -1;
+extern "C" void plb_set_tn_sums_aside(int on) { g_tn_sums_aside = on < 0 ? -1 : (on ? 1 : 0); }
+bool tn_sums_aside(const PlbEngine* e, int64_t Mtot, int64_t Mtot_c) {
+  static const bool v = [] { const char* x = getenv("PLBERT_TN_SUMS_ASIDE"); return !(x && !strcmp(x, "0")); }();
+  if (!(g_tn_sums_aside < 0 ? v : g_tn_sums_aside != 0) || !e->red || !e->side) return false;
+  const int64_t rows[4] = {Mtot, Mtot_c, Mtot_c, Mtot_c};
+  const int n[4] = {3 * e->H, e->I, e->H, e->H}, k[4] = {e->H, e->H, e->I, e->H};
+  for (int i = 0; i < 4; ++i) {
+    int rps;
+    if (!tn_big(rows[i], n[i], k[i]) || tn_splits(rows[i], n[i], k[i], &rps) < 2) return false;
+  }
+  return true;
+}
+
 int weight_grad(PlbEngine* e, const bf16_t* A, int lda, int Ncols, const bf16_t* Bm, int ldb, int64_t Mtot, int N,
-                       int K, float* out, hipStream_t s, bool side_slab) {
+                       int K, float* out, hipStream_t s, bool side_slab, const PlbGemmTNRiders* riders, SlabSum sum) {
   PlbGemmTN t;
   memset(&t, 0, sizeof(t));
   t.A = A; t.lda = lda; t.Ncols = Ncols; t.B = Bm; t.ldb = ldb; t.Mtot = (int)Mtot; t.N = N; t.K = K;
   t.splits = tn_splits(Mtot, N, K, &t.rows_per_split);
   const bool direct = t.splits == 1 && N == Ncols;
-  if (!direct && (int64_t)t.splits * N * K > (side_slab ? e->slab2_floats : e->slab_floats)) return fail("weight_grad: slab too small");
-  t.slab = direct ? out : e->at<float>(side_slab ? e->o_slab2 : e->o_slab);
+  const int64_t room = side_slab ? e->slab2_floats : sum.buf ? e->slabB_floats : e->slab_floats;
+  if (!direct && (int64_t)t.splits * N * K > room) return fail("weight_grad: slab too small");
+  t.slab = direct ? out : e->at<float>(side_slab ? e->o_slab2 : sum.buf ? e->o_slabB : e->o_slab);
+  if (direct && sum.stream) return fail("weight_grad: a direct launch has no slab sum to move");
   if (N == Ncols && tn_big(Mtot, Ncols, K)) {
-    const int tok = plb_prof_begin(PLB_K_GEMM_TN, s, 2.0 * (double)Mtot * N * K, 0.0);
-    TRY(plb_launch_gemm_tn_big(&t, s));
+    double flops = 2.0 * (double)Mtot * N * K;
+    if (riders)
+      for (int u = 0; u < riders->n_units; ++u) flops += 2.0 * (double)riders->unit[u].rows * 256 * 256;
+    const int tok = plb_prof_begin(PLB_K_GEMM_TN, s, flops, 0.0);
+    TRY(plb_launch_gemm_tn_big_pair(&t, riders, s));
     plb_prof_end(tok, s);
   } else {
+    if (riders && riders->n_units) return fail("weight_grad: rider units on a launch without the big-tile form");
     TRY(plb_launch_gemm_tn(&t, s));
   }
-  if (!direct) TRY(plb_launch_reduce_slabs(t.slab, t.splits, (size_t)N * K, out, 0, s));
+  if (!direct) TRY(slab_sum(e, t.slab, t.splits, (size_t)N * K, out, s, sum));
+  return 0;
+}
+
+static int g_tn_riders = -1;
+extern "C" void plb_set_tn_riders(int on) { g_tn_riders = on < 0 ? -1 : (on ? 1 : 0); }
+static bool tn_riders_enabled() {
+  static const bool v = [] { const char* e = getenv("PLBERT_TN_RIDERS"); return !(e && !strcmp(e, "0")); }();
+  return g_tn_riders < 0 ? v : g_tn_riders != 0;
+}
+
+int tn_rider_plan(PlbEngine* e, const int64_t host_rows[kTnRiderHosts], const int host_n[kTnRiderHosts],
+                  const int host_k[kTnRiderHosts], const bf16_t* A, const bf16_t* Bm, int64_t Mtot, int N, int K,
+                  TnRiderPlan* plan) {
+  *plan = TnRiderPlan();
+  if (!tn_riders_enabled() || !tn_fill_chip() || !e->slabd_floats || !tn_big(Mtot, N, K)) return 0;
+  const int rtiles = (N / 256) * (K / 256);
+  int free_cus[kTnRiderHosts], rps[kTnRiderHosts], total = 0;
+  for (int h = 0; h < kTnRiderHosts; ++h) {
+    if (!tn_big(host_rows[h], host_n[h], host_k[h])) return 0;
+    const int grid = (host_n[h] / 256) * (host_k[h] / 256) * tn_splits(host_rows[h], host_n[h], host_k[h], &rps[h]);
+    free_cus[h] = tn_cus() - grid;
+    if (free_cus[h] < 0) free_cus[h] = 0;
+    if (free_cus[h] > PLB_TN_MAX_RIDERS) free_cus[h] = PLB_TN_MAX_RIDERS;
+    total += free_cus[h];
+  }
+  int slots = total / rtiles;
+  if (slots > kTnRiderSlotsMax) slots = kTnRiderSlotsMax;
+  int host_of[kTnRiderHosts * PLB_TN_MAX_RIDERS];
+  for (int h = 0, j = 0; h < kTnRiderHosts; ++h)
+    for (int i = 0; i < free_cus[h] && j < slots * rtiles; ++i) host_of[j++] = h;
+  int64_t begin[kTnRiderSlotsMax + 1];
+  begin[0] = 0;
+  for (int k = 0; k < slots; ++k) {
+    int64_t len = rps[host_of[k * rtiles]];
+    for (int j = k * rtiles; j < (k + 1) * rtiles; ++j)
+      if (rps[host_of[j]] < len) len = rps[host_of[j]];
+    if (begin[k] + len > Mtot - 64) len = Mtot - 64 - begin[k];
+    if (len <= 0) { slots = k; break; }
+    begin[k + 1] = begin[k] + len;
+  }
+  if (slots == 0) return 0;
+  for (int h = 0; h < kTnRiderHosts; ++h) {
+    PlbGemmTNRiders& r = plan->host[h];
+    memset(&r, 0, sizeof(r));
+    r.A = A; r.lda = N; r.Ncols = N; r.B = Bm; r.ldb = K; r.Mtot = (int)Mtot; r.N = N; r.K = K;
+    r.slab = e->at<float>(e->o_slabd); r.slots = slots;
+  }
+  for (int j = 0; j < slots * rtiles; ++j) {
+    PlbGemmTNRiders& r = plan->host[host_of[j]];
+    const int k = j / rtiles;
+    r.unit[r.n_units++] = PlbTNUnit{j % rtiles, (int)begin[k], (int)(begin[k + 1] - begin[k]), k};
+  }
+  const int64_t rest = Mtot - begin[slots];
+  int splits = tn_cus() / rtiles > 0 ? tn_cus() / rtiles : 1;
+  if (splits > rest / 64) splits = (int)(rest / 64);
+  const int64_t r64 = rup((rest + splits - 1) / splits, 64);
+  plan->rows_per_split = (int)r64;
+  plan->splits = (int)((rest + r64 - 1) / r64);
+  plan->slots = slots;
+  plan->rows = begin[slots];
+  if ((int64_t)(slots + plan->splits) * N * K > e->slabd_floats) return fail("weight_grad: slab too small (rider layout)");
+  plan->on = true;
+  return 0;
+}
+
+int weight_grad_rest(PlbEngine* e, const TnRiderPlan& plan, const bf16_t* A, const bf16_t* Bm, int64_t Mtot, int N, int K,
+                     float* out, hipStream_t s, SlabSum sum) {
+  const int64_t rest = Mtot - plan.rows;
+  float* const slab = e->at<float>(e->o_slabd);
+  if ((int64_t)(plan.slots + plan.splits) * N * K > e->slabd_floats) return fail("weight_grad: slab too small (rider layout)");
+  PlbGemmTN t;
+  memset(&t, 0, sizeof(t));
+  t.A = A + plan.rows * N; t.lda = N; t.Ncols = N; t.B = Bm + plan.rows * K; t.ldb = K; t.Mtot = (int)rest; t.N = N; t.K = K;
+  t.rows_per_split = plan.rows_per_split; t.splits = plan.splits;
+  t.slab = slab + (size_t)plan.slots * N * K;
+  const int tok = plb_prof_begin(PLB_K_GEMM_TN, s, 2.0 * (double)rest * N * K, 0.0);
+  TRY(plb_launch_gemm_tn_big(&t, s));
+  plb_prof_end(tok, s);
+  TRY(slab_sum(e, slab, plan.slots + plan.splits, (size_t)N * K, out, s, sum));
   return 0;
 }
 
diff --git a/plbert_amd/csrc/gemm_big.hip b/plbert_amd/csrc/gemm_big.hip
--- a/plbert_amd/csrc/gemm_big.hip
+++ b/plbert_amd/csrc/gemm_big.hip
@@ -34,19 +34,26 @@
 
 DEVI int tn_g(int row) { return ((row >> 1) & 1) | (((row >> 3) & 1) << 1); }
 
-__global__ __launch_bounds__(512) __attribute__((amdgpu_num_vgpr(224))) void gemm_tn_big_kernel(PlbGemmTN p) {
+__global__ __launch_bounds__(512) __attribute__((amdgpu_num_vgpr(224))) void gemm_tn_big_kernel(PlbGemmTN p, PlbGemmTNRiders r) {
   __shared__ __attribute__((aligned(16))) bf16_t smem[2 * 4 * HT];
   const int tid = threadIdx.x, lane = tid & 63;
   const int uw = __builtin_amdgcn_readfirstlane(tid >> 6);
   const int wm = uw >> 2, wn = uw & 3;
-  const int nbk = p.K >> 8;
-  const int tiles = (p.Ncols >> 8) * nbk;
   const int logical = xcd_remap(blockIdx.x, gridDim.x);
-  const int split = logical / tiles, tile = logical % tiles;
+  const int grid1 = (p.Ncols >> 8) * (p.K >> 8) * p.splits;
+  const bool rider = logical >= grid1;
+  const PlbTNUnit ru = r.unit[rider ? logical - grid1 : 0];
+  const bf16_t* const opA = rider ? r.A : p.A;
+  const bf16_t* const opB = rider ? r.B : p.B;
+  const int lda = rider ? r.lda : p.lda, ldb = rider ? r.ldb : p.ldb;
+  const int pN = rider ? r.N : p.N, pK = rider ? r.K : p.K;
+  const int nbk = pK >> 8;
+  const int tiles = ((rider ? r.Ncols : p.Ncols) >> 8) * nbk;
+  const int split = rider ? ru.slot : logical / tiles, tile = rider ? ru.tile : logical % tiles;
   const int bn = tile / nbk, bk = tile % nbk;
-  const int t_begin = split * p.rows_per_split;
-  int t_end = t_begin + p.rows_per_split;
-  if (t_end > p.Mtot) t_end = p.Mtot;
+  const int t_begin = rider ? ru.t_begin : split * p.rows_per_split;
+  int t_end = t_begin + (rider ? ru.rows : p.rows_per_split);
+  if (!rider && t_end > p.Mtot) t_end = p.Mtot;
   const int nk = (t_end - t_begin) >> 6;
 
   const int i0 = 2 * uw, i1 = 2 * uw + 1;
@@ -101,8 +108,8 @@
   do { TR1(dst[0], ad_, (o_)); TR1(dst[1], ad_, (o_) + 512); TR1(dst[2], ad_, (o_) + 4096); TR1(dst[3], ad_, (o_) + 4608); PIN(); } while (0)
 #define RA4(buf, h, mi) RD4(ra1[mi], abase[buf][mi], (h) * 16384)
 #define RB4(bb, buf, h, ni) RD4(rb2[bb][ni], bbase[buf][ni], (2 + (h)) * 16384)
-#define SA_(h, kt) ((const char*)p.A + ((size_t)(t_begin + (kt) * 64) * p.lda + bn * 256 + (h) * 128) * 2)
-#define SB_(h, kt) ((const char*)p.B + ((size_t)(t_begin + (kt) * 64) * p.ldb + bk * 256 + (h) * 128) * 2)
+#define SA_(h, kt) ((const char*)opA + ((size_t)(t_begin + (kt) * 64) * lda + bn * 256 + (h) * 128) * 2)
+#define SB_(h, kt) ((const char*)opB + ((size_t)(t_begin + (kt) * 64) * ldb + bk * 256 + (h) * 128) * 2)
 #define STG_A(buf, h, kt)                                                                     \
   do {                                                                                        \
     const char* sb_ = SA_(h, kt);                                                             \
@@ -117,8 +124,8 @@
     DMA16(sb_, vB1, ldsb + (((buf) * 4 + 2 + (h)) * HT + dst1) * 2);                          \
     PIN();                                                                                    \
   } while (0)
-  const uint32_t vA0 = (uint32_t)(r0 * p.lda + sc0) * 2, vA1 = (uint32_t)(r1 * p.lda + sc1) * 2;
-  const uint32_t vB0 = (uint32_t)(r0 * p.ldb + sc0) * 2, vB1 = (uint32_t)(r1 * p.ldb + sc1) * 2;
+  const uint32_t vA0 = (uint32_t)(r0 * lda + sc0) * 2, vA1 = (uint32_t)(r1 * lda + sc1) * 2;
+  const uint32_t vB0 = (uint32_t)(r0 * ldb + sc0) * 2, vB1 = (uint32_t)(r1 * ldb + sc1) * 2;
   const uint32_t ldsb = LDS_ADDR(&smem[0]);
   unsigned abase[2][4], bbase[2][2];
 #pragma unroll
@@ -220,7 +227,7 @@
 #undef FRAG
 #undef LANDED
 
-  float* out = p.slab + (size_t)split * p.N * p.K;
+  float* out = (rider ? r.slab : p.slab) + (size_t)split * pN * pK;
   int lane_e = (int)__builtin_amdgcn_mbcnt_hi(~0u, __builtin_amdgcn_mbcnt_lo(~0u, 0u));
   asm volatile("" : "+v"(lane_e));
   const int li_e = lane_e & 15, fg_e = lane_e >> 4;
@@ -229,25 +236,48 @@
 #pragma unroll
     for (int mi = 0; mi < 4; ++mi) {
       const int n = bn * 256 + mh * 128 + wm * 64 + mi * 16 + li_e;
-      if (n >= p.N) continue;
+      if (n >= pN) continue;
 #pragma unroll
       for (int nh = 0; nh < 2; ++nh)
 #pragma unroll
         for (int ni = 0; ni < 2; ++ni) {
           const int k0 = bk * 256 + nh * 128 + wn * 32 + ni * 16 + 4 * fg_e;
           const f32x4 v = acc[mh][mi][nh][ni];
-          *(float4*)(out + (size_t)n * p.K + k0) = make_float4(v[0], v[1], v[2], v[3]);
+          *(float4*)(out + (size_t)n * pK + k0) = make_float4(v[0], v[1], v[2], v[3]);
         }
     }
 }
 
 }
 
+static int tn_big_ok(const PlbGemmTN* p) {
+  if (p->Ncols % 256 || p->K % 256 || p->rows_per_split % 64 || p->Mtot % 64 || p->splits <= 0) return 0;
+  if ((long)p->splits * p->rows_per_split < p->Mtot) return 0;
+  return 1;
+}
+
 extern "C" int plb_launch_gemm_tn_big(const PlbGemmTN* p, hipStream_t stream) {
-  if (p->Ncols % 256 || p->K % 256 || p->rows_per_split % 64 || p->Mtot % 64 || p->splits <= 0) return 1;
-  if ((long)p->splits * p->rows_per_split < p->Mtot) return 1;
+  if (!tn_big_ok(p)) return 1;
+  const PlbGemmTNRiders r = {};
   dim3 grid((p->Ncols / 256) * (p->K / 256) * p->splits), block(512);
-  hipLaunchKernelGGL(gemm_tn_big_kernel, grid, block, 0, stream, *p);
+  hipLaunchKernelGGL(gemm_tn_big_kernel, grid, block, 0, stream, *p, r);
+  return hipGetLastError() == hipSuccess ? 0 : 2;
+}
+
+extern "C" int plb_launch_gemm_tn_big_pair(const PlbGemmTN* p, const PlbGemmTNRiders* r, hipStream_t stream) {
+  if (!r || r->n_units == 0) return plb_launch_gemm_tn_big(p, stream);
+  if (!tn_big_ok(p)) return 1;
+  if (r->n_units < 0 || r->n_units > PLB_TN_MAX_RIDERS || !r->A || !r->B || !r->slab) return 1;
+  if (r->Ncols <= 0 || r->K <= 0 || r->Ncols % 256 || r->K % 256 || r->Mtot % 64 || r->N <= 0 || r->N > r->Ncols) return 1;
+  if (r->lda < r->Ncols || r->ldb < r->K || r->slots <= 0) return 1;
+  const int rtiles = (r->Ncols / 256) * (r->K / 256);
+  for (int u = 0; u < r->n_units; ++u) {
+    const PlbTNUnit& q = r->unit[u];
+    if (q.tile < 0 || q.tile >= rtiles || q.slot < 0 || q.slot >= r->slots) return 1;
+    if (q.t_begin < 0 || q.rows < 0 || q.rows % 64 || (long)q.t_begin + q.rows > r->Mtot) return 1;
+  }
+  dim3 grid((p->Ncols / 256) * (p->K / 256) * p->splits + r->n_units), block(512);
+  hipLaunchKernelGGL(gemm_tn_big_kernel, grid, block, 0, stream, *p, *r);
   return hipGetLastError() == hipSuccess ? 0 : 2;
 }
 
diff --git a/plbert_amd/csrc/plbert_kernels.h b/plbert_amd/csrc/plbert_kernels.h
--- a/plbert_amd/csrc/plbert_kernels.h
+++ b/plbert_amd/csrc/plbert_kernels.h
@@ -72,6 +72,17 @@
 int plb_launch_gemm_tn(const PlbGemmTN* p, hipStream_t stream);
 int plb_launch_gemm_tn_fp8(const PlbGemmTN* p, hipStream_t stream);
 int plb_launch_gemm_tn_big(const PlbGemmTN* p, hipStream_t stream);
+#define PLB_TN_MAX_RIDERS 32
+typedef struct { int tile, t_begin, rows, slot; } PlbTNUnit;
+typedef struct {
+  const bf16_t* A; int lda; int Ncols;
+  const bf16_t* B; int ldb;
+  int Mtot, N, K;
+  float* slab; int slots;
+  int n_units;
+  PlbTNUnit unit[PLB_TN_MAX_RIDERS];
+} PlbGemmTNRiders;
+int plb_launch_gemm_tn_big_pair(const PlbGemmTN* p, const PlbGemmTNRiders* r, hipStream_t stream);
 
 int plb_launch_reduce_slabs(const float* slab, int splits, size_t n, float* out, int accumulate, hipStream_t stream);
 
```

After: 1.765 million tokens/s. No clear change (-0.3%).
